# 3dlg-hcvc/minsu3d

Measured on AMD Instinct MI355X. Metric: scenes/sec (fwd+bwd) PointGroup on ~150k-pt 2cm voxels, higher is better.
Workload: dtype f32; 1 GPU; PointGroup m=16, synthetic ScanNet-shaped scenes (~144k points, ~106k voxels @2cm each), 4 scenes/GPU/step, grouping+ScoreNet branch on, fwd+loss+bwd+Adam; scenes_per_gpu=4, parallelism=dp1, grouping_inputs=GT labels, GT offsets + N(0,4cm) (random-init net groups nothing)

## Files before the change

include/minsu3d_hip.h:

```cpp
#ifndef MINSU3D_HIP_H
#define MINSU3D_HIP_H
#include <stddef.h>
#include <stdint.h>

#ifdef __cplusplus
extern "C" {
#endif

#define MS3D_E_WORKSPACE 10001
#define MS3D_E_UNSUPPORTED 10002
#define MS3D_E_INTERNAL 10003

typedef void *ms3d_stream_t;

const char *ms3d_version(void);

size_t ms3d_ballquery_workspace_bytes(int n);
int ms3d_ballquery_batch_p(int n, int meanActive, float radius, const float *xyz, const uint8_t *batch_idxs,
                           const int *batch_offsets, int n_scenes, int max_scene_points, int *idx,
                           int *start_len, int *n_active , int *capped ,
                           void *workspace, size_t workspace_bytes, ms3d_stream_t stream);

size_t ms3d_bfs_workspace_bytes(int N);
int ms3d_pg_bfs_cluster(const int16_t *semantic_label, const int *ball_query_idxs, long n_edges ,
// ... 172 lines not shown
int ms3d_spconv_layer_backward(const float *x, const float *dy, const float *wf_buf, const int *nbr_fwd,
                               const int *nbr_bwd, int Vin, int Vout, int K, int Cin, int Cout, const float *scale,
                               const float *shift, const float *mean, const float *invstd, int pre_relu, int training,
                               int need_dx, float *dx,
                               const float *dx_add ,
                               float *dgb, float *dW, float *ws,
                               const int *ol_fwd_kt_start , const int *ol_fwd_entries,
                               const int *pl_bwd_tile_start , const int *pl_bwd_entries,
                               void *ev_start , void *ev_stop,
                               void *ev_wg_start , void *ev_wg_stop,
                               float *ws_wgrad ,
                               ms3d_stream_t wgrad_stream ,
                               int join ,
                               float *wgrad_slabs ,
                               int *wgrad_deferred_nblk ,
                               void *wgrad_deferred_launch ,
                               ms3d_stream_t stream);
int ms3d_spconv_aux_kind_p(int K, int Cin, int Cout, int precision);
int ms3d_spconv_prep_weights_multi_p(const void *descs, int n, int total_blocks, int precision, ms3d_stream_t stream);
int ms3d_spconv_wgrad_pieces(int Vout, int K, int Cin, int Cout, int offset_list, int precision);
size_t ms3d_spconv_wgrad_ws_floats_p(int Vout, int K, int Cin, int Cout, int precision);
int ms3d_spconv_backward_weight_p(const float *in, const float *dout, const int *nbr, int Vout, int K, int Cin,
                                  int Cout, float *dW, const float *pre_scale, const float *pre_shift, int pre_relu,
                                  float *partial_ws, const int *ol_kt_start, const int *ol_entries, int precision,
                                  ms3d_stream_t stream);
int ms3d_spconv_layer_forward_p(const float *x, const float *W, const int *nbr_fwd, int Vout, int K, int Cin, int Cout,
                                int mirror_bwd, const float *pre_scale, const float *pre_shift, int pre_relu,
                                const float *residual, const float *bias, float *wf_buf, float *y, float *stat_partial,
                                const int *pl_tile_start, const int *pl_entries, void *ev_start, void *ev_stop,
                                int precision, ms3d_stream_t stream);
int ms3d_spconv_layer_backward_p(const float *x, const float *dy, const float *wf_buf, const int *nbr_fwd,
                                 const int *nbr_bwd, int Vin, int Vout, int K, int Cin, int Cout, const float *scale,
                                 const float *shift, const float *mean, const float *invstd, int pre_relu, int training,
                                 int need_dx, float *dx, const float *dx_add, float *dgb, float *dW, float *ws,
                                 const int *ol_fwd_kt_start, const int *ol_fwd_entries, const int *pl_bwd_tile_start,
                                 const int *pl_bwd_entries, void *ev_start, void *ev_stop, void *ev_wg_start,
                                 void *ev_wg_stop, float *ws_wgrad, ms3d_stream_t wgrad_stream, int join,
                                 float *wgrad_slabs, int *wgrad_deferred_nblk, void *wgrad_deferred_launch, int precision,
                                 ms3d_stream_t stream);
int ms3d_spconv_wgrad_is_bf16x3_g(int Vout, int K, int Cin, int Cout, int offset_list, int submanifold);
int ms3d_spconv_backward_weight_g(const float *in, const float *dout, const int *nbr, int Vin, int Vout, int K, int Cin,
                                  int Cout, float *dW, const float *pre_scale, const float *pre_shift, int pre_relu,
                                  float *partial_ws, const int *ol_kt_start, const int *ol_entries, int submanifold,
                                  int precision, ms3d_stream_t stream);
int ms3d_spconv_layer_backward_g(const float *x, const float *dy, const float *wf_buf, const int *nbr_fwd,
                                 const int *nbr_bwd, int Vin, int Vout, int K, int Cin, int Cout, const float *scale,
                                 const float *shift, const float *mean, const float *invstd, int pre_relu, int training,
                                 int need_dx, float *dx, const float *dx_add, float *dgb, float *dW, float *ws,
                                 const int *ol_fwd_kt_start, const int *ol_fwd_entries, const int *pl_bwd_tile_start,
                                 const int *pl_bwd_entries, void *ev_start, void *ev_stop, void *ev_wg_start,
                                 void *ev_wg_stop, float *ws_wgrad, ms3d_stream_t wgrad_stream, int join,
                                 float *wgrad_slabs, int *wgrad_deferred_nblk, void *wgrad_deferred_launch, int precision,
                                 int submanifold, ms3d_stream_t stream);
size_t ms3d_spconv_wgrad_launch_bytes(void);
int ms3d_spconv_wgrad_is_table_walk(int Vout, int K, int Cin, int Cout, int offset_list);
int ms3d_spconv_wgrad_multi(const void *descs, int n_desc, int total_blocks, int variant, ms3d_stream_t stream);
int ms3d_wgrad_reduce_blocks(long n, const float *slabs, const float *dW, int *wide );
int ms3d_wgrad_reduce_multi(const void *descs, int n_desc, int total_blocks, ms3d_stream_t stream);

int ms3d_bn_stats(const float *x, long V, int C, float eps, float momentum, const float *gamma, const float *beta,
                  float *running_mean, float *running_var, float *mean, float *invstd, float *scale, float *shift,
                  float *partial_ws, int partial_rows, ms3d_stream_t stream);
int ms3d_bn_apply(const float *x, long V, int C, const float *scale, const float *shift, int relu, float *y,
                  ms3d_stream_t stream);
int ms3d_reduce_partials(const float *partial, int nparts, int n, float *out, ms3d_stream_t stream);
int ms3d_column_sum(const float *x, long V, int C, float *partial_ws, int partial_rows, float *out2c, ms3d_stream_t stream);
int ms3d_bn_bwd_apply(const float *dz, const float *x, long V, int C, const float *scale, const float *mean,
                      const float *invstd, const float *s1s2, float *dx, ms3d_stream_t stream);
int ms3d_bn_bwd_reduce_apply(const float *partial, int nparts, const float *dz, const float *x, long V, int C,
                             const float *scale, const float *mean, const float *invstd, const float *add, float *dx,
                             float *s1s2, ms3d_stream_t stream);
int ms3d_bn_bwd_apply_add(const float *dz, const float *x, long V, int C, const float *scale, const float *mean,
                          const float *invstd, const float *s1s2, const float *add, float *dx, ms3d_stream_t stream);
int ms3d_bn_bwd_partial(const float *dy, const float *x, long V, int C, const float *scale, const float *shift,
                        const float *mean, const float *invstd, int relu, float *dz, float *partial_ws,
                        int partial_rows, int *nparts_out , ms3d_stream_t stream);

int ms3d_proposal_cross_intersection(const int *pair_point, const int *pair_cluster, int S, int P, int *inter ,
                                     ms3d_stream_t stream);
int ms3d_nms_greedy(const int *inter, const int *order, int P, float threshold, unsigned char *suppressed_ws, int *pick,
                    int *n_pick, ms3d_stream_t stream);

int ms3d_elastic_distort(const double *xyz , int N, float *noise, float *noise_tmp, int bx, int by, int bz,
                         double gran, double mag, double *out , ms3d_stream_t stream);

int ms3d_adam_chunk_elems(void);
int ms3d_adam_step(const int *chunks, int n_chunks, void *const *p_ptrs, const void *const *g_ptrs, void *const *m_ptrs,
                   void *const *v_ptrs, const long *sizes, float lr, float beta1, float beta2, float eps,
                   float weight_decay, double bias_correction1, double bias_correction2, ms3d_stream_t stream);
int ms3d_adam_step_multi(const int *chunks, int n_chunks, void *const *p_ptrs, const void *const *g_ptrs,
                         void *const *m_ptrs, void *const *v_ptrs, const long *sizes, const float *coef, float beta1,
                         float beta2, float eps, float weight_decay, ms3d_stream_t stream);

size_t ms3d_scan_i32_workspace_bytes(void);
int ms3d_scan_i32(const int *in, int *out, int n, int *total_out_dev, void *workspace, ms3d_stream_t stream);

int ms3d_point_losses_blocks(long N);
int ms3d_point_losses_forward(const float *scores , const short *labels , const float *pred_offsets ,
                              const float *centre , const float *xyz , const short *instance_ids ,
                              long N, int C, float *d_scores, float *d_norm, float *d_dir, double *partial_ws, float *out5,
                              ms3d_stream_t stream);
int ms3d_point_losses_scale_grads(float *d_scores, long n_scores, float *d_norm, const float *d_dir, long n_off,
                                  const float *out5, const float *g_sem, const float *g_norm, const float *g_dir,
                                  ms3d_stream_t stream);

#ifdef __cplusplus
// ... 4 lines not shown
```

minsu3d_amd/MinkowskiEngine/functional.py:

```python
import contextlib
import threading

import torch

from ..backend import get_backend

PRECISION_CODES = {"highest": 0, "high": 1, "medium": 2}
_pass = threading.local()


def precision_code(name):
    try:
        return PRECISION_CODES[name]
    except KeyError:
        raise ValueError(f"unknown float32 matmul precision {name!r}") from None


@contextlib.contextmanager
def pass_precision(code):
    prev = getattr(_pass, "code", None)
    _pass.code = code
    try:
        yield
    finally:
# ... 92 lines not shown
                skip[1].armed = True
            elif not (skip[1].armed and residual is not None):
                skip = None
        ctx.skip = skip
        ctx.save_for_backward(x, W)
        ctx.mark_non_differentiable(stats)
        ctx.set_materialize_grads(False)
        return y, stats

    @staticmethod
    def backward(ctx, dy, _dstats):
        be = get_backend()
        spec, bn = ctx.spec, ctx.bn
        x, W = ctx.saved_tensors
        dy = dy.contiguous()
        role, link = ctx.skip if ctx.skip is not None else (None, None)
        add = None
        if role == "head":
            add, link.grad = link.grad, None
        if bn is not None and not bn["relu"]:
            wft = be.prep_weights(W.view(spec.K, spec.cin, spec.cout), spec.K, spec.cout, spec.cin, transpose=True,
                                  mirror=spec.mirror)
            da = be.conv_forward(dy, wft, spec.nbr_bwd, spec.vin, spec.K, spec.cout, spec.cin)
            dz, dgb = be.bn_bwd_reduce(da, x, bn["scale"], bn["shift"], bn["mean"], bn["invstd"], False)
            dx = (be.bn_bwd_apply(dz, x, bn["scale"], bn["mean"], bn["invstd"], dgb) if bn["training"] else dz * bn["scale"])
            dW = be.conv_backward_weight(x, dy, spec.nbr_fwd, spec.vout, spec.K, spec.cin, spec.cout,
                                         pre=(bn["scale"], bn["shift"]), pre_relu=False, **_pk(ctx.prec), **_sk(spec))
        else:
            fused = add is not None and ctx.needs_input_grad[0] and be.fuses_dx_add(bn)
            extra = {"dx_add": add} if fused else {}
            if _queue(ctx.defer) is not None:
                extra["defer"] = _queue(ctx.defer)
            elif (not ctx.w_direct or (W.is_leaf and W.grad is not None)) and hasattr(be, "wgrad_stream_mode") \
                    and be.wgrad_stream_mode() == 2:
                extra["join_now"] = True
            dx, dgb, dW = be.conv_layer_backward(x, dy, ctx.wf_buf, spec.nbr_fwd, spec.nbr_bwd, spec.vin, spec.vout,
                                                 spec.K, spec.cin, spec.cout, bn, ctx.needs_input_grad[0], **extra,
                                                 **_pk(ctx.prec), **_sk(spec))
            if fused:
                add = None
        if add is not None and dx is not None:
            dx = dx + add
        dgamma = dgb[1] if dgb is not None else None
        dbeta = dgb[0] if dgb is not None else None
        d_res = dy if ctx.has_res else None
        if role == "tail" and ctx.has_res:
            link.grad, d_res = dy, None
        db = None
        if ctx.bias_shape is not None and ctx.needs_input_grad[9]:
            db = (be.column_sum(dy) if (hasattr(be, "column_sum") and dy.is_cuda) else dy.sum(0)).view(ctx.bias_shape)
        return dx, dW.view_as(W), dgamma, dbeta, d_res, None, None, None, None, db


class ResBlockFn(torch.autograd.Function):

    @staticmethod
    def forward(ctx, x, W1, g0, b0, W2, g1, b1, spec, stats_in, bn0, bn1, want_stats):
        be = get_backend()
        V = spec.vout
        tok = getattr(be, "weight_token", None)
        prec = ctx.prec = conv_precision(be)
        r1, r2 = _ready(W1, tok, prec), _ready(W2, tok, prec)
        fast = None
        if (r1 is not None and r2 is not None and spec.cin == spec.cout and torch.is_tensor(stats_in) and x.is_contiguous()
                and hasattr(be, "res_block_forward")):
            fast = be.res_block_forward(x, stats_in, r1, r2, spec.nbr_fwd, V, spec.cout, bn0, g0.detach(), b0.detach(), bn1,
                                        g1.detach(), b1.detach(), want_stats, **_pk(prec))
        if fast is not None:
            y1, y2, st2, (m0, i0, s0, h0), (m1, i1, s1, h1) = fast
            wf1, wf2 = r1, r2
        else:
            m0, i0, s0, h0 = be.bn_finalize(stats_in, V, bn0.eps, bn0.momentum, g0.detach(), b0.detach(), bn0.running_mean,
                                            bn0.running_var)
            y1, st1, wf1 = be.conv_layer_forward(x, W1, spec.nbr_fwd, V, 27, spec.cin, spec.cout, True, (s0, h0), True, None,
                                                 None, True, **({"wf_ready": r1} if r1 is not None else {}), **_pk(prec))
            m1, i1, s1, h1 = be.bn_finalize(st1, V, bn1.eps, bn1.momentum, g1.detach(), b1.detach(), bn1.running_mean,
                                            bn1.running_var)
            y2, st2, wf2 = be.conv_layer_forward(y1, W2, spec.nbr_fwd, V, 27, spec.cout, spec.cout, True, (s1, h1), True, x,
                                                 None, want_stats, **({"wf_ready": r2} if r2 is not None else {}), **_pk(prec))
        ctx.spec, ctx.wf = spec, (wf1, wf2)
        ctx.bn = (dict(scale=s0, shift=h0, mean=m0, invstd=i0, relu=True, training=True),
                  dict(scale=s1, shift=h1, mean=m1, invstd=i1, relu=True, training=True))
        ctx.defer = (_defer_of(W1, tok), _defer_of(W2, tok))
        ctx.save_for_backward(x, y1, W1, W2)
        if st2 is None:
            st2 = x.new_zeros(0)
        ctx.mark_non_differentiable(st2)
        ctx.set_materialize_grads(False)
        return y2, st2

    @staticmethod
    def backward(ctx, dy, _dstats):
        be = get_backend()
        spec = ctx.spec
        x, y1, W1, W2 = ctx.saved_tensors
        dy = dy.contiguous()
        V, c0, c1 = spec.vout, spec.cin, spec.cout
        e2 = {"defer": _queue(ctx.defer[1])} if _queue(ctx.defer[1]) is not None else {}
        dx1, dgb1, dW2 = be.conv_layer_backward(y1, dy, ctx.wf[1], spec.nbr_fwd, spec.nbr_bwd, V, V, 27, c1, c1, ctx.bn[1], True, **e2,
                                                **_pk(ctx.prec))
        e1 = {"defer": _queue(ctx.defer[0])} if _queue(ctx.defer[0]) is not None else {}
        dx, dgb0, dW1 = be.conv_layer_backward(x, dx1, ctx.wf[0], spec.nbr_fwd, spec.nbr_bwd, V, V, 27, c0, c1, ctx.bn[0],
                                               ctx.needs_input_grad[0], dx_add=dy, **e1, **_pk(ctx.prec))
        return dx, dW1.view_as(W1), dgb0[1], dgb0[0], dW2.view_as(W2), dgb1[1], dgb1[0], None, None, None, None, None


class ResBlockDownFn(torch.autograd.Function):

    @staticmethod
    def forward(ctx, x, Wd, W1, g0, b0, W2, g1, b1, spec, ident, stats_in, bn0, bn1):
        be = get_backend()
        V, cin, cout = spec.vout, spec.cin, spec.cout
        tok = getattr(be, "weight_token", None)
        prec = ctx.prec = conv_precision(be)

        def ready(W):
            r = _ready(W, tok, prec)
            return dict({"wf_ready": r} if r is not None else {}, **_pk(prec))

        skip, _, wfd = be.conv_layer_forward(x, Wd.view(1, cin, cout), ident, V, 1, cin, cout, False, None, False, None, None,
                                             False, **ready(Wd))
        if isinstance(stats_in, tuple):
            m0, i0, s0, h0 = be.bn_finalize_parts(stats_in, V, bn0.eps, bn0.momentum, g0.detach(), b0.detach(),
                                                  bn0.running_mean, bn0.running_var)
        else:
            m0, i0, s0, h0 = be.bn_finalize(stats_in, V, bn0.eps, bn0.momentum, g0.detach(), b0.detach(), bn0.running_mean,
                                            bn0.running_var)
        y1, st1, wf1 = be.conv_layer_forward(x, W1, spec.nbr_fwd, V, 27, cin, cout, True, (s0, h0), True, None, None, True,
                                             **ready(W1))
        m1, i1, s1, h1 = be.bn_finalize(st1, V, bn1.eps, bn1.momentum, g1.detach(), b1.detach(), bn1.running_mean,
                                        bn1.running_var)
        y2, st2, wf2 = be.conv_layer_forward(y1, W2, spec.nbr_fwd, V, 27, cout, cout, True, (s1, h1), True, skip, None, True,
                                             **ready(W2))
        ctx.spec, ctx.wf, ctx.ident = spec, (wfd, wf1, wf2), ident
        ctx.bn = (dict(scale=s0.contiguous(), shift=h0.contiguous(), mean=m0.contiguous(), invstd=i0.contiguous(), relu=True,
                       training=True),
                  dict(scale=s1, shift=h1, mean=m1, invstd=i1, relu=True, training=True))

        ctx.defer = (_defer_of(Wd, tok), _defer_of(W1, tok), _defer_of(W2, tok))
        ctx.save_for_backward(x, y1, Wd, W1, W2)
        ctx.mark_non_differentiable(st2)
        ctx.set_materialize_grads(False)
        return y2, st2

    @staticmethod
    def backward(ctx, dy, _dstats):
        be = get_backend()
        spec = ctx.spec
        x, y1, Wd, W1, W2 = ctx.saved_tensors
        dy = dy.contiguous()
        V, cin, cout = spec.vout, spec.cin, spec.cout
        ex = lambda d: dict({"defer": _queue(d)} if _queue(d) is not None else {}, **_pk(ctx.prec))
        dx1, dgb1, dW2 = be.conv_layer_backward(y1, dy, ctx.wf[2], spec.nbr_fwd, spec.nbr_bwd, V, V, 27, cout, cout, ctx.bn[1],
                                                True, **ex(ctx.defer[2]))
        need = ctx.needs_input_grad[0]
        dxb, dgb0, dW1 = be.conv_layer_backward(x, dx1, ctx.wf[1], spec.nbr_fwd, spec.nbr_bwd, V, V, 27, cin, cout, ctx.bn[0],
                                                need, **ex(ctx.defer[1]))
        dx, _, dWd = be.conv_layer_backward(x, dy, ctx.wf[0], ctx.ident, ctx.ident, V, V, 1, cin, cout, None, need,
                                            **({"dx_add": dxb} if need else {}), **ex(ctx.defer[0]))
        return dx, dWd.view_as(Wd), dW1.view_as(W1), dgb0[1], dgb0[0], dW2.view_as(W2), dgb1[1], dgb1[0], None, None, None, None, None


class BnReluConvFn(torch.autograd.Function):

    @staticmethod
    def forward(ctx, x, W, g, b, spec, stats_in, bn, want_stats):
        be = get_backend()
        tok = getattr(be, "weight_token", None)
        if isinstance(stats_in, tuple):
            m0, i0, s0, h0 = be.bn_finalize_parts(stats_in, spec.vin, bn.eps, bn.momentum, g.detach(), b.detach(),
                                                  bn.running_mean, bn.running_var)
        else:
            m0, i0, s0, h0 = be.bn_finalize(stats_in, spec.vin, bn.eps, bn.momentum, g.detach(), b.detach(), bn.running_mean,
                                            bn.running_var)
        prec = ctx.prec = conv_precision(be)
        r = _ready(W, tok, prec)
        y, st, wf = be.conv_layer_forward(x, W.view(spec.K, spec.cin, spec.cout), spec.nbr_fwd, spec.vout, spec.K, spec.cin,
                                          spec.cout, spec.mirror, (s0, h0), True, None, None, want_stats,
                                          **({"wf_ready": r} if r is not None else {}), **_pk(prec))
        ctx.spec, ctx.wf = spec, wf
        ctx.bn = dict(scale=s0.contiguous(), shift=h0.contiguous(), mean=m0.contiguous(), invstd=i0.contiguous(), relu=True,
                      training=True)
        ctx.defer = _defer_of(W, tok)
        ctx.save_for_backward(x, W)
        if st is None:
            st = x.new_zeros(0)
        ctx.mark_non_differentiable(st)
        ctx.set_materialize_grads(False)
        return y, st

    @staticmethod
    def backward(ctx, dy, _dstats):
        be = get_backend()
        spec = ctx.spec
        x, W = ctx.saved_tensors
        e = {"defer": _queue(ctx.defer)} if _queue(ctx.defer) is not None else {}
        dx, dgb, dW = be.conv_layer_backward(x, dy.contiguous(), ctx.wf, spec.nbr_fwd, spec.nbr_bwd, spec.vin, spec.vout, spec.K,
                                             spec.cin, spec.cout, ctx.bn, ctx.needs_input_grad[0], **e, **_pk(ctx.prec), **_sk(spec))
        return dx, dW.view_as(W), dgb[1], dgb[0], None, None, None, None


class BNActFn(torch.autograd.Function):
    @staticmethod
    def forward(ctx, x, gamma, beta, bn):
        ctx.bn = bn
        ctx.save_for_backward(x)
        return get_backend().bn_apply(x, bn["scale"], bn["shift"], bn["relu"])

    @staticmethod
    def backward(ctx, dy):
# ... 235 lines not shown
```

minsu3d_amd/backend.py:

```python
import ctypes as C
import os

import numpy as np
import torch

from . import _lib

_BACKEND = None


def get_backend():
    global _BACKEND
    if _BACKEND is None:
        _BACKEND = HipBackend()
    return _BACKEND


def set_backend(b):
    global _BACKEND
    prev = _BACKEND
    _BACKEND = b
    return prev


# ... 83 lines not shown
def wgrad_stream(device):
    s = _WGRAD.get(device)
    if s is None:
        s = _WGRAD[device] = torch.cuda.Stream(device=device)
    return s


_HEADS = {}


def heads_stream(device):
    s = _HEADS.get(device)
    if s is None:
        s = _HEADS[device] = torch.cuda.Stream(device=device)
    return s


def side_stream(device):
    s = _SIDE.get(device)
    if s is None:
        s = _SIDE[device] = torch.cuda.Stream(device=device)
    return s


def _load_host_ext():
    if os.environ.get("MS3D_HOST_EXT", "1") == "0":
        return None
    path = os.path.join(os.path.dirname(os.path.abspath(__file__)), "lib", "_ms3d_host.so")
    if not os.path.exists(path) or (os.environ.get("MS3D_LIB") and os.environ["MS3D_LIB"] != _lib.LIB_PATH):
        return None
    import importlib.util
    try:
        spec = importlib.util.spec_from_file_location("_ms3d_host", path)
        mod = importlib.util.module_from_spec(spec)
        spec.loader.exec_module(mod)
        return mod
    except (ImportError, OSError) as e:
        import warnings
        warnings.warn(f"minsu3d_amd: host extension {path} did not load ({e}); using the ctypes path")
        return None


class HipBackend:
    name = "hip"

    def __init__(self):
        self.lib = _lib.lib()
        self.ext = _load_host_ext() if not os.environ.get("MS3D_LIB") else None
        self.ws = _Workspace()
        self.kernel_timer = None
        self.weight_token = 0
        self.matmul_precision_aware = True
        self._prep_table = None

    @staticmethod
    def _dev(t):
        if not t.is_cuda:
            if not torch.cuda.is_available():
                raise _lib.HipLibraryError("HipBackend needs a GPU (got a CPU tensor and no device is present); "
                                           "the product path has no CPU fallback")
            t = t.cuda(non_blocking=True)
        return t.contiguous()

    def ballquery_batch_p(self, coords, batch_idxs, batch_offsets, radius, meanActive, max_scene_points=0):
        coords = self._dev(coords); batch_idxs = self._dev(batch_idxs); batch_offsets = self._dev(batch_offsets)
        n = coords.size(0)
        dev = coords.device
        start_len = torch.zeros((n, 2), dtype=torch.int32, device=dev)
        if n == 0:
            return torch.zeros(0, dtype=torch.int32, device=dev), start_len
        if max_scene_points <= 0:
            max_scene_points = SCENE_BOUNDS.get(batch_offsets)
            if max_scene_points is None:
                max_scene_points = int((batch_offsets[1:] - batch_offsets[:-1]).max().item())
                SCENE_BOUNDS.put(batch_offsets, max_scene_points)
        ws_bytes = self.lib.ms3d_ballquery_workspace_bytes(n)
        ws = self.ws.get("bq", ws_bytes, dev)
        n_active, capped = C.c_int(0), C.c_int(0)
        timer = self.kernel_timer
        ev0 = timer.op_begin() if timer is not None else None
        hint_key = (round(float(radius), 6), int(meanActive))
        hints = self.__dict__.setdefault("_bq_mean_active", {})
        meanActive = max(int(meanActive), hints.get(hint_key, 0))
        while True:
            idx = torch.empty(n * meanActive, dtype=torch.int32, device=dev)
            rc = self.lib.ms3d_ballquery_batch_p(
                n, int(meanActive), C.c_float(radius), _lib.ptr(coords), _lib.ptr(batch_idxs),
                _lib.ptr(batch_offsets), int(batch_offsets.numel() - 1), int(max_scene_points), _lib.ptr(idx),
                _lib.ptr(start_len), C.byref(n_active), C.byref(capped), _lib.ptr(ws), C.c_size_t(ws.numel()),
                _lib.stream_handle())
            _lib.check(rc, "ms3d_ballquery_batch_p")
            if n_active.value <= n * meanActive:
                break
            meanActive = int(n_active.value // n + 1)
            hints[hint_key] = meanActive + meanActive // 8 + 1
        if ev0 is not None:
            timer.op_end("ballquery_batch_p", ev0, n * 20 + n_active.value * (6.64 * 12 + 4))
        GRAPHS.put(start_len, int(capped.value))
        return idx[:n_active.value], start_len

    def _bfs(self, fn_name, args_head, ball_idx, start_len, args_tail):
        hint = int(GRAPHS.get(start_len, -1))
        ball_idx = self._dev(ball_idx); start_len = self._dev(start_len)
        N = start_len.size(0)
        dev = start_len.device
        cluster_idxs = torch.empty((max(N, 1), 2), dtype=torch.int32, device=dev)
# ... 236 lines not shown
            _lib.ptr(d_scores), C.c_long(d_scores.numel()), _lib.ptr(d_off[0]), _lib.ptr(d_off[1]),
            C.c_long(d_off[0].numel()), _lib.ptr(out5), _lib.ptr(g_sem), _lib.ptr(g_norm), _lib.ptr(g_dir),
            _lib.stream_handle()), "ms3d_point_losses_scale_grads")

    def _iou(self, fn_name, prop_idx, prop_off, inst_labels, inst_pointnum, sigmoid=None):
        prop_idx = self._dev(prop_idx); prop_off = self._dev(prop_off)
        inst_labels = self._dev(inst_labels); inst_pointnum = self._dev(inst_pointnum)
        assert prop_idx.dtype == torch.int32 and inst_labels.dtype == torch.int16
        I, P = inst_pointnum.numel(), prop_off.numel() - 1
        iou = torch.zeros((P, I), dtype=torch.float32, device=prop_idx.device)
        args = [I, P, _lib.ptr(prop_idx), _lib.ptr(prop_off), _lib.ptr(inst_labels), _lib.ptr(inst_pointnum),
                _lib.ptr(iou)]
        if sigmoid is not None:
            args.append(_lib.ptr(self._dev(sigmoid)))
        rc = getattr(self.lib, fn_name)(*args, _lib.stream_handle())
        _lib.check(rc, fn_name)
        return iou

    def get_iou(self, pi, po, il, pn): return self._iou("ms3d_get_iou", pi, po, il, pn)
    def get_mask_iou_on_cluster(self, pi, po, il, pn): return self._iou("ms3d_get_mask_iou_on_cluster", pi, po, il, pn)
    def get_mask_iou_on_pred(self, pi, po, il, pn, sg): return self._iou("ms3d_get_mask_iou_on_pred", pi, po, il, pn, sg)

    def get_mask_label(self, prop_idx, prop_off, inst_labels, inst_cls, iou, ignored_label, iou_thr):
        prop_idx = self._dev(prop_idx); prop_off = self._dev(prop_off); iou = self._dev(iou)
        P, I = iou.shape
        ml = torch.zeros(prop_idx.shape, dtype=torch.bool, device=prop_idx.device)
        mlm = torch.zeros(prop_idx.shape, dtype=torch.bool, device=prop_idx.device)
        rc = self.lib.ms3d_get_mask_label(I, P, int(ignored_label), C.c_float(iou_thr), _lib.ptr(prop_idx),
                                          _lib.ptr(prop_off), _lib.ptr(self._dev(inst_labels)),
                                          _lib.ptr(self._dev(inst_cls)), _lib.ptr(iou), _lib.ptr(ml), _lib.ptr(mlm),
                                          _lib.stream_handle())
        _lib.check(rc, "ms3d_get_mask_label")
        return ml, mlm


def _f32(t):
    return None if t is None else t.contiguous()


def _p(t):
    return None if t is None else t.data_ptr()


_VP, _I = C.c_void_p, C.c_int
_FAST_ARGTYPES = {
    "ms3d_spconv_layer_forward": [_VP] * 3 + [_I] * 5 + [_VP] * 2 + [_I] + [_VP] * 5 + [_VP] * 2 + [_VP] * 2 + [_VP],
    "ms3d_spconv_layer_backward": [_VP] * 5 + [_I] * 5 + [_VP] * 4 + [_I] * 3 + [_VP] * 5 + [_VP] * 4 + [_VP] * 4 +
                                  [_VP, _VP, _I, _VP, _VP, _VP, _VP],
    "ms3d_spconv_layer_forward_p": [_VP] * 3 + [_I] * 5 + [_VP] * 2 + [_I] + [_VP] * 5 + [_VP] * 2 + [_VP] * 2 + [_I, _VP],
    "ms3d_spconv_layer_backward_p": [_VP] * 5 + [_I] * 5 + [_VP] * 4 + [_I] * 3 + [_VP] * 5 + [_VP] * 4 + [_VP] * 4 +
                                    [_VP, _VP, _I, _VP, _VP, _VP, _I, _VP],
    "ms3d_spconv_layer_backward_g": [_VP] * 5 + [_I] * 5 + [_VP] * 4 + [_I] * 3 + [_VP] * 5 + [_VP] * 4 + [_VP] * 4 +
                                    [_VP, _VP, _I, _VP, _VP, _VP, _I, _I, _VP],
    "ms3d_bn_finalize": [_VP, _I, C.c_long, _I, C.c_float, C.c_float] + [_VP] * 4 + [_VP] * 4 + [_VP],
}


class KernelTimer:

    def __init__(self, lib):
        self.lib = lib
        lib.ms3d_event_create.restype = C.c_void_p
        lib.ms3d_event_elapsed_ms.restype = C.c_float
        self.records = []
        self.sampling = False
        self.steps_sampled = 0
        self._pool = []

    def reserve(self, n_events):
        while len(self._pool) < n_events:
            self._pool.append(C.c_void_p(self.lib.ms3d_event_create()))

    def _event(self):
        return self._pool.pop() if self._pool else C.c_void_p(self.lib.ms3d_event_create())

    def conv(self, kind, K, cin, cout, nbr, rows):
        if not self.sampling:
            return None
        pairs = getattr(nbr, "_ms3d_pairs_dev", None)
        if pairs is None:
            pairs = (nbr >= 0).sum()
            nbr._ms3d_pairs_dev = pairs
        ev = (self._event(), self._event())
        self.records.append((("spconv_" + kind, K, cin, cout, rows), ev[0], ev[1],
                             (pairs, (cin + cout) * 4 + 8, K * cin * cout * 4), 2 * cin * cout))
        return ev

    def conv_group(self, kind, layers):
        if not self.sampling or not layers:
            return None
        ev = (self._event(), self._event())
        parts = []
        for K, cin, cout, rows, nbr in layers:
            pairs = getattr(nbr, "_ms3d_pairs_dev", None)
            if pairs is None:
                pairs = (nbr >= 0).sum()
                nbr._ms3d_pairs_dev = pairs
            parts.append((pairs, (cin + cout) * 4 + 8, K * cin * cout * 4, 2 * cin * cout))
        K, cin, cout, rows, _ = layers[0]
        self.records.append((("spconv_" + kind, K, cin, cout, rows, len(layers)), ev[0], ev[1], parts, None))
        return ev

    def op_begin(self):
        if not self.sampling:
            return None
        ev = self._event()
# ... 575 lines not shown
        if not on:
            return None
        q = WgradQueue(self.lib, self.kernel_timer)
        q.side_mode = self.wgrad_stream_mode() == 3
        return q

    def wgrad_batch_enabled(self):
        on = self.__dict__.get("_wgrad_batch")
        if on is None:
            on = self._wgrad_batch = os.environ.get("MS3D_WGRAD_BATCH", "1") != "0"
        return on

    def conv_layer_forward(self, x, W3, nbr_fwd, vout, K, cin, cout, mirror_bwd, pre, pre_relu, residual, bias,
                           want_stats, wf_ready=None, precision=0):
        x = self._dev(x)
        dev = x.device
        wf_buf = wf_ready if wf_ready is not None else torch.empty(self.wf_floats(K, cin, cout), dtype=torch.float32, device=dev)
        pl = self.pairlist(nbr_fwd, K, vout, cin, cout)
        nparts = self._geom("ms3d_spconv_partial_blocks", vout, K, cin, cout, self._pl_rows(pl)) if want_stats else 0
        ps, pb = (pre if pre is not None else (None, None))
        timer = self.kernel_timer
        tok = timer.conv("fwd", K, cin, cout, nbr_fwd, vout) if timer is not None else None
        ev0, ev1 = tok if tok is not None else (None, None)
        ext = self.ext
        if ext is not None:
            y, stats = ext.conv_layer_forward(
                x, None if wf_ready is not None else self._dev(W3), nbr_fwd, vout, K, cin, cout, bool(mirror_bwd),
                _f32(ps), _f32(pb), bool(pre_relu), _f32(residual), _f32(bias), wf_buf, nparts, pl[0], pl[1],
                (ev0.value or 0) if ev0 is not None else 0, (ev1.value or 0) if ev1 is not None else 0, int(precision))
            return y, stats, wf_buf
        y = torch.empty((vout, cout), dtype=torch.float32, device=dev)
        stats = torch.empty((nparts, 2, cout), dtype=torch.float32, device=dev) if want_stats else None
        _lib.check(self._fast("ms3d_spconv_layer_forward_p")(
            _p(x), _p(None if wf_ready is not None else self._dev(W3)), _p(nbr_fwd), int(vout), int(K), int(cin), int(cout),
            int(bool(mirror_bwd)), _p(_f32(ps)), _p(_f32(pb)), int(bool(pre_relu)), _p(_f32(residual)),
            _p(_f32(bias)), _p(wf_buf), _p(y), _p(stats), _p(pl[0]), _p(pl[1]),
            ev0, ev1, int(precision), _lib.stream_handle()), "ms3d_spconv_layer_forward_p")
        return y, stats, wf_buf

    def res_block_forward(self, x, stats_in, wf1, wf2, nbr, V, c, bn0, g0, b0, bn1, g1, b1, want_stats, precision=0):
        ext = self.ext
        timer = self.kernel_timer
        if (ext is None or (timer is not None and getattr(timer, "sampling", True)) or not hasattr(ext, "res_block_forward")
                or os.environ.get("MS3D_RESBLOCK_EXT", "1") == "0"):
            return None
        pl = self.pairlist(nbr, 27, V, c, c)
        nparts = self._geom("ms3d_spconv_partial_blocks", V, 27, c, c, self._pl_rows(pl))
        y1, y2, st2, o0, o1 = ext.res_block_forward(
            x, stats_in, wf1, wf2, nbr, V, c, pl[0], pl[1], nparts, bool(want_stats), _f32(g0), _f32(b0), bn0.running_mean,
            bn0.running_var, bn0.eps, bn0.momentum, _f32(g1), _f32(b1), bn1.running_mean, bn1.running_var, bn1.eps, bn1.momentum,
            int(precision))
        return y1, y2, st2, o0.unbind(0), o1.unbind(0)

    def conv_layer_backward(self, x, dy, wf_buf, nbr_fwd, nbr_bwd, vin, vout, K, cin, cout, bn, need_dx, dx_add=None,
                            defer=None, join_now=False, precision=0, submanifold=None):
        sub = -1 if submanifold is None else int(bool(submanifold))
        x = self._dev(x); dy = self._dev(dy)
        dev = x.device
        ws = self.ws.get("layer", 4 * self._geom("ms3d_spconv_layer_ws_floats", vin, vout, K, cin, cout), dev)
        has_bn = bn is not None
        want_dx = need_dx or has_bn
        plf = self.offsetlist(nbr_fwd, K, vout)
        plb = self.pairlist(nbr_bwd, K, vin, cout, cin) if want_dx else (None, None)
        timer = self.kernel_timer
        tok = timer.conv("fwd", K, cout, cin, nbr_bwd, vin) if (timer is not None and want_dx) else None
        ev0, ev1 = tok if tok is not None else (None, None)
        tok = timer.conv("wgrad", K, cin, cout, nbr_fwd, vout) if timer is not None else None
        ev2, ev3 = tok if tok is not None else (None, None)
        mode = self.wgrad_stream_mode()
        batch = defer is not None and mode == 0 and self.wgrad_batch_enabled() and \
            self._geom("ms3d_spconv_wgrad_is_table_walk", vout, K, cin, cout, int(plf[0] is not None)) == 1
        timing = None
        if batch and ev2 is not None:
            timing = timer.records.pop()[0][1:] + (nbr_fwd,)
            timer._pool.extend((ev2, ev3))
            ev2 = ev3 = None
        if self.ext is not None and mode == 0:
            evs = [(e.value or 0) if e is not None else 0 for e in (ev0, ev1, ev2, ev3)]
            dx, dgb, dW, slabs, nblk, desc = (self.ext.conv_layer_backward_g if sub >= 0 else self.ext.conv_layer_backward)(
                x, dy, wf_buf, nbr_fwd, nbr_bwd, vin, vout, K, cin, cout,
                bn["scale"] if has_bn else None, bn["shift"] if has_bn else None, bn["mean"] if has_bn else None,
                bn["invstd"] if has_bn else None, bool(has_bn and bn["relu"]), bool(has_bn and bn["training"]), bool(need_dx),
                _f32(dx_add) if (dx_add is not None and need_dx) else None, ws, plf[0], plf[1], plb[0], plb[1], *evs,
                self._geom("ms3d_spconv_wgrad_ws_floats", vout, K, cin, cout) if defer is not None else 0, batch,
                int(precision), *((sub,) if sub >= 0 else ()))
            if desc:
                defer.add_launch(desc, (x, dy, nbr_fwd, bn, slabs, dW), timing)
            if nblk > 0:
                defer.add(slabs, dW, K * cin * cout, nblk)
            return dx, dgb, dW
        dx = torch.empty((vin, cin), dtype=torch.float32, device=dev) if want_dx else None
        dgb = torch.empty((2, cin), dtype=torch.float32, device=dev) if has_bn else None
        dW = torch.empty((K, cin, cout), dtype=torch.float32, device=dev)
        side = wgrad_stream(dev) if mode else None
        ws2 = None
        if side is not None:
            with torch.cuda.stream(side):
                ws2 = self.ws.get("layer_wgrad", 4 * self._geom("ms3d_spconv_layer_ws_floats", vin, vout, K, cin, cout), dev)
            if mode != 3:
                defer = None
        slabs, n_defer = None, None
        if defer is not None:
            if "_defer_n" not in self.__dict__:
                self._defer_n = C.c_int(0)
                self._defer_n_addr = C.addressof(self._defer_n)
            slabs = torch.empty(self._geom("ms3d_spconv_wgrad_ws_floats", vout, K, cin, cout), dtype=torch.float32, device=dev)
            n_defer = self._defer_n_addr
        launch = (C.c_char * 128)() if (batch and slabs is not None) else None
        _lib.check(self._fast("ms3d_spconv_layer_backward_g")(
            _p(x), _p(dy), _p(wf_buf), _p(nbr_fwd), _p(nbr_bwd), int(vin), int(vout), int(K),
            int(cin), int(cout), _p(bn["scale"] if has_bn else None), _p(bn["shift"] if has_bn else None),
            _p(bn["mean"] if has_bn else None), _p(bn["invstd"] if has_bn else None),
            int(bool(has_bn and bn["relu"])), int(bool(has_bn and bn["training"])), int(bool(need_dx)), _p(dx),
            _p(_f32(dx_add) if (dx_add is not None and need_dx) else None), _p(dgb), _p(dW), _p(ws), _p(plf[0]), _p(plf[1]), _p(plb[0]),
            _p(plb[1]), ev0, ev1, ev2, ev3, _p(ws2), side.cuda_stream if side is not None else None,
            int(mode == 1 or (mode == 2 and join_now) or (mode == 3 and defer is None)), _p(slabs), n_defer,
            C.addressof(launch) if launch is not None else None, int(precision),
            sub if sub >= 0 else int(K == 27 and vin == vout), _lib.stream_handle()),
            "ms3d_spconv_layer_backward_g")
        if launch is not None and np.frombuffer(launch, dtype=np.int32, count=6)[4] != 0:
            defer.add_launch(bytes(launch), (x, dy, nbr_fwd, bn, slabs, dW), timing)
        if slabs is not None and self._defer_n.value > 0:
            defer.add(slabs, dW, K * cin * cout, self._defer_n.value)
        if mode == 2:
            x.record_stream(side); dy.record_stream(side); dW.record_stream(side)
            if not join_now:
                self._queue_wgrad_join(side)
        elif mode == 3 and defer is not None:
            x.record_stream(side); dy.record_stream(side); dW.record_stream(side)
            if slabs is not None:
                slabs.record_stream(side)
        return (dx if need_dx else None), dgb, dW

    @staticmethod
    def fuses_dx_add(bn):
        return bn is None or (bool(bn["relu"]) and bool(bn["training"]))

    def wgrad_stream_mode(self):
        m = self.__dict__.get("_wgrad_mode")
        if m is None:
            m = self._wgrad_mode = int(os.environ.get("MS3D_WGRAD_STREAM", "0"))
        return m

    def _queue_wgrad_join(self, side):
        if self.__dict__.get("_wgrad_join_queued"):
            return

        def join():
            self._wgrad_join_queued = False
            torch.cuda.current_stream().wait_stream(side)
        try:
            torch.autograd.Variable._execution_engine.queue_callback(join)
            self._wgrad_join_queued = True
        except RuntimeError:
            join()

    def conv_backward_weight(self, x, dout, nbr, vout, K, cin, cout, pre=None, pre_relu=False, precision=0, submanifold=None):
        x = self._dev(x); dout = self._dev(dout)
        dW = torch.empty((K, cin, cout), dtype=torch.float32, device=x.device)
        ps, pb = (pre if pre is not None else (None, None))
        self.lib.ms3d_spconv_wgrad_ws_floats.restype = C.c_size_t
        ws = self.ws.get("wgrad", 4 * self.lib.ms3d_spconv_wgrad_ws_floats(int(vout), int(K), int(cin), int(cout)), x.device)
        ol = self.offsetlist(nbr, K, vout)
        if submanifold is not None:
            _lib.check(self.lib.ms3d_spconv_backward_weight_g(
                _lib.ptr(x), _lib.ptr(dout), _lib.ptr(nbr), int(x.size(0)), int(vout), int(K), int(cin), int(cout), _lib.ptr(dW),
                _lib.ptr(_f32(ps)), _lib.ptr(_f32(pb)), int(bool(pre_relu)), _lib.ptr(ws), _lib.ptr(ol[0]), _lib.ptr(ol[1]),
                int(bool(submanifold)), int(precision), _lib.stream_handle()), "ms3d_spconv_backward_weight_g")
            return dW
        _lib.check(self.lib.ms3d_spconv_backward_weight_p(
            _lib.ptr(x), _lib.ptr(dout), _lib.ptr(nbr), int(vout), int(K), int(cin), int(cout), _lib.ptr(dW),
            _lib.ptr(_f32(ps)), _lib.ptr(_f32(pb)), int(bool(pre_relu)), _lib.ptr(ws), _lib.ptr(ol[0]), _lib.ptr(ol[1]),
            int(precision), _lib.stream_handle()), "ms3d_spconv_backward_weight_p")
        return dW
# ... 90 lines not shown
```

minsu3d_amd/csrc/spconv.hip:

```cpp
#include <stdlib.h>
#include <atomic>
#include <map>
#include <mutex>
#include <unordered_map>
#include "common.h"
#include "../../include/minsu3d_hip.h"

typedef float f32x4 __attribute__((ext_vector_type(4)));

namespace {

constexpr int MAX_NBT = 8;
constexpr size_t LDS_BUDGET = 150 * 1024;
static hipError_t raise_lds_ceiling(const void *fn)
{
    hipFuncAttributes fa;
    hipError_t e = hipFuncGetAttributes(&fa, fn);
    if (e != hipSuccess) return e;
    return hipFuncSetAttribute(fn, hipFuncAttributeMaxDynamicSharedMemorySize, 160 * 1024 - (int)fa.sharedSizeBytes);
}

int env_int(const char *name, int dflt)
{
    const char *e = getenv(name);
    return e ? atoi(e) : dflt;
}

struct ConvArgs {
    const float *in;
    const float *wf;
    const float *wfs;
    const void *wfb;
    const int *nbr;
    float *out;
    const float *pre_scale;
    const float *pre_shift;
    const float *residual;
    const float *bias;
    const float *bn_x;
    const float *bn_scale;
    const float *bn_shift;
    const float *bn_mean;
    const float *bn_invstd;
    float *bn_partial;
    int out_stats;
    int Vout, K, Cin, Cout;
    int NCH;
    int NBtot;
    int G;
    int GC;
    int RT;
    int ntiles;
    int pre_relu;
    const int *pl_tile_start;
    const int *pl_entries;
    int dyn_picks;
    int k1_path;
    float *ws_slabs;
    unsigned *ws_cnt;
    int ws_ng, ws_kg, ws_R, ws_tpp;
};

__device__ __forceinline__ long stream_slot(long o, int NBtot)
{
    const int lane = (int)(o & 63);
    long r = o >> 6;
    const int nb = (int)(r % NBtot); r /= NBtot;
    const int t = (int)(r & 3); r >>= 2;
    return ((r * NBtot + nb) * 64 + lane) * 4 + t;
}

typedef __bf16 bf16x8 __attribute__((ext_vector_type(8)));

__host__ __device__ constexpr int aux_pieces(int aux_kind) { return aux_kind == 2 ? 3 : aux_kind == 3 ? 2 : aux_kind == 4 ? 1 : 0; }

__host__ __device__ inline bool bf3_dims_ok(int K, int Cin, int Cout)
{
    return K > 1 && Cin % 16 == 0 && Cout % 16 == 0 && Cin >= 48 && Cout >= 48 && Cin <= 256 && Cout <= 256;
}

__device__ __forceinline__ void split3(float v, __bf16 &h0, __bf16 &h1, __bf16 &h2)
{
    h0 = (__bf16)v;
    const float r1 = v - (float)h0;
    h1 = (__bf16)r1;
    const float r2 = r1 - (float)h1;
    h2 = (__bf16)r2;
}

typedef float f32x2_t __attribute__((ext_vector_type(2)));
typedef __bf16 bf16x2_t __attribute__((ext_vector_type(2)));
__device__ __forceinline__ uint32_t cvt_pk_bf16(float a, float b)
{
    const bf16x2_t h = __builtin_convertvector((f32x2_t){a, b}, bf16x2_t);
    return *reinterpret_cast<const uint32_t *>(&h);
}
template <int P = 3>
__device__ __forceinline__ void act_split8(const f32x4 &lo, const f32x4 &hi, bool affine, const f32x4 &s0, const f32x4 &s1,
                                           const f32x4 &b0, const f32x4 &b1, float floor_, int keep, bf16x8 &a0, bf16x8 &a1,
                                           bf16x8 &a2)
{
    float v[8];
#pragma unroll
    for (int t = 0; t < 4; t++) { v[t] = lo[t]; v[4 + t] = hi[t]; }
    if (affine) {
#pragma unroll
        for (int t = 0; t < 4; t++) {
            v[t] = fmaxf(fmaf(v[t], s0[t], b0[t]), floor_);
            v[4 + t] = fmaxf(fmaf(v[4 + t], s1[t], b1[t]), floor_);
        }
    }
    uint32_t q0[4], q1[4], q2[4];
    if constexpr (P == 3) {
#pragma unroll
// ... 139 lines not shown
        const int ch = (int)(r % NB), k = (int)(r / NB);
        const int c = 16 * ch + 4 * q + t, j = 16 * nb + jl;
        const int ks = d.mirror_bwd ? (d.K - 1 - k) : k;
        const float v = (c < d.Cout && j < d.Cin) ? d.W[((size_t)ks * d.Cin + j) * d.Cout + c] : 0.f;
        d.wft[o] = v;
        if (d.stream == 1) d.wft[total + stream_slot(o, NCH)] = v;
    }
    if (d.stream == 5 - PB) {
        constexpr int P = PB;
        auto image = [&](float *aux, int Ci, int Co, int nb_tot, bool transposed) {
            const int NC32 = (Ci + 31) >> 5;
            if (o >= (long)d.K * NC32 * nb_tot * 64) return;
            const int g = lane >> 4;
            long r = o >> 6;
            const int nb = (int)(r % nb_tot); r /= nb_tot;
            const int c32 = (int)(r % NC32), k = (int)(r / NC32);
            const int ks = (transposed && d.mirror_bwd) ? (d.K - 1 - k) : k;
            const int j = 16 * nb + jl;
            bf16x8 p0, p1, p2;
#pragma unroll
            for (int e = 0; e < 8; e++) {
                const int c = 32 * c32 + 8 * g + e;
                float v = 0.f;
                if (c < Ci && j < Co) v = transposed ? d.W[((size_t)ks * d.Cin + j) * d.Cout + c] : d.W[((size_t)ks * d.Cin + c) * d.Cout + j];
                __bf16 h0, h1, h2;
                split3(v, h0, h1, h2);
                p0[e] = h0; p1[e] = h1; p2[e] = h2;
            }
            bf16x8 *dst = reinterpret_cast<bf16x8 *>(aux) + ((((size_t)k * NC32 + c32) * nb_tot + nb) * P) * 64 + lane;
            dst[0] = p0;
            if (P >= 2) dst[64] = p1;
            if (P >= 3) dst[128] = p2;
        };
        image(d.wf + total, d.Cin, d.Cout, NB, false);
        image(d.wft + total, d.Cout, d.Cin, NCH, true);
    }
}

constexpr int OG = 9;

template <int GSZ>
__device__ __forceinline__ void load_indices(const ConvArgs &p, int row, int g0, int k_hi, int (&idx)[GSZ])
{
    const bool row_ok = row >= 0 && row < p.Vout;
    const int safe_row = row_ok ? row : 0;
#pragma unroll
    for (int u = 0; u < GSZ; u++) {
        const int k = min(g0 + u, k_hi - 1);
        const int v = p.nbr[(size_t)k * p.Vout + safe_row];
        idx[u] = v | ((row_ok && g0 + u < k_hi) ? 0 : -1);
    }
}

template <int NBT, bool ALIGNED, bool DIRECT = false, int GSZ = ((DIRECT || NBT < 5) ? OG : (NBT < 7 ? 7 : 6))>
__device__ __forceinline__ void accumulate_offsets(const ConvArgs &p, const float *__restrict__ sW, int k_lo, int k_hi,
                                                   int kw0, int my_row, int q, int nb0, f32x4 (&acc)[NBT])
{
    const int l = lane_id();
    int opaque0 = 0;
    asm volatile("" : "+s"(opaque0));
    for (int g0 = k_lo; g0 < k_hi; g0 += GSZ) {
        int idx[GSZ];
        load_indices(p, my_row, g0, k_hi, idx);
        bool any[GSZ];
#pragma unroll
        for (int u = 0; u < GSZ; u++) any[u] = __ballot(idx[u] >= 0) != 0ull;
        auto fetch = [&](int ch, f32x4 (&a)[GSZ], f32x4 &sc, f32x4 &sh) {
            const int c0 = 16 * ch + 4 * q;
#pragma unroll
            for (int u = 0; u < GSZ; u++) {
                const float *row = p.in + (size_t)max(idx[u], 0) * p.Cin + c0;
                if (ALIGNED) {
                    a[u] = *reinterpret_cast<const f32x4 *>(row);
                } else {
#pragma unroll
                    for (int t = 0; t < 4; t++) a[u][t] = (c0 + t < p.Cin) ? row[t] : 0.f;
                }
            }
            if (p.pre_scale) {
                if (ALIGNED) {
                    sc = *reinterpret_cast<const f32x4 *>(p.pre_scale + c0);
                    sh = *reinterpret_cast<const f32x4 *>(p.pre_shift + c0);
                } else {
#pragma unroll
                    for (int t = 0; t < 4; t++) {
                        sc[t] = (c0 + t < p.Cin) ? p.pre_scale[c0 + t] : 0.f;
                        sh[t] = (c0 + t < p.Cin) ? p.pre_shift[c0 + t] : 0.f;
                    }
                }
            }
        };
        f32x4 a_next[GSZ], sc_next = {0.f, 0.f, 0.f, 0.f}, sh_next = sc_next;
        if (DIRECT) fetch(0, a_next, sc_next, sh_next);
        for (int ch = 0; ch < p.NCH; ch++) {
            f32x4 a[GSZ], s = {0.f, 0.f, 0.f, 0.f}, b = s;
            if (DIRECT) {
#pragma unroll
                for (int u = 0; u < GSZ; u++) a[u] = a_next[u];
                s = sc_next;
                b = sh_next;
                if (ch + 1 < p.NCH) fetch(ch + 1 + opaque0, a_next, sc_next, sh_next);
            } else {
                fetch(ch, a, s, b);
            }
            if (p.pre_scale) {
#pragma unroll
                for (int u = 0; u < GSZ; u++)
#pragma unroll
                    for (int t = 0; t < 4; t++) {
                        const float v = fmaf(a[u][t], s[t], b[t]);
                        a[u][t] = p.pre_relu ? fmaxf(v, 0.f) : v;
                    }
            }
#pragma unroll
            for (int u = 0; u < GSZ; u++) {
                const int keep = ~(idx[u] >> 31);
#pragma unroll
                for (int t = 0; t < 4; t++) a[u][t] = __int_as_float(__float_as_int(a[u][t]) & keep);
            }
            if (DIRECT) {
                constexpr int UB0 = NBT <= 2 ? GSZ : (NBT <= 4 ? 3 : 1);
                constexpr int UB = UB0 < GSZ ? UB0 : GSZ;
#pragma unroll
                for (int u0 = 0; u0 < GSZ; u0 += UB) {
                    float wreg[UB][4][NBT];
#pragma unroll
                    for (int uu = 0; uu < UB; uu++) {
                        const float *w = p.wf + ((size_t)((min(g0 + u0 + uu, p.K - 1) * p.NCH + ch) * 4) * p.NBtot + nb0) * 64 + l;
#pragma unroll
                        for (int t = 0; t < 4; t++)
#pragma unroll
                            for (int nb = 0; nb < NBT; nb++) wreg[uu][t][nb] = w[(size_t)(t * p.NBtot + nb) * 64];
                    }
                    __builtin_amdgcn_sched_barrier(0);
#pragma unroll
                    for (int uu = 0; uu < UB; uu++)
#pragma unroll
                        for (int t = 0; t < 4; t++)
#pragma unroll
                            for (int nb = 0; nb < NBT; nb++)
                                acc[nb] = __builtin_amdgcn_mfma_f32_16x16x4f32(a[u0 + uu][t], wreg[uu][t][nb], acc[nb], 0, 0, 0);
                }
            } else {
#pragma unroll
                for (int u = 0; u < GSZ; u++) {
                    if (!any[u]) continue;
                    const float *w = sW + (size_t)(((kw0 + (g0 - k_lo) + u) * p.NCH + ch) * 4) * NBT * 64 + l;
#pragma unroll
                    for (int t = 0; t < 4; t++) {
#pragma unroll
                        for (int nb = 0; nb < NBT; nb++)
                            acc[nb] = __builtin_amdgcn_mfma_f32_16x16x4f32(a[u][t], w[(t * NBT + nb) * 64], acc[nb], 0, 0, 0);
                    }
                }
            }
        }
// ... 294 lines not shown
        }
    };

    {
        const int tile = vb * waves + wave_id();
        const int row0 = tile * 16, my_row = row0 + (l & 15);
        f32x4 acc[NBT];
#pragma unroll
        for (int nb = 0; nb < NBT; nb++) acc[nb] = (f32x4){0.f, 0.f, 0.f, 0.f};
        int idx[OG];
        load_idx(0, min(p.G, p.K), my_row, idx);
        for (int k0 = 0; k0 < p.K; k0 += p.G) {
            const int gn = min(p.G, p.K - k0);
            int idx_n[OG];
            load_idx(k0 + p.G, min(k0 + 2 * p.G, p.K), my_row, idx_n);
            bool any[OG];
#pragma unroll
            for (int u = 0; u < OG; u++) any[u] = __ballot(idx[u] >= 0) != 0ull;
            for (int c_lo = 0; c_lo < NC32; c_lo += GC) {
                const int ccnt = min(GC, NC32 - c_lo);
                Round r;
                gather(c_lo, idx, r);
                __syncthreads();
                stage(k0, gn, c_lo, ccnt);
                asm volatile("s_waitcnt vmcnt(0)" ::: "memory");
                __syncthreads();
                if (tile < p.ntiles) compute(c_lo, 0, ccnt, idx, any, r, acc);
                for (int cc = 1; cc < ccnt; cc++) {
                    gather(c_lo + cc, idx, r);
                    if (tile < p.ntiles) compute(c_lo + cc, cc, ccnt, idx, any, r, acc);
                }
            }
#pragma unroll
            for (int u = 0; u < OG; u++) idx[u] = idx_n[u];
        }
        if (tile < p.ntiles) store_tile<NBT>(p, row0, nb0, acc, s_part + (size_t)wave_id() * stat_slot_floats(NBT));
    }
    if (with_partial) stats_flush<NBT>(p, s_part, waves, nb0);
}

constexpr int bf3_round_offsets(int nbt) { return nbt == 2 || nbt == 4 || nbt == 6 ? 5 : 4; }

template <int NBT, int P = 3>
int launch_fwd_bf3(const ConvArgs &p, dim3 grid, int threads, size_t lds, hipStream_t stream)
{
    constexpr int OG = bf3_round_offsets(NBT);
    static const hipError_t attr = raise_lds_ceiling((const void *)spconv_fwd_bf3_kernel<NBT, OG, P>);
    MS3D_CHECK(attr);
    spconv_fwd_bf3_kernel<NBT, OG, P><<<grid, threads, lds, stream>>>(p);
    MS3D_LAUNCH_CHECK();
    return 0;
}

template <int NBT, bool ALIGNED>
__global__ __launch_bounds__(256) void spconv_fwd_small_kernel(ConvArgs p)
{
    extern __shared__ float lds[];
    const int l = lane_id(), q = l >> 4;
    const int waves = blockDim.x >> 6;
    const int nb0 = blockIdx.y * NBT;
    float *s_acc = lds;
    float *s_part = lds + (size_t)(waves - 1) * NBT * 256;
    const bool with_partial = p.bn_x != nullptr || p.out_stats != 0;
    if (with_partial) stats_clear<NBT>(s_part, 1);
    const int rt = p.RT > 1 ? p.RT : 1;
    for (int tt = 0; tt < rt; tt++) {
        const int tile = blockIdx.x * rt + tt;
        if (tile >= p.ntiles) break;
        const int row0 = tile * 16, my_row = row0 + (l & 15);
        f32x4 acc[NBT];
#pragma unroll
        for (int nb = 0; nb < NBT; nb++) acc[nb] = (f32x4){0.f, 0.f, 0.f, 0.f};
        const int k_lo = wave_id() * OG, k_hi = min(p.K, k_lo + OG);
        if (p.K == 1 && (p.k1_path & 2)) { if (k_lo < k_hi) accumulate_k1<NBT, ALIGNED, true>(p, nullptr, my_row, q, nb0, acc); }
        else if (k_lo < k_hi) accumulate_offsets<NBT, ALIGNED, true>(p, nullptr, k_lo, k_hi, 0, my_row, q, nb0, acc);
        if (tt > 0) __syncthreads();
        if (wave_id() > 0) {
#pragma unroll
            for (int nb = 0; nb < NBT; nb++)
#pragma unroll
                for (int r = 0; r < 4; r++) s_acc[((size_t)(wave_id() - 1) * NBT + nb) * 256 + r * 64 + l] = acc[nb][r];
        }
        __syncthreads();
        if (wave_id() == 0) {
            for (int w = 1; w < waves; w++)
#pragma unroll
                for (int nb = 0; nb < NBT; nb++)
#pragma unroll
                    for (int r = 0; r < 4; r++) acc[nb][r] += s_acc[((size_t)(w - 1) * NBT + nb) * 256 + r * 64 + l];
            store_tile<NBT>(p, row0, nb0, acc, s_part);
        }
    }
    if (with_partial) stats_flush<NBT>(p, s_part, 1, nb0);
}

template <int NBT, int P = 3>
__global__ __launch_bounds__(256) void spconv_fwd_small_bf3_kernel(ConvArgs p)
{
    extern __shared__ float lds[];
    constexpr int NG = (NBT + 3) / 4;
    constexpr int GB = NBT / NG, GR = NBT % NG;
    const int l = lane_id(), g8 = l >> 4;
    const int waves = blockDim.x >> 6;
    const int nb0 = blockIdx.y * NBT;
    const int NC32 = (p.Cin + 31) >> 5;
    float *s_acc = lds;
    float *s_part = lds + (size_t)(waves - 1) * NBT * 256;
    const bool with_partial = p.bn_x != nullptr || p.out_stats != 0;
    if (with_partial) stats_clear<NBT>(s_part, 1);
    const int tile = blockIdx.x;
    const int row0 = tile * 16, my_row = row0 + (l & 15);
    const bool row_ok = my_row < p.Vout;
    const int safe_row = row_ok ? my_row : 0;
    f32x4 acc[NBT];
#pragma unroll
    for (int nb = 0; nb < NBT; nb++) acc[nb] = (f32x4){0.f, 0.f, 0.f, 0.f};
    const uint4 *img = reinterpret_cast<const uint4 *>(p.wfb);
    const int k_lo = wave_id() * OG, k_hi = min(p.K, k_lo + OG);
    for (int k0 = k_lo; k0 < k_hi; k0 += OGB) {
        int idx[OGB];
#pragma unroll
        for (int u = 0; u < OGB; u++) {
            const int k = min(k0 + u, k_hi - 1);
            const int v = p.nbr[(size_t)k * p.Vout + safe_row];
            idx[u] = v | ((row_ok && k0 + u < k_hi) ? 0 : -1);
        }
        bool any[OGB];
#pragma unroll
// ... 203 lines not shown
        for (int t = 0; t < RT; t++) { g_c.lo[t] = g_n.lo[t]; g_c.hi[t] = g_n.hi[t]; }
        if (wrap) {
#pragma unroll
            for (int t = 0; t < RT; t++) idx_c[t] = idx_n[t];
            load_idx(kn + 1, idx_n);
        }
        k = kn; c32 = c32n;
    }
#pragma unroll
    for (int t = 0; t < RT; t++)
#pragma unroll
        for (int nb = 0; nb < NBT; nb++)
#pragma unroll
            for (int r = 0; r < 4; r++) s_acc[(((size_t)w * RT + t) * NBT + nb) * 256 + r * 64 + l] = acc[t][nb][r];
    __syncthreads();
    for (int t = w; t < RT; t += waves) {
        if (tile0 + t >= p.ntiles) break;
        f32x4 sum[NBT];
#pragma unroll
        for (int nb = 0; nb < NBT; nb++) sum[nb] = (f32x4){0.f, 0.f, 0.f, 0.f};
        for (int ww = 0; ww < waves; ww++)
#pragma unroll
            for (int nb = 0; nb < NBT; nb++)
#pragma unroll
                for (int r = 0; r < 4; r++) sum[nb][r] += s_acc[(((size_t)ww * RT + t) * NBT + nb) * 256 + r * 64 + l];
        store_tile<NBT>(p, (tile0 + t) * 16, nb0, sum, s_part + (size_t)w * stat_slot_floats(NBT));
    }
    if (with_partial) stats_flush<NBT>(p, s_part, waves, nb0);
}

template <int NBT, int RT, int P = 3>
int launch_fwd_small_bf3_rt(const ConvArgs &p, dim3 grid, int threads, size_t lds, hipStream_t stream)
{
    static const hipError_t attr = raise_lds_ceiling((const void *)spconv_fwd_small_bf3_rt_kernel<NBT, RT, P>);
    MS3D_CHECK(attr);
    spconv_fwd_small_bf3_rt_kernel<NBT, RT, P><<<grid, threads, lds, stream>>>(p);
    MS3D_LAUNCH_CHECK();
    return 0;
}

template <int NBT, int P = 3>
int launch_fwd_small_bf3(const ConvArgs &p, dim3 grid, int threads, size_t lds, hipStream_t stream)
{
    spconv_fwd_small_bf3_kernel<NBT, P><<<grid, threads, lds, stream>>>(p);
    MS3D_LAUNCH_CHECK();
    return 0;
}

template <int NBT>
int launch_fwd_small(const ConvArgs &p, dim3 grid, int threads, size_t lds, bool aligned, hipStream_t stream)
{
    const size_t need = ((size_t)(threads / 64 - 1) * NBT * 256 + ((p.bn_x || p.out_stats) ? stat_slot_floats(NBT) : 0)) * sizeof(float) + 16;
    if (lds > need) lds = need;
    if (aligned)
        spconv_fwd_small_kernel<NBT, true><<<grid, threads, lds, stream>>>(p);
    else
        spconv_fwd_small_kernel<NBT, false><<<grid, threads, lds, stream>>>(p);
    MS3D_LAUNCH_CHECK();
    return 0;
}

template <int NBT>
int launch_fwd(const ConvArgs &p, dim3 grid, int threads, size_t lds, bool aligned, hipStream_t stream)
{
    const bool res = p.G >= p.K;
#define MS3D_FWD_LAUNCH(A, R)                                                                                        \
    do {                                                                                                             \
        static const hipError_t attr = raise_lds_ceiling((const void *)spconv_fwd_kernel<NBT, A, R>);                \
        MS3D_CHECK(attr);                                                                                            \
        spconv_fwd_kernel<NBT, A, R><<<grid, threads, lds, stream>>>(p);                                             \
    } while (0)
    if (aligned && res) MS3D_FWD_LAUNCH(true, true);
    else if (aligned) MS3D_FWD_LAUNCH(true, false);
    else if (res) MS3D_FWD_LAUNCH(false, true);
    else MS3D_FWD_LAUNCH(false, false);
#undef MS3D_FWD_LAUNCH
    MS3D_LAUNCH_CHECK();
    return 0;
}


struct WsBlock { int u, g, nb0, k_lo, kcnt, t_begin, t_end; };

template <int NBT>
__device__ __forceinline__ bool ws_block(const ConvArgs &p, WsBlock &b)
{
    const int ny = p.NBtot / NBT, units = p.ws_R * ny;
    const int id = (int)blockIdx.x;
    b.u = (id / (8 * p.ws_ng)) * 8 + (id & 7);
    b.g = (id >> 3) % p.ws_ng;
    if (b.u >= units) return false;
    const int c = b.u % ny, r = b.u / ny;
    b.nb0 = c * NBT;
    b.k_lo = b.g * p.ws_kg;
    b.kcnt = min(p.K, b.k_lo + p.ws_kg) - b.k_lo;
    b.t_begin = r * p.ws_tpp;
    b.t_end = min(p.ntiles, b.t_begin + p.ws_tpp);
    return true;
}

__device__ __forceinline__ f32x4 *ws_slab_ptr(const ConvArgs &p, int g, int tile, int nb)
{
    return reinterpret_cast<f32x4 *>(p.ws_slabs) + (((size_t)g * p.ntiles + tile) * p.NBtot + nb) * 64 + lane_id();
}

template <int NBT>
__device__ __forceinline__ void ws_finish(const ConvArgs &p, const WsBlock &b, float *s_part, int *s_flag)
// ... 712 lines not shown
            }
        }
        if (l < F4) reinterpret_cast<f32x4 *>(acc_t + PSR * RS)[l] = (f32x4){0.f, 0.f, 0.f, 0.f};
        __builtin_amdgcn_wave_barrier();
    }
    if (with_partial) {
        float *scr = acc_t;
        *reinterpret_cast<f32x4 *>(scr + 8 * l) = ep_lane ? st1 : (f32x4){0.f, 0.f, 0.f, 0.f};
        *reinterpret_cast<f32x4 *>(scr + 8 * l + 4) = ep_lane ? st2 : (f32x4){0.f, 0.f, 0.f, 0.f};
        __builtin_amdgcn_wave_barrier();
        if (l < F4) {
            f32x4 a1 = {0.f, 0.f, 0.f, 0.f}, a2 = a1;
            for (int j = 0; j < RPS; j++) {
                const f32x4 v1 = *reinterpret_cast<const f32x4 *>(scr + 8 * (l + j * F4));
                const f32x4 v2 = *reinterpret_cast<const f32x4 *>(scr + 8 * (l + j * F4) + 4);
#pragma unroll
                for (int t = 0; t < 4; t++) { a1[t] += v1[t]; a2[t] += v2[t]; }
            }
            *reinterpret_cast<f32x4 *>(scr + 512 + 4 * l) = a1;
            *reinterpret_cast<f32x4 *>(scr + 512 + CW + 4 * l) = a2;
        }
        __syncthreads();
        float *dst = p.bn_partial + ((size_t)blockIdx.y * gridDim.x + blockIdx.x) * 2 * p.Cout;
        const float *wave0 = s_pre + ((2 * p.Cin + 3) & ~3) + PSCH + 512;
        for (int t = threadIdx.x; t < 2 * p.Cout; t += blockDim.x) {
            const int which = t >= p.Cout, c = t - which * p.Cout - 16 * nb0;
            float sum = 0.f;
            if (c >= 0 && c < CW)
                for (int wv = 0; wv < waves; wv++) sum += wave0[(size_t)wv * pairstream_wave_floats(NBT) + which * CW + c];
            dst[t] = sum;
        }
    }
}

template <int NBT, int CG>
int launch_fwd_pairstream(ConvArgs p, dim3 grid, int threads, size_t lds, hipStream_t stream)
{
    p.ntiles = ms3d_divup(p.Vout, PSR);
    static const hipError_t attr = raise_lds_ceiling((const void *)spconv_fwd_pairstream_kernel<NBT, CG>);
    MS3D_CHECK(attr);
    spconv_fwd_pairstream_kernel<NBT, CG><<<grid, threads, lds, stream>>>(p);
    MS3D_LAUNCH_CHECK();
    return 0;
}

struct WgradArgs {
    const float *in;
    const float *dout;
    const int *nbr;
    float *partial;
    const float *pre_scale;
    const float *pre_shift;
    int Vout, K, Cin, Cout, NBtot, rows_per_block, pre_relu;
    const int *ol_kt_start;
    const int *ol_entries;
};

template <int KG, int NBT>
__device__ __forceinline__ void wgrad_body(const WgradArgs &p, const int bx, const int by, const int bz, float *s_red)
{
    const int l = lane_id(), q = l >> 4, cl = l & 15;
    const int k0 = by * KG;
    const int c = bz * 16 + cl;
    const bool c_ok = c < p.Cin;
    const int c_safe = c_ok ? c : 0;
    const int c_mask = c_ok ? -1 : 0;
    const float sc = (p.pre_scale && c_ok) ? p.pre_scale[c] : 1.f;
    const float sh = (p.pre_scale && c_ok) ? p.pre_shift[c] : 0.f;
    f32x4 acc[KG][NBT];
#pragma unroll
    for (int a = 0; a < KG; a++)
#pragma unroll
        for (int b = 0; b < NBT; b++) acc[a][b] = (f32x4){0.f, 0.f, 0.f, 0.f};

    const int r_begin = bx * p.rows_per_block;
    const int r_end = min(p.Vout, r_begin + p.rows_per_block);
    const int nw = blockDim.x >> 6;
    for (int r0 = r_begin + wave_id() * 4; r0 < r_end; r0 += 8 * nw) {
        int idx[2][KG];
        float a[2][KG], b[2][NBT];
        bool ok[2];
#pragma unroll
        for (int h = 0; h < 2; h++) {
            const int row = r0 + h * 4 * nw + q;
            ok[h] = row < r_end;
            const int safe_row = ok[h] ? row : r_begin;
#pragma unroll
            for (int nb = 0; nb < NBT; nb++) {
                const int j = 16 * nb + cl;
                const float v = p.dout[(size_t)safe_row * p.Cout + (j < p.Cout ? j : 0)];
                b[h][nb] = __int_as_float(__float_as_int(v) & ((ok[h] && j < p.Cout) ? -1 : 0));
            }
#pragma unroll
            for (int kk = 0; kk < KG; kk++) {
                const int v = p.nbr[(size_t)min(k0 + kk, p.K - 1) * p.Vout + safe_row];
                idx[h][kk] = v | ((k0 + kk < p.K && ok[h]) ? 0 : -1);
            }
        }
#pragma unroll
        for (int h = 0; h < 2; h++)
#pragma unroll
            for (int kk = 0; kk < KG; kk++) a[h][kk] = p.in[(size_t)max(idx[h][kk], 0) * p.Cin + c_safe];
#pragma unroll
        for (int h = 0; h < 2; h++) {
#pragma unroll
            for (int kk = 0; kk < KG; kk++) {
                float v = a[h][kk];
                if (p.pre_scale) {
                    v = fmaf(v, sc, sh);
                    if (p.pre_relu) v = fmaxf(v, 0.f);
                }
                a[h][kk] = __int_as_float(__float_as_int(v) & ~(idx[h][kk] >> 31) & c_mask);
            }
#pragma unroll
            for (int kk = 0; kk < KG; kk++) {
                if (__ballot(idx[h][kk] >= 0) == 0ull) continue;
#pragma unroll
                for (int nb = 0; nb < NBT; nb++)
                    acc[kk][nb] = __builtin_amdgcn_mfma_f32_16x16x4f32(a[h][kk], b[h][nb], acc[kk][nb], 0, 0, 0);
            }
        }
    }
    float *dst = p.partial + (size_t)bx * p.K * p.Cin * p.Cout;
#pragma unroll
    for (int kk = 0; kk < KG; kk++) {
        const int k = k0 + kk;
        __syncthreads();
#pragma unroll
        for (int nb = 0; nb < NBT; nb++)
#pragma unroll
            for (int r = 0; r < 4; r++) s_red[(wave_id() * NBT + nb) * 256 + r * 64 + l] = acc[kk][nb][r];
        __syncthreads();
        for (int e = threadIdx.x; e < NBT * 256; e += blockDim.x) {
            float v = 0.f;
            for (int w = 0; w < nw; w++) v += s_red[w * NBT * 256 + e];
            const int nb = e >> 8, r = (e >> 6) & 3, ln = e & 63;
            const int ci = bz * 16 + 4 * (ln >> 4) + r, j = 16 * nb + (ln & 15);
            if (k < p.K && ci < p.Cin && j < p.Cout) dst[((size_t)k * p.Cin + ci) * p.Cout + j] = v;
        }
    }
}

template <int KG, int NBT>
__global__ __launch_bounds__(256) void spconv_wgrad_kernel(WgradArgs p)
{
    __shared__ float s_red[4 * NBT * 256];
    wgrad_body<KG, NBT>(p, blockIdx.x, blockIdx.y, blockIdx.z, s_red);
}

struct WgradLaunch {
    int block_begin;
    int gx, gy, gz;
    int variant;
    int nblk;
    int pad[2];
    WgradArgs p;
};
static_assert(sizeof(WgradLaunch) <= 128, "ms3d_spconv_wgrad_launch_bytes() promises 128");

template <int KG, int NBT>
__global__ __launch_bounds__(256) void spconv_wgrad_multi_kernel(const unsigned char *__restrict__ descs, int n_desc)
{
    __shared__ float s_red[4 * NBT * 256];
    int lo = 0, hi = n_desc - 1;
    const int blk = blockIdx.x;
    while (lo < hi) {
        const int mid = (lo + hi + 1) >> 1;
        if (reinterpret_cast<const WgradLaunch *>(descs + 128 * (size_t)mid)->block_begin <= blk) lo = mid; else hi = mid - 1;
    }
    const WgradLaunch d = *reinterpret_cast<const WgradLaunch *>(descs + 128 * (size_t)lo);
    const int local = blk - d.block_begin;
    wgrad_body<KG, NBT>(d.p, local % d.gx, (local / d.gx) % d.gy, local / (d.gx * d.gy), s_red);
}

template <int P>
__device__ __forceinline__ void split_rows_bf3(long blk, const float *__restrict__ x, long V, int C, int NB, long ntile,
                                               bf16x8 *__restrict__ img)
{
    const long o = blk * 256 + threadIdx.x;
    if (o >= ntile * NB * 64) return;
    const int lane = (int)(o & 63);
    const long tn = o >> 6;
    const int nb = (int)(tn % NB);
    const long t = tn / NB;
    const int j = 16 * nb + (lane & 15);
    bf16x8 p0, p1, p2;
#pragma unroll
    for (int e = 0; e < 8; e++) {
        const long row = 32 * t + 8 * (lane >> 4) + e;
        const float v = (row < V && j < C) ? x[row * C + j] : 0.f;
        __bf16 h0, h1, h2;
        split3(v, h0, h1, h2);
        p0[e] = h0; p1[e] = h1; p2[e] = h2;
    }
    bf16x8 *dst = img + (tn * P) * 64 + lane;
    dst[0] = p0;
    if (P >= 2) dst[64] = p1;
    if (P >= 3) dst[128] = p2;
}

template <int P>
__device__ __forceinline__ void act_split_bf3(long blk, const float *__restrict__ x, long V, int C,
                                              const float *__restrict__ scale, const float *__restrict__ shift, int relu,
                                              bf16x8 *__restrict__ xs)
{
    const int C8 = C >> 3;
    const long o = blk * 256 + threadIdx.x;
    if (o >= V * C8) return;
    const long row = o / C8;
    const int c0 = (int)(o % C8) * 8;
    const f32x4 a = *reinterpret_cast<const f32x4 *>(x + row * C + c0), b = *reinterpret_cast<const f32x4 *>(x + row * C + c0 + 4);
    float v[8] = {a[0], a[1], a[2], a[3], b[0], b[1], b[2], b[3]};
    bf16x8 p0, p1, p2;
#pragma unroll
    for (int e = 0; e < 8; e++) {
        float y = v[e];
        if (scale) {
            y = fmaf(y, scale[c0 + e], shift[c0 + e]);
            if (relu) y = fmaxf(y, 0.f);
        }
        __bf16 h0, h1, h2;
        split3(y, h0, h1, h2);
        p0[e] = h0; p1[e] = h1; p2[e] = h2;
    }
    bf16x8 *dst = xs + (row * P) * C8 + (c0 >> 3);
// ... 243 lines not shown
        const long e4 = (long)b0 * 64 + sub * 16 + g;
        const float4 *p4 = reinterpret_cast<const float4 *>(partial);
        float4 s = make_float4(0.f, 0.f, 0.f, 0.f);
        if (e4 < n4) {
            int b = sl;
            for (; b + 12 < nblk; b += 16) {
                float4 v[4];
#pragma unroll
                for (int u = 0; u < 4; u++) v[u] = p4[(size_t)(b + 4 * u) * n4 + e4];
#pragma unroll
                for (int u = 0; u < 4; u++) { s.x += v[u].x; s.y += v[u].y; s.z += v[u].z; s.w += v[u].w; }
            }
            for (; b < nblk; b += 4) {
                const float4 v = p4[(size_t)b * n4 + e4];
                s.x += v.x; s.y += v.y; s.z += v.z; s.w += v.w;
            }
        }
#pragma unroll
        for (int dd = 16; dd <= 32; dd <<= 1) {
            s.x += __shfl_xor(s.x, dd, 64); s.y += __shfl_xor(s.y, dd, 64);
            s.z += __shfl_xor(s.z, dd, 64); s.w += __shfl_xor(s.w, dd, 64);
        }
        if (sl == 0 && e4 < n4) reinterpret_cast<float4 *>(d.dW)[e4] = s;
        return;
    }
    const int el = threadIdx.x & 15, sl = threadIdx.x >> 4;
    const long n = d.n, e = (long)b0 * 16 + el;
    float s0 = 0.f, s1 = 0.f;
    if (e < n) {
        int b = sl;
        for (; b + 16 < nblk; b += 32) {
            s0 += partial[(size_t)b * n + e];
            s1 += partial[(size_t)(b + 16) * n + e];
        }
        if (b < nblk) s0 += partial[(size_t)b * n + e];
    }
    s_sum[sl][el] = s0 + s1;
    __syncthreads();
    if (threadIdx.x < 16 && e < n) {
        float t = 0.f;
#pragma unroll
        for (int j = 0; j < 16; j++) t += s_sum[j][threadIdx.x];
        d.dW[e] = t;
    }
}

template <int KG, int NBT>
int launch_wgrad(const WgradArgs &p, int nblk_rows, hipStream_t stream, WgradLaunch *defer = nullptr)
{
    dim3 grid(nblk_rows, ms3d_divup(p.K, KG), ms3d_divup(p.Cin, 16));
    if (defer) {
        defer->block_begin = 0;
        defer->gx = grid.x; defer->gy = grid.y; defer->gz = grid.z;
        defer->variant = KG * 100 + NBT;
        defer->nblk = nblk_rows;
        defer->p = p;
        return 0;
    }
    spconv_wgrad_kernel<KG, NBT><<<grid, 256, 0, stream>>>(p);
    MS3D_LAUNCH_CHECK();
    return 0;
}

template <int KG, int NBT>
int launch_wgrad_multi(const void *descs, int n_desc, int total_blocks, hipStream_t stream)
{
    spconv_wgrad_multi_kernel<KG, NBT><<<total_blocks, 256, 0, stream>>>(static_cast<const unsigned char *>(descs), n_desc);
    MS3D_LAUNCH_CHECK();
    return 0;
}

constexpr int WGRAD_TB = 2;

constexpr int wgrad_list_wave_kb(int nbt, int nch, int tb) { return tb * (nch + nbt) > 2 * nch * nbt ? tb * (nch + nbt) : 2 * nch * nbt; }
constexpr int wgrad_list_max_waves(int nbt, int nch, int tb) { return 150 / wgrad_list_wave_kb(nbt, nch, tb) > 16 ? 16 : 150 / wgrad_list_wave_kb(nbt, nch, tb); }

template <int NBT, int NCH, int TB = WGRAD_TB>
__global__ __launch_bounds__(64 * wgrad_list_max_waves(NBT, NCH, TB)) void spconv_wgrad_offsetlist_kernel(WgradArgs p)
{
    constexpr int NT = NCH + NBT;
    constexpr int NA = NCH * NBT;
    constexpr int WAVE_KB = TB * NT > 2 * NA ? TB * NT : 2 * NA;
    extern __shared__ float lds[];
    __shared__ int s_lo[32], s_cum[33], s_pk[16][2];
    const int l = lane_id(), q = l >> 4, cl = l & 15;
    const int nw = blockDim.x >> 6, w = wave_id();
    float *s_tile = lds + (size_t)w * WAVE_KB * 256;
    const int tiles = (p.Vout + MS3D_PL_ROWS - 1) / MS3D_PL_ROWS;
    const int *__restrict__ part_start = p.ol_kt_start + (size_t)p.K * tiles + 1;
    const int t_lo = part_start[blockIdx.x << p.rows_per_block], t_hi = part_start[(blockIdx.x + 1) << p.rows_per_block];
    if (w == 0) {
        const int kk = min(l, p.K - 1);
        const int lo = p.ol_kt_start[(size_t)kk * tiles + t_lo], hi = p.ol_kt_start[(size_t)kk * tiles + t_hi];
        const int n = l < p.K ? hi - lo : 0;
        const int incl = wave_incl_scan(n);
        if (l < p.K) {
            s_lo[l] = lo;
            s_cum[l] = incl - n;
        }
        if (l == p.K - 1) s_cum[p.K] = incl;
    }
    if (threadIdx.x < 32) s_pk[threadIdx.x >> 1][threadIdx.x & 1] = -1;
    __syncthreads();

    const int qs = q ^ ((cl >> 1) & 3);
    const int cbase = blockIdx.z * NCH * 16;
    const int col0 = blockIdx.y * NBT * 16;
    f32x4 sc[NCH], sh[NCH];
#pragma unroll
    for (int ch = 0; ch < NCH; ch++) {
        const int c0 = cbase + 16 * ch + 4 * q;
        const bool ok = p.pre_scale && c0 < p.Cin;
        sc[ch] = ok ? *reinterpret_cast<const f32x4 *>(p.pre_scale + c0) : (f32x4){1.f, 1.f, 1.f, 1.f};
        sh[ch] = ok ? *reinterpret_cast<const f32x4 *>(p.pre_shift + c0) : (f32x4){0.f, 0.f, 0.f, 0.f};
    }
    const int2 *__restrict__ entries = reinterpret_cast<const int2 *>(p.ol_entries);
    float *slab = p.partial + (size_t)blockIdx.x * p.K * p.Cin * p.Cout;
    int opaque0 = 0;
    asm volatile("" : "+s"(opaque0));
    auto store_slab = [&](int k, const f32x4 (&acc)[NA]) {
// ... 358 lines not shown
                    if (!(fmaf(xv.z, sc.z, sh.z) > 0.f)) g.z = 0.f;
                    if (!(fmaf(xv.w, sc.w, sh.w) > 0.f)) g.w = 0.f;
                }
                reinterpret_cast<float4 *>(dz)[e] = g;
                s1[0] += g.x; s1[1 % VEC] += g.y; s1[2 % VEC] += g.z; s1[3 % VEC] += g.w;
                s2[0] += g.x * ((xv.x - mu.x) * is.x); s2[1 % VEC] += g.y * ((xv.y - mu.y) * is.y);
                s2[2 % VEC] += g.z * ((xv.z - mu.z) * is.z); s2[3 % VEC] += g.w * ((xv.w - mu.w) * is.w);
            }
        } else {
            const float sc = scale[c], sh = shift[c], mu = mean[c], is = invstd[c];
#pragma unroll 2
            for (long e = r_begin * CQ + tid; e < e_end; e += stride) {
                const float xv = x[e];
                float g = dy[e];
                if (relu && !(fmaf(xv, sc, sh) > 0.f)) g = 0.f;
                dz[e] = g;
                s1[0] += g;
                s2[0] += g * ((xv - mu) * is);
            }
        }
    }
#pragma unroll
    for (int u = 0; u < VEC; u++) {
        s_red[tid * 2 * VEC + u] = s1[u];
        s_red[tid * 2 * VEC + VEC + u] = s2[u];
    }
    __syncthreads();
    for (int t = tid; t < 2 * C; t += 256) {
        const int which = t >= C, c = t - which * C, cq = c / VEC, u = c - cq * VEC;
        float sum = 0.f;
        for (int j = 0; j < rpp; j++) sum += s_red[(j * CQ + cq) * 2 * VEC + which * VEC + u];
        partial[(size_t)blockIdx.x * 2 * C + t] = sum;
    }
}

__global__ __launch_bounds__(1024) void reduce_partial_kernel(const float *__restrict__ partial, int nparts, int n,
                                                              float *__restrict__ out)
{
    __shared__ double s_sum[16][17];
    const int col = blockIdx.x * 16 + (threadIdx.x & 15), lane_p = threadIdx.x >> 4;
    double s = 0.0;
    if (col < n)
        for (int p = lane_p; p < nparts; p += 64) s += (double)partial[(size_t)p * n + col];
    s += __shfl_xor(s, 16, 64);
    s += __shfl_xor(s, 32, 64);
    if ((threadIdx.x & 63) < 16) s_sum[threadIdx.x >> 6][threadIdx.x & 15] = s;
    __syncthreads();
    if (threadIdx.x < 16 && col < n) {
        double t = 0.0;
#pragma unroll
        for (int i = 0; i < 16; i++) t += s_sum[i][threadIdx.x];
        out[col] = (float)t;
    }
}

struct BnBwdState {
    unsigned long long word[1024];
    int ticket, done;
};

__global__ __launch_bounds__(1024) void bn_bwd_reduce_apply_kernel(const float *__restrict__ partial, int nparts, const float *dz,
                                                                  const float *__restrict__ x, long n, int C, long V,
                                                                  const float *__restrict__ scale,
                                                                  const float *__restrict__ mean,
                                                                  const float *__restrict__ invstd,
                                                                  const float *__restrict__ add, float *dx,
                                                                  float *__restrict__ s1s2_out, BnBwdState *__restrict__ st)
{
    __shared__ double s_sum[16][17];
    __shared__ float s_s[1024];
    __shared__ int s_bid;
    const int n2 = 2 * C, nred = (n2 + 15) / 16;
    if (threadIdx.x == 0) s_bid = atomicAdd(&st->ticket, 1);
    __syncthreads();
    const int bid = s_bid;
    if (bid < nred) {
        const int col = bid * 16 + (threadIdx.x & 15), lane_p = threadIdx.x >> 4;
        double s = 0.0;
        if (col < n2)
            for (int p = lane_p; p < nparts; p += 64) s += (double)partial[(size_t)p * n2 + col];
        s += __shfl_xor(s, 16, 64);
        s += __shfl_xor(s, 32, 64);
        if ((threadIdx.x & 63) < 16) s_sum[threadIdx.x >> 6][threadIdx.x & 15] = s;
        __syncthreads();
        if (threadIdx.x < 16 && col < n2) {
            double t = 0.0;
#pragma unroll
            for (int i = 0; i < 16; i++) t += s_sum[i][threadIdx.x];
            const float f = (float)t;
            s1s2_out[col] = f;
            __hip_atomic_store(&st->word[col], (1ull << 32) | (unsigned long long)__float_as_uint(f), __ATOMIC_RELAXED,
                               __HIP_MEMORY_SCOPE_AGENT);
        }
    }
    for (int t = threadIdx.x; t < n2; t += 1024) {
        unsigned long long w;
        do {
            w = __hip_atomic_load(&st->word[t], __ATOMIC_RELAXED, __HIP_MEMORY_SCOPE_AGENT);
        } while ((w >> 32) == 0);
        s_s[t] = __uint_as_float((unsigned)w);
    }
    __syncthreads();
    if (dx) {
        const float invV = 1.f / (float)V;
        const long stride = (long)gridDim.x * 1024;
        if ((C & 3) == 0) {
// ... 193 lines not shown
        if (sp.slabs) { if (hipStreamSynchronize(stream) != hipSuccess || hipFree(sp.slabs) != hipSuccess) return nullptr; }
        sp.slabs = nullptr; sp.slab_floats = 0;
        const size_t n = need_floats < ((size_t)8 << 20) ? ((size_t)8 << 20) : need_floats + need_floats / 2;
        if (hipMalloc((void **)&sp.slabs, n * sizeof(float)) != hipSuccess) return nullptr;
        sp.slab_floats = n;
    }
    if (need_cnt > sp.ncnt) {
        if (sp.cnt) { if (hipStreamSynchronize(stream) != hipSuccess || hipFree(sp.cnt) != hipSuccess) return nullptr; }
        sp.cnt = nullptr; sp.ncnt = 0;
        const int n = need_cnt < 4096 ? 4096 : 2 * need_cnt;
        if (hipMalloc((void **)&sp.cnt, (size_t)n * sizeof(unsigned)) != hipSuccess) return nullptr;
        if (hipMemset(sp.cnt, 0, (size_t)n * sizeof(unsigned)) != hipSuccess || hipDeviceSynchronize() != hipSuccess) return nullptr;
        sp.ncnt = n;
    }
    return &sp;
}
constexpr int PAIRLIST_MIN_ROWS = 30000;
int pairlist_min_rows()
{
    static const int v = [] {
        const char *e = getenv("MS3D_PAIRLIST_MIN_ROWS");
        return e ? atoi(e) : PAIRLIST_MIN_ROWS;
    }();
    return v;
}
int pairstream_mode()
{
    static const int v = [] { const char *e = getenv("MS3D_PAIRSTREAM"); return e ? atoi(e) : 1; }();
    return v;
}
bool pairlist_shape_ok(int Vout, int K, int Cin, int Cout)
{
    const bool wide_ok = pairstream_mode() == 2 && Cin <= 64 && Cout <= 256 && (size_t)Vout * 8 * Cin < (1ull << 32);
    return pairlist_min_rows() >= 0 && Vout >= pairlist_min_rows() && Vout <= (1 << 22) && K > 1 && K <= 27 &&
           Cin % 16 == 0 && Cout % 16 == 0 && ((Cin <= 32 && Cout <= 32) || wide_ok);
}
bool bf3_enabled()
{
    static const bool on = [] { const char *e = getenv("MS3D_BF16X3"); return !e || atoi(e) != 0; }();
    return on;
}
bool pairstream_layer_ok(int K, int Cin, int Cout)
{
    if (bf3_enabled() && bf3_dims_ok(K, Cin, Cout)) return false;
    const int mode = pairstream_mode();
    const bool on = (mode == 1 && Cin != Cout) || mode == 3 || (mode == 2 && Cin > 64);
    return on && pairlist_min_rows() >= 0 && K > 1 && K <= 27 && Cin % 16 == 0 && Cout % 16 == 0 && (Cin > 32 || Cout > 32) &&
           Cin <= 256 && Cout <= 256;
}
bool pairstream_shape_ok(int Vout, int K, int Cin, int Cout)
{
    return pairstream_layer_ok(K, Cin, Cout) && Vout >= pairlist_min_rows() && Vout <= (1 << 22);
}
constexpr int SMALL_TILES = 1100;
FwdGeom fwd_geometry(int Vout, int K, int Cin, int Cout, bool with_bn_partial, int pl_rows)
{
    const bool with_pairlist = pl_rows != 0;
    FwdGeom g{};
    const int NCH = ms3d_divup(Cin, 16), NBtot = ms3d_divup(Cout, 16);
    const int ntiles = ms3d_divup(Vout, 16);
    static const int small_tiles = [] {
        const char *e = getenv("MS3D_SMALL_TILES");
        return e ? atoi(e) : SMALL_TILES;
    }();
    if (ws_geometry(Vout, K, Cin, Cout, g)) return g;
    if (ntiles <= small_tiles && (size_t)NCH * NBtot >= 4 && ms3d_divup(K, OG) <= 4) {
        const int ks = ms3d_divup(K, OG);
        int ny = ms3d_divup(NBtot, MAX_NBT);
        while (NBtot % ny != 0) ny++;
        while ((long)ntiles * ny * ks < 1024 && ny < NBtot) {
            ny++;
            while (NBtot % ny != 0) ny++;
        }
        g.small = true;
        g.ny = ny;
        g.nbt = NBtot / ny;
        g.threads = ks * 64;
        g.nblk = ntiles;
        g.G = K;
        g.rt = 1;
        g.lds = ((size_t)(ks - 1) * g.nbt * 256 + (with_bn_partial ? stat_slot_floats(g.nbt) : 0)) * sizeof(float) + 16;
        g.ok = ks <= 4 && g.nbt >= 1 && g.nbt <= MAX_NBT;
        static const int env_rt = [] { const char *e = getenv("MS3D_SMALL_RT"); return e ? atoi(e) : 3; }();
        if (bf3_enabled() && bf3_dims_ok(K, Cin, Cout) && g.nbt >= 2 && K >= 4) {
            const int rt = (ntiles >= 3 * 230 && env_rt >= 3) ? 3 : 1;
            if (rt > 1) {
                const int waves = 4;
                g.rt = rt;
                g.threads = waves * 64;
                g.nblk = ms3d_divup(ntiles, rt);
                g.lds = ((size_t)waves * rt * g.nbt * 256 + (with_bn_partial ? waves * stat_slot_floats(g.nbt) : 0)) * sizeof(float) + 16;
            }
        }
        return g;
    }
    if (with_pairlist && pairstream_shape_ok(Vout, K, Cin, Cout)) {
        static const int env_nbt = [] { const char *e = getenv("MS3D_PS_NBT"); return e ? atoi(e) : 0; }();
        static const int env_w = [] { const char *e = getenv("MS3D_PS_W"); return e ? atoi(e) : 8; }();
        int nbt = 1, cg = 1;
        const int max_nbt = env_nbt > 0 ? env_nbt : ((K == 27 && NBtot % 4 == 0) ? 4 : 2);
        for (int c = max_nbt; c >= 1; c--)
            if (NBtot % c == 0) { nbt = c; break; }
        for (int c = 4; c >= 1; c--)
            if (NCH % c == 0) { cg = c; break; }
        const int ny = NBtot / nbt;
        const size_t spart = (size_t)(((2 * Cout + 3) & ~3) + 4 + ((2 * Cin + 3) & ~3)) * sizeof(float);
// ... 42 lines not shown
        const int tiles = ms3d_divup(Vout, cr);
        g.pl_rows = cr;
        if (W > 16) W = 16;
        if (env_w > 0 && W > env_w) W = env_w;
        if (W >= 2) {
            const int wfill = ms3d_divup(tiles, MS3D_PL_PARTS);
            if (W > wfill) W = wfill < 2 ? 2 : wfill;
            g.pairlist = true;
            g.ny = NBtot / nbt;
            g.nbt = nbt;
            g.threads = W * 64;
            g.nblk = MS3D_PL_PARTS;
            g.G = K;
            g.lds = (size_t)K * NCH * 4 * nbt * 64 * sizeof(float) + spart + (size_t)W * pairlist_wave_floats(nbt, cr) * sizeof(float);
            g.ok = true;
            return g;
        }
    }
    int ny = ms3d_divup(NBtot, MAX_NBT);
    while (NBtot % ny != 0) ny++;
    while ((long)ntiles * ny < 1024 && ny < NBtot) {
        ny++;
        while (NBtot % ny != 0) ny++;
    }
    g.ny = ny;
    g.nbt = NBtot / ny;
    const size_t per_offset = (size_t)NCH * 4 * g.nbt * 64 * sizeof(float);
    const size_t extra = with_bn_partial ? STAT_MAX_WAVES * stat_slot_floats(g.nbt) * sizeof(float) : 0;
    const bool resident = per_offset * K + extra <= LDS_BUDGET;
    if (resident) {
        g.G = K;
        const size_t need = per_offset * K + extra;
        int threads = need <= 32 * 1024 ? 256 : (need <= 76 * 1024 ? 512 : 1024);
        while (threads > 128 && (long)ms3d_divup(ntiles, threads / 64) * ny < 128) threads >>= 1;
        g.threads = threads;
        g.nblk = ms3d_divup(ntiles, threads / 64);
        if (g.nblk > 1024) g.nblk = 1024;
        g.lds = need;
    } else {
        g.G = (int)((LDS_BUDGET - extra) / per_offset);
        if (g.G > K) g.G = K;
        static const int env_waves = [] { const char *e = getenv("MS3D_STREAM_WAVES"); return e ? atoi(e) : 0; }();
        const int rounds = ms3d_divup(ms3d_divup(ntiles, 16), 256);
        int waves = env_waves > 0 ? env_waves : ms3d_divup(ntiles, rounds * 256);
        waves = waves < 2 ? 2 : (waves > 16 ? 16 : waves);
        g.threads = waves * 64;
        g.nblk = ms3d_divup(ntiles, waves);
        g.lds = per_offset * g.G + extra;
    }
    if (g.nblk < 1) g.nblk = 1;
    g.ok = g.G >= 1 && g.nbt >= 1 && g.nbt <= MAX_NBT;
    return g;
}
}

extern "C" {

int ms3d_spconv_wants_stream_image(int K, int Cin, int Cout)
{
    return (pairstream_layer_ok(K, Cin, Cout) || pairstream_layer_ok(K, Cout, Cin)) ? 1 : 0;
}

int ms3d_spconv_aux_kind(int K, int Cin, int Cout)
{
    if (bf3_enabled() && bf3_dims_ok(K, Cin, Cout)) return 2;
    return ms3d_spconv_wants_stream_image(K, Cin, Cout) ? 1 : 0;
}

int ms3d_spconv_aux_kind_p(int K, int Cin, int Cout, int precision)
{
    if (precision < 0 || precision > 2) return MS3D_E_UNSUPPORTED;
    const int kind = ms3d_spconv_aux_kind(K, Cin, Cout);
    return kind == 2 ? 2 + precision : kind;
}

int ms3d_kmap_pairlist_wanted(int K, int Vout) { return pairlist_min_rows() >= 0 && Vout >= pairlist_min_rows() && K > 1 && K <= 27; }

int ms3d_spconv_pairlist_rows(int Vout, int K, int Cin, int Cout)
{
    const FwdGeom g = fwd_geometry(Vout, K, Cin, Cout, false, MS3D_PL_ROWS);
    return g.stream ? PSR : (g.pairlist ? g.pl_rows : 0);
}

int ms3d_spconv_pairlist_rows_dense(int Vout, int K, int Cin, int Cout)
{
    const int plain = ms3d_spconv_pairlist_rows(Vout, K, Cin, Cout);
    static const int narrow = env_int("MS3D_PL_NARROW", 1);
    if (plain != MS3D_PL_ROWS || !narrow || K != 27 || Cin != 32 || Cout != 32) return plain;
    const FwdGeom g = fwd_geometry(Vout, K, Cin, Cout, false, PL_ROWS_NARROW);
    return (g.ok && g.pairlist && g.pl_rows == PL_ROWS_NARROW) ? PL_ROWS_NARROW : plain;
}

int ms3d_spconv_partial_blocks(int Vout, int K, int Cin, int Cout, int with_pairlist)
{
    const FwdGeom g = fwd_geometry(Vout, K, Cin, Cout, true, with_pairlist == 1 ? MS3D_PL_ROWS : with_pairlist);
    return g.nblk * g.ny;
}

static int spconv_forward_impl(const float *in, const float *wf, const int *nbr, int Vout, int K, int Cin, int Cout,
                               float *out, const float *pre_scale, const float *pre_shift, int pre_relu,
                               const float *residual, const float *bn_x, const float *bn_scale, const float *bn_shift,
                               const float *bn_mean, const float *bn_invstd, float *bn_partial, int out_stats,
                               const float *bias, const int *pl_tile_start, const int *pl_entries, const float *wf_aux,
                               int aux_kind, ms3d_stream_t stream_);

int ms3d_spconv_forward(const float *in, const float *wf, const int *nbr, int Vout, int K, int Cin, int Cout,
                        float *out, const float *pre_scale, const float *pre_shift, int pre_relu,
                        const float *residual, const float *bn_x, const float *bn_scale, const float *bn_shift,
                        const float *bn_mean, const float *bn_invstd, float *bn_partial, int out_stats,
                        const float *bias, const int *pl_tile_start, const int *pl_entries, const float *wf_stream,
                        ms3d_stream_t stream_)
{
    return spconv_forward_impl(in, wf, nbr, Vout, K, Cin, Cout, out, pre_scale, pre_shift, pre_relu, residual, bn_x, bn_scale,
                               bn_shift, bn_mean, bn_invstd, bn_partial, out_stats, bias, pl_tile_start, pl_entries,
                               wf_stream, wf_stream ? 1 : 0, stream_);
}

static int spconv_forward_impl(const float *in, const float *wf, const int *nbr, int Vout, int K, int Cin, int Cout,
                               float *out, const float *pre_scale, const float *pre_shift, int pre_relu,
                               const float *residual, const float *bn_x, const float *bn_scale, const float *bn_shift,
                               const float *bn_mean, const float *bn_invstd, float *bn_partial, int out_stats,
                               const float *bias, const int *pl_tile_start, const int *pl_entries, const float *wf_stream,
                               int aux_kind, ms3d_stream_t stream_)
{
    hipStream_t stream = (hipStream_t)stream_;
    if (Vout <= 0) return 0;
    ConvArgs p;
    p.bias = bias;
    p.wfs = nullptr;
    p.wfb = nullptr;
    const int pieces = aux_pieces(aux_kind);
    if (aux_kind != 1 && !pieces) wf_stream = nullptr;
    p.pl_tile_start = pl_tile_start; p.pl_entries = pl_entries;
    p.out_stats = (out_stats && bn_partial && !bn_x) ? 1 : 0;
    static const int dyn_picks = [] { const char *e = getenv("MS3D_PL_DYNAMIC"); return e ? atoi(e) : 0; }();
    p.dyn_picks = dyn_picks;
    static const int k1_path = [] { const char *e = getenv("MS3D_K1_PATH"); return e ? atoi(e) : 3; }();
    p.k1_path = k1_path;
    p.in = in; p.wf = wf; p.nbr = nbr; p.out = out; p.pre_scale = pre_scale; p.pre_shift = pre_shift;
    p.residual = residual; p.bn_x = bn_x; p.bn_scale = bn_scale; p.bn_shift = bn_shift; p.bn_mean = bn_mean;
    p.bn_invstd = bn_invstd; p.bn_partial = bn_partial; p.Vout = Vout; p.K = K; p.Cin = Cin; p.Cout = Cout;
    p.NCH = ms3d_divup(Cin, 16); p.NBtot = ms3d_divup(Cout, 16); p.ntiles = ms3d_divup(Vout, 16); p.pre_relu = pre_relu;
    const FwdGeom g = fwd_geometry(Vout, K, Cin, Cout, bn_x != nullptr || p.out_stats,
                                   (pl_tile_start && pl_entries) ? ms3d_kmap_pairlist_rows_of(pl_tile_start) : 0);
    if (!g.ok) return MS3D_E_UNSUPPORTED;
    p.G = g.G;
    dim3 grid(g.nblk, g.ny);
    const bool aligned = (Cin % 16 == 0);
    p.ws_slabs = nullptr; p.ws_cnt = nullptr; p.ws_ng = p.ws_kg = p.ws_R = p.ws_tpp = 0;
    if (g.ws) {
        const int units = g.ws_R * g.ny;
        WsSpace *sp = ws_space(stream, g.ws_ng > 1 ? (size_t)g.ws_ng * p.ntiles * p.NBtot * 256 : 0, units);
        if (!sp) return (int)hipErrorOutOfMemory;
        p.ws_slabs = sp->slabs; p.ws_cnt = sp->cnt;
        p.ws_ng = g.ws_ng; p.ws_kg = g.ws_kg; p.ws_R = g.ws_R; p.ws_tpp = g.ws_tpp;
        const int nblk = ms3d_divup(units, 8) * 8 * g.ws_ng;
        switch (g.nbt) {
            case 1: return launch_fwd_ws<1>(p, nblk, g.threads, g.lds, stream);
            case 2: return launch_fwd_ws<2>(p, nblk, g.threads, g.lds, stream);
            case 3: return launch_fwd_ws<3>(p, nblk, g.threads, g.lds, stream);
            case 4: return launch_fwd_ws<4>(p, nblk, g.threads, g.lds, stream);
        }
        return MS3D_E_UNSUPPORTED;
    }
    if (g.stream) {
        if (!wf_stream || aux_kind != 1) return MS3D_E_UNSUPPORTED;
        p.wfs = wf_stream;
#define MS3D_PS(NBT_, CG_) \
    if (g.nbt == NBT_ && g.cg == CG_) return launch_fwd_pairstream<NBT_, CG_>(p, grid, g.threads, g.lds, stream);
        MS3D_PS(1, 1) MS3D_PS(1, 2) MS3D_PS(1, 3) MS3D_PS(1, 4)
        MS3D_PS(2, 1) MS3D_PS(2, 2) MS3D_PS(2, 3) MS3D_PS(2, 4)
        MS3D_PS(3, 1) MS3D_PS(3, 2) MS3D_PS(3, 3) MS3D_PS(3, 4)
        MS3D_PS(4, 1) MS3D_PS(4, 2) MS3D_PS(4, 3) MS3D_PS(4, 4)
#undef MS3D_PS
        return MS3D_E_UNSUPPORTED;
    }
    if (g.pairlist) {
        if (g.nbt == 1 && p.NCH == 1) return launch_fwd_pairlist<1, 1>(p, grid, g.threads, g.lds, stream);
        if (g.nbt == 1 && p.NCH == 2) return launch_fwd_pairlist<1, 2>(p, grid, g.threads, g.lds, stream);
        if (g.nbt == 2 && p.NCH == 1) return launch_fwd_pairlist<2, 1>(p, grid, g.threads, g.lds, stream);
        if (g.nbt == 2 && p.NCH == 2 && g.pl_rows == PL_ROWS_NARROW) return launch_fwd_pairlist<2, 2, PL_ROWS_NARROW>(p, grid, g.threads, g.lds, stream);
        if (g.nbt == 2 && p.NCH == 2) return launch_fwd_pairlist<2, 2>(p, grid, g.threads, g.lds, stream);
        if (g.nbt == 1 && p.NCH == 3) return launch_fwd_pairlist<1, 3>(p, grid, g.threads, g.lds, stream);
        if (g.nbt == 1 && p.NCH == 4) return launch_fwd_pairlist<1, 4>(p, grid, g.threads, g.lds, stream);
        return MS3D_E_UNSUPPORTED;
    }
    p.RT = g.small ? g.rt : 1;
#define MS3D_BF_NBT(LAUNCH, P_, ...)                                                                                   \
    switch (g.nbt) {                                                                                                   \
        case 2: return LAUNCH<2, ##__VA_ARGS__, P_>(p, grid, g.threads, LDS_, stream);                                \
        case 3: return LAUNCH<3, ##__VA_ARGS__, P_>(p, grid, g.threads, LDS_, stream);                                \
        case 4: return LAUNCH<4, ##__VA_ARGS__, P_>(p, grid, g.threads, LDS_, stream);                                \
        case 5: return LAUNCH<5, ##__VA_ARGS__, P_>(p, grid, g.threads, LDS_, stream);                                \
        case 6: return LAUNCH<6, ##__VA_ARGS__, P_>(p, grid, g.threads, LDS_, stream);                                \
        case 7: return LAUNCH<7, ##__VA_ARGS__, P_>(p, grid, g.threads, LDS_, stream);                                \
        case 8: return LAUNCH<8, ##__VA_ARGS__, P_>(p, grid, g.threads, LDS_, stream);                                \
    }
#define MS3D_BF_P(LAUNCH, ...)                                                                                         \
    if (pieces == 3) { MS3D_BF_NBT(LAUNCH, 3, ##__VA_ARGS__) }                                                         \
    else if (pieces == 2) { MS3D_BF_NBT(LAUNCH, 2, ##__VA_ARGS__) }                                                    \
    else { MS3D_BF_NBT(LAUNCH, 1, ##__VA_ARGS__) }
// ... 72 lines not shown
int ms3d_spconv_wgrad_is_bf16x3(int Vout, int K, int Cin, int Cout, int offset_list) { return wgrad_bf3_ok(Vout, K, Cin, Cout, offset_list != 0) ? 1 : 0; }
int ms3d_spconv_wgrad_is_bf16x3_g(int Vout, int K, int Cin, int Cout, int offset_list, int submanifold)
{
    return wgrad_bf3_ok(Vout, K, Cin, Cout, offset_list != 0, submanifold != 0) ? 1 : 0;
}
int ms3d_spconv_wgrad_is_table_walk(int Vout, int K, int Cin, int Cout, int offset_list)
{
    const bool use_list = offset_list && wgrad_list_cols_ok(K, ms3d_divup(Cout, 16)) && K <= 27 && Cin % 16 == 0 && Cout % 16 == 0;
    return (Vout > 0 && !use_list && !wgrad_bf3_ok(Vout, K, Cin, Cout, use_list) && ms3d_divup(Cout, 16) <= 14) ? 1 : 0;
}
static int wgrad_k1_chunks(int Vout, int K, int Cin, int Cout)
{
    static const int k1_max = [] { const char *e = getenv("MS3D_WGRAD_K1_CHUNKS"); return e ? atoi(e) : 1024; }();
    if (K != 1 || (long)Cin * Cout > 4096 || k1_max <= 0) return 0;
    int c = ms3d_divup(Vout, 128);
    return c > k1_max ? k1_max : c;
}
int ms3d_spconv_wgrad_pieces(int Vout, int K, int Cin, int Cout, int offset_list, int precision)
{
    if (precision < 0 || precision > 2) return MS3D_E_UNSUPPORTED;
    return ms3d_spconv_wgrad_is_bf16x3(Vout, K, Cin, Cout, offset_list) ? 3 - precision : 0;
}

size_t ms3d_spconv_wgrad_ws_floats_p(int Vout, int K, int Cin, int Cout, int precision)
{
    if (precision < 0 || precision > 2) return 0;
    const int k1 = wgrad_k1_chunks(Vout, K, Cin, Cout), rc = ms3d_spconv_wgrad_row_chunks(Vout);
    size_t n = (size_t)(k1 > rc ? k1 : rc) * K * Cin * Cout + 64;
    if (wgrad_bf3_ok(Vout, K, Cin, Cout, false)) {
        const int P = 3 - precision;
        n += (size_t)ms3d_divup(Vout, 32) * ms3d_divup(Cout, 16) * P * 64 * 4 + 8;
        n += (size_t)Vout * Cin * P / 2 + 8;
    }
    return n;
}

size_t ms3d_spconv_wgrad_ws_floats(int Vout, int K, int Cin, int Cout) { return ms3d_spconv_wgrad_ws_floats_p(Vout, K, Cin, Cout, 0); }

int ms3d_spconv_wgrad_row_chunks(int Vout)
{
    static const int max_chunks = [] {
        const char *e = getenv("MS3D_WGRAD_MAX_CHUNKS");
        return e ? atoi(e) : 256;
    }();
    int chunks = ms3d_divup(Vout, 256);
    if (chunks > max_chunks) chunks = max_chunks;
    return chunks < 1 ? 1 : chunks;
}

static int spconv_backward_weight_impl(const float *in, const float *dout, const int *nbr, int Vout, int K, int Cin, int Cout,
                                       float *dW, const float *pre_scale, const float *pre_shift, int pre_relu,
                                       float *partial_ws, const int *ol_kt_start, const int *ol_entries, int *defer_nblk,
                                       ms3d_stream_t stream_, void *defer_launch = nullptr, int precision = 0,
                                       bool submanifold = true);

int ms3d_spconv_backward_weight_p(const float *in, const float *dout, const int *nbr, int Vout, int K, int Cin, int Cout,
                                  float *dW, const float *pre_scale, const float *pre_shift, int pre_relu,
                                  float *partial_ws, const int *ol_kt_start, const int *ol_entries, int precision,
                                  ms3d_stream_t stream_)
{
    if (precision < 0 || precision > 2) return MS3D_E_UNSUPPORTED;
    return spconv_backward_weight_impl(in, dout, nbr, Vout, K, Cin, Cout, dW, pre_scale, pre_shift, pre_relu, partial_ws,
                                       ol_kt_start, ol_entries, nullptr, stream_, nullptr, precision);
}

int ms3d_spconv_backward_weight_g(const float *in, const float *dout, const int *nbr, int Vin, int Vout, int K, int Cin,
                                  int Cout, float *dW, const float *pre_scale, const float *pre_shift, int pre_relu,
                                  float *partial_ws, const int *ol_kt_start, const int *ol_entries, int submanifold,
                                  int precision, ms3d_stream_t stream_)
{
    if (precision < 0 || precision > 2 || Vin < 0) return MS3D_E_UNSUPPORTED;
    if (submanifold && Vin != Vout) return MS3D_E_UNSUPPORTED;
    return spconv_backward_weight_impl(in, dout, nbr, Vout, K, Cin, Cout, dW, pre_scale, pre_shift, pre_relu, partial_ws,
                                       ol_kt_start, ol_entries, nullptr, stream_, nullptr, precision, submanifold != 0);
}

int ms3d_spconv_backward_weight(const float *in, const float *dout, const int *nbr, int Vout, int K, int Cin, int Cout,
                                float *dW, const float *pre_scale, const float *pre_shift, int pre_relu,
                                float *partial_ws, const int *ol_kt_start, const int *ol_entries, ms3d_stream_t stream_)
{
    return spconv_backward_weight_impl(in, dout, nbr, Vout, K, Cin, Cout, dW, pre_scale, pre_shift, pre_relu, partial_ws,
                                       ol_kt_start, ol_entries, nullptr, stream_);
}

static int spconv_backward_weight_impl(const float *in, const float *dout, const int *nbr, int Vout, int K, int Cin, int Cout,
                                       float *dW, const float *pre_scale, const float *pre_shift, int pre_relu,
                                       float *partial_ws, const int *ol_kt_start, const int *ol_entries, int *defer_nblk,
                                       ms3d_stream_t stream_, void *defer_launch, int precision, bool submanifold)
{
    hipStream_t stream = (hipStream_t)stream_;
    const long n = (long)K * Cin * Cout;
    if (defer_nblk) *defer_nblk = 0;
    WgradLaunch *dl = defer_nblk ? static_cast<WgradLaunch *>(defer_launch) : nullptr;
    if (dl) dl->variant = 0;
    if (Vout <= 0) {
        MS3D_CHECK(hipMemsetAsync(dW, 0, sizeof(float) * n, stream));
        return 0;
    }
    WgradArgs p;
    p.in = in; p.dout = dout; p.nbr = nbr; p.partial = partial_ws; p.pre_scale = pre_scale; p.pre_shift = pre_shift;
    p.Vout = Vout; p.K = K; p.Cin = Cin; p.Cout = Cout; p.NBtot = ms3d_divup(Cout, 16); p.pre_relu = pre_relu;
    int chunks = ms3d_spconv_wgrad_row_chunks(Vout);
    static const int wide_chunks = [] { const char *e = getenv("MS3D_WGRAD_WIDE_CHUNKS"); return e ? atoi(e) : 128; }();
    static const int xwide_chunks = [] { const char *e = getenv("MS3D_WGRAD_XWIDE_CHUNKS"); return e ? atoi(e) : 128; }();
    if (n >= 100000 && chunks > wide_chunks) chunks = wide_chunks;
    if (n >= 400000 && chunks > xwide_chunks) chunks = xwide_chunks;
    const bool use_list = ol_kt_start && ol_entries && wgrad_list_cols_ok(K, p.NBtot) && K <= 27 && Cin % 16 == 0 && Cout % 16 == 0;
    p.ol_kt_start = ol_kt_start; p.ol_entries = ol_entries;
    int nblk;
    static const int list_wide_chunks = [] { const char *e = getenv("MS3D_WGRAD_LIST_WIDE_CHUNKS"); return e ? atoi(e) : 64; }();
    static const int nch2 = env_int("MS3D_WGRAD_LIST_NCH2", 1);
    const bool wide2 = nch2 && use_list && K == 27 && p.NBtot == 4 && Cin % 32 == 0 && Cin >= 64;
    if (use_list && ms3d_divup(Cin, 16) >= 3 && chunks > list_wide_chunks) chunks = wide2 ? 2 * list_wide_chunks : list_wide_chunks;
    if (use_list) {
        int shift = 0;
        while ((MS3D_PL_PARTS >> shift) > chunks) shift++;
        p.rows_per_block = shift;
        nblk = MS3D_PL_PARTS >> shift;
    } else {
        if (!wgrad_bf3_ok(Vout, K, Cin, Cout, false, submanifold)) {
            static const int rounds = [] { const char *e = getenv("MS3D_WGRAD_F32_ROUNDS"); return e ? atoi(e) : 1; }();
            const int nbq = p.NBtot;
            const int kg = nbq <= 3 ? (K >= 27 ? 9 : 8) : nbq <= 7 ? 4 : nbq == 8 ? 3 : 2;
            const int yz = ms3d_divup(K, kg) * ms3d_divup(Cin, 16);
            if (rounds > 0) {
                int c = (1024 * rounds) / yz;
                if (c < 4) c = 4;
                if (c < chunks) chunks = c;
            }
            const int k1 = wgrad_k1_chunks(Vout, K, Cin, Cout);
            if (k1 > chunks) chunks = k1;
        }
        p.rows_per_block = ms3d_divup(ms3d_divup(Vout, chunks), 16) * 16;
        nblk = ms3d_divup(Vout, p.rows_per_block);
    }
    const int nb = p.NBtot;
    if (nb > 14) return MS3D_E_UNSUPPORTED;
    int rc;
    if (use_list) {
        const int nbs = nb <= 4 ? nb : ms3d_divup(nb, ms3d_divup(nb, 4));
        const bool two = ms3d_divup(Cin, 16) % 2 == 0 && nbs <= 2;
        rc = nbs == 1 ? (two ? launch_wgrad_offsetlist<1, 2>(p, nblk, stream) : launch_wgrad_offsetlist<1, 1>(p, nblk, stream))
           : nbs == 2 ? (two ? launch_wgrad_offsetlist<2, 2>(p, nblk, stream) : launch_wgrad_offsetlist<2, 1>(p, nblk, stream))
           : nbs == 3 ? launch_wgrad_offsetlist<3, 1>(p, nblk, stream)
                      : (wide2 ? launch_wgrad_offsetlist<4, 2, 1>(p, nblk, stream) : launch_wgrad_offsetlist<4, 1>(p, nblk, stream));
        if (rc) return rc;
        if (defer_nblk) { *defer_nblk = nblk; return 0; }
        launch_wgrad_reduce(partial_ws, nblk, n, dW, stream);
        MS3D_LAUNCH_CHECK();
        return 0;
    }
    if (wgrad_bf3_ok(Vout, K, Cin, Cout, use_list, submanifold)) {
        const int P = 3 - precision;
        float *base = partial_ws + (size_t)ms3d_spconv_wgrad_row_chunks(Vout) * K * Cin * Cout;
        bf16x8 *img = reinterpret_cast<bf16x8 *>((reinterpret_cast<uintptr_t>(base) + 15) & ~(uintptr_t)15);
        const long ntile = ms3d_divup(Vout, 32);
        bf16x8 *xs = img + (size_t)ntile * nb * P * 64;
        const long t1 = ntile * nb * 64, t2 = (long)Vout * (Cin / 8);
        const int nb1 = (int)((t1 + 255) / 256), nb2 = (int)((t2 + 255) / 256);
        if (P == 3)
            wgrad_bf3_operands_kernel<3><<<nb1 + nb2, 256, 0, stream>>>(dout, in, Vout, Cin, Cout, nb, ntile, nb1, pre_scale,
// ... 8 lines not shown
        WgradBf3Args q;
        q.xs = xs; q.dout_img = img; q.nbr = nbr; q.partial = partial_ws; q.Vout = Vout; q.K = K; q.Cin = Cin; q.Cout = Cout;
        q.NBtot = nb;
        {
            const int kg = nb <= 4 ? (nb == 3 ? 14 : 9) : 9;
            const int yz = ms3d_divup(K, kg) * ms3d_divup(Cin, 16);
            static const int rounds = [] { const char *e = getenv("MS3D_WGRAD_BF3_ROUNDS"); return e ? atoi(e) : 2; }();
            int c = (512 * rounds) / yz;
            if (c < 8) c = 8;
            if (c < chunks) chunks = c;
        }
        q.rows_per_block = ms3d_divup(ms3d_divup(Vout, chunks), 32) * 32;
        nblk = ms3d_divup(Vout, q.rows_per_block);
#define MS3D_WG_BF(P_)                                                                                                 \
    (nb == 3 ? launch_wgrad_bf3<14, 3, 1, P_>(q, nblk, stream) : nb == 4 ? launch_wgrad_bf3<9, 4, 1, P_>(q, nblk, stream)   \
     : nb <= 6 ? launch_wgrad_bf3<9, 3, 2, P_>(q, nblk, stream) : launch_wgrad_bf3<9, 4, 2, P_>(q, nblk, stream))
        rc = P == 3 ? MS3D_WG_BF(3) : P == 2 ? MS3D_WG_BF(2) : MS3D_WG_BF(1);
#undef MS3D_WG_BF
        if (rc) return rc;
        if (defer_nblk) { *defer_nblk = nblk; return 0; }
        launch_wgrad_reduce(partial_ws, nblk, n, dW, stream);
        MS3D_LAUNCH_CHECK();
        return 0;
    }
    if (nb == 1) rc = (K >= 27) ? launch_wgrad<9, 1>(p, nblk, stream, dl) : launch_wgrad<8, 1>(p, nblk, stream, dl);
    else if (nb == 2) rc = (K >= 27) ? launch_wgrad<9, 2>(p, nblk, stream, dl) : launch_wgrad<8, 2>(p, nblk, stream, dl);
    else if (nb == 3) rc = (K >= 27) ? launch_wgrad<9, 3>(p, nblk, stream, dl) : launch_wgrad<8, 3>(p, nblk, stream, dl);
    else if (nb == 4) rc = launch_wgrad<4, 4>(p, nblk, stream, dl);
    else if (nb == 5) rc = launch_wgrad<4, 5>(p, nblk, stream, dl);
    else if (nb == 6) rc = launch_wgrad<4, 6>(p, nblk, stream, dl);
    else if (nb == 7) rc = launch_wgrad<4, 7>(p, nblk, stream, dl);
    else if (nb == 8) rc = launch_wgrad<3, 8>(p, nblk, stream, dl);
    else if (nb <= 10) rc = launch_wgrad<2, 10>(p, nblk, stream, dl);
    else if (nb <= 12) rc = launch_wgrad<2, 12>(p, nblk, stream, dl);
    else rc = launch_wgrad<2, 14>(p, nblk, stream, dl);
    if (rc) return rc;
    if (defer_nblk) { *defer_nblk = nblk; return 0; }
    launch_wgrad_reduce(partial_ws, nblk, n, dW, stream);
    MS3D_LAUNCH_CHECK();
    return 0;
}

size_t ms3d_spconv_wgrad_launch_bytes(void) { return 128; }

int ms3d_spconv_wgrad_multi(const void *descs, int n_desc, int total_blocks, int variant, ms3d_stream_t stream_)
{
    hipStream_t stream = (hipStream_t)stream_;
    if (n_desc <= 0 || total_blocks <= 0) return 0;
    switch (variant) {
#define MS3D_WM(KG, NBT) case KG * 100 + NBT: return launch_wgrad_multi<KG, NBT>(descs, n_desc, total_blocks, stream);
        MS3D_WM(9, 1) MS3D_WM(8, 1) MS3D_WM(9, 2) MS3D_WM(8, 2) MS3D_WM(9, 3) MS3D_WM(8, 3) MS3D_WM(4, 4) MS3D_WM(4, 5)
        MS3D_WM(4, 6) MS3D_WM(4, 7) MS3D_WM(3, 8) MS3D_WM(2, 10) MS3D_WM(2, 12) MS3D_WM(2, 14)
#undef MS3D_WM
    }
    return MS3D_E_UNSUPPORTED;
}

int ms3d_wgrad_reduce_blocks(long n, const float *slabs, const float *dW, int *wide)
{
    const bool w = n >= 32768 && (n & 3) == 0 && ((uintptr_t)slabs & 15) == 0 && ((uintptr_t)dW & 15) == 0;
    if (wide) *wide = w ? 1 : 0;
    return w ? ms3d_divup(n / 4, 64) : ms3d_divup(n, 16);
}

int ms3d_wgrad_reduce_multi(const void *descs, int n_desc, int total_blocks, ms3d_stream_t stream)
{
    if (n_desc <= 0 || total_blocks <= 0) return 0;
    wgrad_reduce_multi_kernel<<<total_blocks, 256, 0, (hipStream_t)stream>>>(static_cast<const WgradReduceDesc *>(descs),
                                                                           n_desc);
    MS3D_LAUNCH_CHECK();
    return 0;
}

int ms3d_bn_stats(const float *x, long V, int C, float eps, float momentum, const float *gamma, const float *beta,
                  float *running_mean, float *running_var, float *mean, float *invstd, float *scale, float *shift,
                  float *partial_ws, int partial_rows, ms3d_stream_t stream_)
{
    hipStream_t stream = (hipStream_t)stream_;
    if (V <= 0) return MS3D_E_UNSUPPORTED;
    int nblk = (int)((V + 255) / 256);
    if (nblk > partial_rows) nblk = partial_rows;
    if (nblk < 1) nblk = 1;
    const int rows_per_block = (int)((V + nblk - 1) / nblk);
    const int rc = launch_bn_partial_stats(x, V, C, partial_ws, nblk, rows_per_block, stream);
    if (rc) return rc;
    bn_finalize_stats_kernel<<<ms3d_divup(C, 16), 1024, 0, stream>>>(partial_ws, nblk, C, V, eps, momentum, gamma, beta,
                                                                  running_mean, running_var, mean, invstd, scale, shift);
    MS3D_LAUNCH_CHECK();
    return 0;
}

int ms3d_column_sum(const float *x, long V, int C, float *partial_ws, int partial_rows, float *out2c, ms3d_stream_t stream_)
{
    hipStream_t stream = (hipStream_t)stream_;
    if (V <= 0) {
        MS3D_CHECK(hipMemsetAsync(out2c, 0, sizeof(float) * 2 * C, stream));
        return 0;
    }
    int nblk = (int)((V + 1023) / 1024);
    if (nblk > partial_rows) nblk = partial_rows;
    if (nblk < 1) nblk = 1;
    const int rows_per_block = (int)((V + nblk - 1) / nblk);
    const int rc = launch_bn_partial_stats(x, V, C, partial_ws, nblk, rows_per_block, stream);
    if (rc) return rc;
    return ms3d_reduce_partials(partial_ws, nblk, 2 * C, out2c, stream_);
}
// ... 119 lines not shown
    int rc = W ? prep_weights_pair_impl(W, K, Cin, Cout, mirror_bwd, wf, wft, wf + nwf, wft + nwf, aux_kind, (hipStream_t)stream) : 0;
    if (rc) return rc;
    if (ev_start) MS3D_CHECK(hipEventRecord((hipEvent_t)ev_start, (hipStream_t)stream));
    rc = spconv_forward_impl(x, wf, nbr_fwd, Vout, K, Cin, Cout, y, pre_scale, pre_shift, pre_relu, residual, nullptr,
                             nullptr, nullptr, nullptr, nullptr, stat_partial, stat_partial != nullptr, bias, pl_tile_start,
                             pl_entries, wf + nwf, aux_kind, stream);
    if (ev_stop) MS3D_CHECK(hipEventRecord((hipEvent_t)ev_stop, (hipStream_t)stream));
    return rc;
}

int ms3d_spconv_layer_forward(const float *x, const float *W, const int *nbr_fwd, int Vout, int K, int Cin, int Cout,
                              int mirror_bwd, const float *pre_scale, const float *pre_shift, int pre_relu,
                              const float *residual, const float *bias, float *wf_buf, float *y, float *stat_partial,
                              const int *pl_tile_start, const int *pl_entries, void *ev_start, void *ev_stop,
                              ms3d_stream_t stream)
{
    return ms3d_spconv_layer_forward_p(x, W, nbr_fwd, Vout, K, Cin, Cout, mirror_bwd, pre_scale, pre_shift, pre_relu, residual,
                                       bias, wf_buf, y, stat_partial, pl_tile_start, pl_entries, ev_start, ev_stop, 0, stream);
}

void *ms3d_event_create(void)
{
    hipEvent_t e = nullptr;
    return hipEventCreate(&e) == hipSuccess ? (void *)e : nullptr;
}
void ms3d_event_destroy(void *e) { if (e) (void)hipEventDestroy((hipEvent_t)e); }
int ms3d_event_record(void *e, ms3d_stream_t stream) { return (int)hipEventRecord((hipEvent_t)e, (hipStream_t)stream); }
float ms3d_event_elapsed_ms(void *start, void *stop)
{
    float ms = -1.f;
    if (hipEventSynchronize((hipEvent_t)stop) != hipSuccess) return -1.f;
    if (hipEventElapsedTime(&ms, (hipEvent_t)start, (hipEvent_t)stop) != hipSuccess) return -1.f;
    return ms;
}

static hipEvent_t order_event()
{
    constexpr int MAX_DEV = 16, POOL = 256;
    static hipEvent_t pool[MAX_DEV][POOL];
    static bool ready[MAX_DEV][POOL];
    static unsigned next[MAX_DEV];
    static std::mutex lock;
    int dev = 0;
    if (hipGetDevice(&dev) != hipSuccess || dev < 0 || dev >= MAX_DEV) return nullptr;
    std::lock_guard<std::mutex> guard(lock);
    const unsigned i = next[dev]++ & (POOL - 1);
    if (!ready[dev][i]) {
        if (hipEventCreateWithFlags(&pool[dev][i], hipEventDisableTiming) != hipSuccess) return nullptr;
        ready[dev][i] = true;
    }
    return pool[dev][i];
}

int ms3d_spconv_layer_backward_g(const float *x, const float *dy, const float *wf_buf, const int *nbr_fwd,
                                 const int *nbr_bwd, int Vin, int Vout, int K, int Cin, int Cout, const float *scale,
                                 const float *shift, const float *mean, const float *invstd, int pre_relu, int training,
                                 int need_dx, float *dx, const float *dx_add, float *dgb, float *dW, float *ws,
                                 const int *ol_fwd_kt_start, const int *ol_fwd_entries, const int *pl_bwd_tile_start,
                                 const int *pl_bwd_entries, void *ev_start, void *ev_stop, void *ev_wg_start, void *ev_wg_stop,
                                 float *ws_wgrad, ms3d_stream_t wgrad_stream, int join, float *wgrad_slabs,
                                 int *wgrad_deferred_nblk, void *wgrad_deferred_launch, int precision, int submanifold,
                                 ms3d_stream_t stream)
{
    if (submanifold && Vin != Vout) return MS3D_E_UNSUPPORTED;
    const size_t nwf = ms3d_spconv_wf_floats(K, Cin, Cout);
    const float *wft = wf_buf + 3 * nwf, *wfts = wf_buf + 4 * nwf;
    const int aux_kind = ms3d_spconv_aux_kind_p(K, Cin, Cout, precision);
    if (aux_kind == MS3D_E_UNSUPPORTED) return MS3D_E_UNSUPPORTED;
    const bool bn = scale != nullptr;
    int rc;
    hipStream_t main = (hipStream_t)stream, side = wgrad_stream ? (hipStream_t)wgrad_stream : main;
    float *slabs;
    hipEvent_t done = nullptr;
    auto run_wgrad = [&]() -> int {
        if (ev_wg_start) MS3D_CHECK(hipEventRecord((hipEvent_t)ev_wg_start, side));
        int r = spconv_backward_weight_impl(x, dy, nbr_fwd, Vout, K, Cin, Cout, dW, scale, shift, pre_relu,
                                            wgrad_slabs ? wgrad_slabs : slabs, ol_fwd_kt_start, ol_fwd_entries,
                                            wgrad_slabs ? wgrad_deferred_nblk : nullptr, (ms3d_stream_t)side,
                                            (wgrad_slabs && !ev_wg_start) ? wgrad_deferred_launch : nullptr, precision,
                                            submanifold != 0);
        if (ev_wg_stop) MS3D_CHECK(hipEventRecord((hipEvent_t)ev_wg_stop, side));
        return r;
    };
    if (side != main) {
        if (!ws_wgrad) return MS3D_E_WORKSPACE;
        slabs = ws_wgrad;
        hipEvent_t ready = order_event();
        done = order_event();
        if (!ready || !done) return MS3D_E_INTERNAL;
        MS3D_CHECK(hipEventRecord(ready, main));
        MS3D_CHECK(hipStreamWaitEvent(side, ready, 0));
        rc = run_wgrad();
        if (rc) return rc;
        MS3D_CHECK(hipEventRecord(done, side));
    }
    if (ev_start && (need_dx || bn)) MS3D_CHECK(hipEventRecord((hipEvent_t)ev_start, main));
    if (need_dx || bn) {
        if (!bn) {
            rc = spconv_forward_impl(dy, wft, nbr_bwd, Vin, K, Cout, Cin, dx, nullptr, nullptr, 0, dx_add, nullptr, nullptr,
                                     nullptr, nullptr, nullptr, nullptr, 0, nullptr, pl_bwd_tile_start, pl_bwd_entries, wfts,
                                     aux_kind, stream);
            if (rc) return rc;
            if (ev_stop) MS3D_CHECK(hipEventRecord((hipEvent_t)ev_stop, main));
            ev_stop = nullptr;
        } else {
            if (!pre_relu) return MS3D_E_UNSUPPORTED;
            const int nparts = ms3d_spconv_partial_blocks(Vin, K, Cout, Cin, (pl_bwd_tile_start && pl_bwd_entries)
                                                                                 ? ms3d_kmap_pairlist_rows_of(pl_bwd_tile_start) : 0);
            float *partial = ws;
            rc = spconv_forward_impl(dy, wft, nbr_bwd, Vin, K, Cout, Cin, dx, nullptr, nullptr, 0, nullptr, x, scale, shift,
                                     mean, invstd, partial, 0, nullptr, pl_bwd_tile_start, pl_bwd_entries, wfts, aux_kind,
                                     stream);
            if (rc) return rc;
            if (ev_stop) MS3D_CHECK(hipEventRecord((hipEvent_t)ev_stop, main));
            ev_stop = nullptr;
            if (need_dx && training) {
                rc = ms3d_bn_bwd_reduce_apply(partial, nparts, dx, x, Vin, Cin, scale, mean, invstd, dx_add, dx, dgb, stream);
                if (rc) return rc;
            } else {
                rc = ms3d_reduce_partials(partial, nparts, 2 * Cin, dgb, stream);
                if (rc) return rc;
            }
            if (need_dx && !training) {
                {
                    if (dx_add) return MS3D_E_UNSUPPORTED;
                    rc = ms3d_bn_apply(dx, Vin, Cin, scale, nullptr, 0, dx, stream);
                }
                if (rc) return rc;
            }
        }
    }
    if (side != main) {
        if (join) MS3D_CHECK(hipStreamWaitEvent(main, done, 0));
        return 0;
    }
    const int pb0 = ms3d_spconv_partial_blocks(Vin, K, Cout, Cin, 0), pb1 = ms3d_spconv_partial_blocks(Vin, K, Cout, Cin, 1);
    const int pb2 = ms3d_spconv_partial_blocks(Vin, K, Cout, Cin, ms3d_spconv_pairlist_rows_dense(Vin, K, Cout, Cin));
    slabs = ws + (size_t)(pb0 > pb1 ? (pb0 > pb2 ? pb0 : pb2) : (pb1 > pb2 ? pb1 : pb2)) * 2 * Cin;
    return run_wgrad();
}

int ms3d_spconv_layer_backward_p(const float *x, const float *dy, const float *wf_buf, const int *nbr_fwd,
                                 const int *nbr_bwd, int Vin, int Vout, int K, int Cin, int Cout, const float *scale,
                                 const float *shift, const float *mean, const float *invstd, int pre_relu, int training,
                                 int need_dx, float *dx, const float *dx_add, float *dgb, float *dW, float *ws,
                                 const int *ol_fwd_kt_start, const int *ol_fwd_entries, const int *pl_bwd_tile_start,
                                 const int *pl_bwd_entries, void *ev_start, void *ev_stop, void *ev_wg_start, void *ev_wg_stop,
                                 float *ws_wgrad, ms3d_stream_t wgrad_stream, int join, float *wgrad_slabs,
                                 int *wgrad_deferred_nblk, void *wgrad_deferred_launch, int precision, ms3d_stream_t stream)
{
    return ms3d_spconv_layer_backward_g(x, dy, wf_buf, nbr_fwd, nbr_bwd, Vin, Vout, K, Cin, Cout, scale, shift, mean, invstd,
                                        pre_relu, training, need_dx, dx, dx_add, dgb, dW, ws, ol_fwd_kt_start, ol_fwd_entries,
                                        pl_bwd_tile_start, pl_bwd_entries, ev_start, ev_stop, ev_wg_start, ev_wg_stop, ws_wgrad,
                                        wgrad_stream, join, wgrad_slabs, wgrad_deferred_nblk, wgrad_deferred_launch, precision,
                                        K == 27 && Vin == Vout, stream);
}

int ms3d_spconv_layer_backward(const float *x, const float *dy, const float *wf_buf, const int *nbr_fwd,
                               const int *nbr_bwd, int Vin, int Vout, int K, int Cin, int Cout, const float *scale,
                               const float *shift, const float *mean, const float *invstd, int pre_relu, int training,
                               int need_dx, float *dx, const float *dx_add, float *dgb, float *dW, float *ws,
                               const int *ol_fwd_kt_start, const int *ol_fwd_entries, const int *pl_bwd_tile_start,
                               const int *pl_bwd_entries, void *ev_start, void *ev_stop, void *ev_wg_start, void *ev_wg_stop,
                               float *ws_wgrad, ms3d_stream_t wgrad_stream, int join, float *wgrad_slabs,
                               int *wgrad_deferred_nblk, void *wgrad_deferred_launch, ms3d_stream_t stream)
{
    return ms3d_spconv_layer_backward_p(x, dy, wf_buf, nbr_fwd, nbr_bwd, Vin, Vout, K, Cin, Cout, scale, shift, mean, invstd,
                                        pre_relu, training, need_dx, dx, dx_add, dgb, dW, ws, ol_fwd_kt_start, ol_fwd_entries,
                                        pl_bwd_tile_start, pl_bwd_entries, ev_start, ev_stop, ev_wg_start, ev_wg_stop, ws_wgrad,
                                        wgrad_stream, join, wgrad_slabs, wgrad_deferred_nblk, wgrad_deferred_launch, 0, stream);
}

}
```

minsu3d_amd/csrc_host/ms3d_host.cpp:

```cpp
#include <torch/extension.h>
#include <c10/hip/HIPStream.h>

#include <tuple>

#include "../../include/minsu3d_hip.h"

namespace {

inline ms3d_stream_t cur() { return (ms3d_stream_t)c10::hip::getCurrentHIPStream().stream(); }

inline void check(int rc, const char *what)
{
    TORCH_CHECK(rc == 0, what, " failed with code ", rc, " (libminsu3d_hip.so; there is no CPU fallback)");
}

using OptT = c10::optional<at::Tensor>;

inline const float *fptr(const OptT &t)
{
    if (!t.has_value() || !t->defined()) return nullptr;
    TORCH_CHECK(t->is_contiguous() && t->scalar_type() == at::kFloat, "expected a contiguous float32 tensor");
    return t->data_ptr<float>();
}
inline const int *iptr(const OptT &t)
{
    if (!t.has_value() || !t->defined()) return nullptr;
    TORCH_CHECK(t->is_contiguous() && t->scalar_type() == at::kInt, "expected a contiguous int32 tensor");
    return t->data_ptr<int>();
}

}

std::tuple<at::Tensor, OptT> conv_layer_forward(const at::Tensor &x, const OptT &W, const at::Tensor &nbr_fwd, int64_t vout,
                                                int64_t K, int64_t cin, int64_t cout, bool mirror_bwd, const OptT &pre_scale,
                                                const OptT &pre_shift, bool pre_relu, const OptT &residual, const OptT &bias,
                                                at::Tensor wf_buf, int64_t nparts , const OptT &pl_tile_start,
                                                const OptT &pl_entries, int64_t ev_start, int64_t ev_stop, int64_t precision)
{
    TORCH_CHECK(x.is_cuda() && x.is_contiguous() && x.scalar_type() == at::kFloat, "x: contiguous float32 device tensor");
    at::Tensor y = at::empty({vout, cout}, x.options());
    OptT stats;
    if (nparts > 0) stats = at::empty({nparts, 2, cout}, x.options());
    check(ms3d_spconv_layer_forward_p(x.data_ptr<float>(), fptr(W), nbr_fwd.data_ptr<int>(), (int)vout, (int)K, (int)cin,
                                      (int)cout, mirror_bwd ? 1 : 0, fptr(pre_scale), fptr(pre_shift), pre_relu ? 1 : 0,
                                      fptr(residual), fptr(bias), wf_buf.data_ptr<float>(), y.data_ptr<float>(),
                                      stats.has_value() ? stats->data_ptr<float>() : nullptr, iptr(pl_tile_start),
                                      iptr(pl_entries), (void *)ev_start, (void *)ev_stop, (int)precision, cur()),
          "ms3d_spconv_layer_forward_p");
    return {y, stats};
}

std::tuple<OptT, OptT, at::Tensor, OptT, int64_t, py::bytes> conv_layer_backward(
    const at::Tensor &x, const at::Tensor &dy, const at::Tensor &wf_buf, const at::Tensor &nbr_fwd, const at::Tensor &nbr_bwd,
    int64_t vin, int64_t vout, int64_t K, int64_t cin, int64_t cout, const OptT &scale, const OptT &shift, const OptT &mean,
    const OptT &invstd, bool relu, bool training, bool need_dx, const OptT &dx_add, at::Tensor ws, const OptT &ol_kt_start,
    const OptT &ol_entries, const OptT &pl_tile_start, const OptT &pl_entries, int64_t ev0, int64_t ev1, int64_t ev2,
    int64_t ev3, int64_t defer_floats, bool defer_launch, int64_t precision, int64_t submanifold)
{
    if (submanifold < 0) submanifold = (K == 27 && vin == vout) ? 1 : 0;
    TORCH_CHECK(x.is_cuda() && x.is_contiguous() && dy.is_contiguous(), "x / dy: contiguous device tensors");
    const bool has_bn = scale.has_value() && scale->defined();
    OptT dx, dgb, slabs;
    if (need_dx || has_bn) dx = at::empty({vin, cin}, x.options());
    if (has_bn) dgb = at::empty({2, cin}, x.options());
    at::Tensor dW = at::empty({K, cin, cout}, x.options());
    int nblk = 0;
    alignas(16) unsigned char launch[128];
    reinterpret_cast<int *>(launch)[4] = 0;
    if (defer_floats > 0) slabs = at::empty({defer_floats}, x.options());
    check(ms3d_spconv_layer_backward_g(
              x.data_ptr<float>(), dy.data_ptr<float>(), wf_buf.data_ptr<float>(), nbr_fwd.data_ptr<int>(),
              nbr_bwd.data_ptr<int>(), (int)vin, (int)vout, (int)K, (int)cin, (int)cout, fptr(scale), fptr(shift), fptr(mean),
              fptr(invstd), (has_bn && relu) ? 1 : 0, (has_bn && training) ? 1 : 0, need_dx ? 1 : 0,
              dx.has_value() ? dx->data_ptr<float>() : nullptr, need_dx ? fptr(dx_add) : nullptr,
              dgb.has_value() ? dgb->data_ptr<float>() : nullptr, dW.data_ptr<float>(), (float *)ws.data_ptr(), iptr(ol_kt_start),
              iptr(ol_entries), iptr(pl_tile_start), iptr(pl_entries), (void *)ev0, (void *)ev1, (void *)ev2, (void *)ev3,
              nullptr, nullptr, 0, slabs.has_value() ? slabs->data_ptr<float>() : nullptr,
              slabs.has_value() ? &nblk : nullptr, (slabs.has_value() && defer_launch) ? (void *)launch : nullptr,
              (int)precision, (int)submanifold, cur()),
          "ms3d_spconv_layer_backward_g");
    if (!need_dx) dx = c10::nullopt;
    const bool described = reinterpret_cast<int *>(launch)[4] != 0;
    return {dx, dgb, dW, slabs, (int64_t)nblk, py::bytes(reinterpret_cast<const char *>(launch), described ? 128 : 0)};
}

at::Tensor bn_finalize(const at::Tensor &partial, int64_t V, double eps, double momentum, const OptT &gamma, const OptT &beta,
                       OptT running_mean, OptT running_var)
{
    const int64_t C = partial.size(2);
    at::Tensor outs = at::empty({4, C}, partial.options());
    float *o = outs.data_ptr<float>();
    check(ms3d_bn_finalize(partial.data_ptr<float>(), (int)partial.size(0), (long)V, (int)C, (float)eps, (float)momentum,
                           fptr(gamma), fptr(beta),
                           running_mean.has_value() && running_mean->defined() ? running_mean->data_ptr<float>() : nullptr,
                           running_var.has_value() && running_var->defined() ? running_var->data_ptr<float>() : nullptr, o,
                           o + C, o + 2 * C, o + 3 * C, cur()),
          "ms3d_bn_finalize");
    return outs;
}

std::tuple<at::Tensor, at::Tensor, OptT, at::Tensor, at::Tensor> res_block_forward(
    const at::Tensor &x, const at::Tensor &stats_in, at::Tensor wf1, at::Tensor wf2, const at::Tensor &nbr, int64_t V, int64_t C,
    const OptT &pl_tile_start, const OptT &pl_entries, int64_t nparts, bool want_stats, const OptT &g0, const OptT &b0,
    OptT rm0, OptT rv0, double eps0, double mom0, const OptT &g1, const OptT &b1, OptT rm1, OptT rv1, double eps1, double mom1,
    int64_t precision)
{
    TORCH_CHECK(x.is_cuda() && x.is_contiguous() && x.scalar_type() == at::kFloat && x.size(1) == C, "x: contiguous f32 [V, C]");
    TORCH_CHECK(stats_in.dim() == 3 && stats_in.size(2) == C && stats_in.is_contiguous(), "stats_in: [nparts, 2, C]");
    auto rs = [](OptT &t) -> float * { return t.has_value() && t->defined() ? t->data_ptr<float>() : nullptr; };
    const ms3d_stream_t st = cur();
    at::Tensor bn0 = at::empty({4, C}, x.options()), bn1 = at::empty({4, C}, x.options());
    float *o0 = bn0.data_ptr<float>(), *o1 = bn1.data_ptr<float>();
    check(ms3d_bn_finalize(stats_in.data_ptr<float>(), (int)stats_in.size(0), (long)V, (int)C, (float)eps0, (float)mom0, fptr(g0),
                           fptr(b0), rs(rm0), rs(rv0), o0, o0 + C, o0 + 2 * C, o0 + 3 * C, st), "ms3d_bn_finalize");
    at::Tensor y1 = at::empty({V, C}, x.options()), st1 = at::empty({nparts, 2, C}, x.options());
    check(ms3d_spconv_layer_forward_p(x.data_ptr<float>(), nullptr, nbr.data_ptr<int>(), (int)V, 27, (int)C, (int)C, 1, o0 + 2 * C,
                                      o0 + 3 * C, 1, nullptr, nullptr, wf1.data_ptr<float>(), y1.data_ptr<float>(),
                                      st1.data_ptr<float>(), iptr(pl_tile_start), iptr(pl_entries), nullptr, nullptr,
                                      (int)precision, st),
          "ms3d_spconv_layer_forward_p");
    check(ms3d_bn_finalize(st1.data_ptr<float>(), (int)nparts, (long)V, (int)C, (float)eps1, (float)mom1, fptr(g1), fptr(b1),
                           rs(rm1), rs(rv1), o1, o1 + C, o1 + 2 * C, o1 + 3 * C, st), "ms3d_bn_finalize");
    at::Tensor y2 = at::empty({V, C}, x.options());
    OptT st2;
    if (want_stats) st2 = at::empty({nparts, 2, C}, x.options());
    check(ms3d_spconv_layer_forward_p(y1.data_ptr<float>(), nullptr, nbr.data_ptr<int>(), (int)V, 27, (int)C, (int)C, 1, o1 + 2 * C,
                                      o1 + 3 * C, 1, x.data_ptr<float>(), nullptr, wf2.data_ptr<float>(), y2.data_ptr<float>(),
                                      st2.has_value() ? st2->data_ptr<float>() : nullptr, iptr(pl_tile_start), iptr(pl_entries),
                                      nullptr, nullptr, (int)precision, st),
          "ms3d_spconv_layer_forward_p");
    return {y1, y2, st2, bn0, bn1};
}

at::Tensor gather_rows(const at::Tensor &x, const at::Tensor &idx)
{
    TORCH_CHECK(x.is_cuda() && x.is_contiguous() && idx.is_contiguous() && idx.scalar_type() == at::kLong &&
                x.scalar_type() == at::kFloat && x.dim() == 2, "gather_rows: f32 [V, C] rows and an int64 index");
    at::Tensor out = at::empty({idx.numel(), x.size(1)}, x.options());
    check(ms3d_gather_rows(x.data_ptr<float>(), (const long long *)idx.data_ptr<int64_t>(), (long)idx.numel(), (int)x.size(1),
                           out.data_ptr<float>(), cur()), "ms3d_gather_rows");
    return out;
}

PYBIND11_MODULE(TORCH_EXTENSION_NAME, m)
{
    m.doc() = "host-side fast path of the minsu3d_amd sparse-voxel engine (pybind over libminsu3d_hip.so's C ABI)";
    m.def("conv_layer_forward", &conv_layer_forward);
    m.def("conv_layer_forward",
          [](const at::Tensor &x, const OptT &W, const at::Tensor &nbr_fwd, int64_t vout, int64_t K, int64_t cin, int64_t cout,
             bool mirror_bwd, const OptT &pre_scale, const OptT &pre_shift, bool pre_relu, const OptT &residual,
             const OptT &bias, at::Tensor wf_buf, int64_t nparts, const OptT &pl_tile_start, const OptT &pl_entries,
             int64_t ev_start, int64_t ev_stop) {
              return conv_layer_forward(x, W, nbr_fwd, vout, K, cin, cout, mirror_bwd, pre_scale, pre_shift, pre_relu, residual,
                                        bias, wf_buf, nparts, pl_tile_start, pl_entries, ev_start, ev_stop, 0);
          });
    m.def("conv_layer_backward_g", &conv_layer_backward);
    m.def("conv_layer_backward",
          [](const at::Tensor &x, const at::Tensor &dy, const at::Tensor &wf_buf, const at::Tensor &nbr_fwd,
             const at::Tensor &nbr_bwd, int64_t vin, int64_t vout, int64_t K, int64_t cin, int64_t cout, const OptT &scale,
             const OptT &shift, const OptT &mean, const OptT &invstd, bool relu, bool training, bool need_dx,
             const OptT &dx_add, at::Tensor ws, const OptT &ol_kt_start, const OptT &ol_entries, const OptT &pl_tile_start,
             const OptT &pl_entries, int64_t ev0, int64_t ev1, int64_t ev2, int64_t ev3, int64_t defer_floats,
             bool defer_launch, int64_t precision) {
              return conv_layer_backward(x, dy, wf_buf, nbr_fwd, nbr_bwd, vin, vout, K, cin, cout, scale, shift, mean, invstd,
                                         relu, training, need_dx, dx_add, ws, ol_kt_start, ol_entries, pl_tile_start,
                                         pl_entries, ev0, ev1, ev2, ev3, defer_floats, defer_launch, precision, -1);
          });
    m.def("conv_layer_backward",
          [](const at::Tensor &x, const at::Tensor &dy, const at::Tensor &wf_buf, const at::Tensor &nbr_fwd,
             const at::Tensor &nbr_bwd, int64_t vin, int64_t vout, int64_t K, int64_t cin, int64_t cout, const OptT &scale,
             const OptT &shift, const OptT &mean, const OptT &invstd, bool relu, bool training, bool need_dx,
             const OptT &dx_add, at::Tensor ws, const OptT &ol_kt_start, const OptT &ol_entries, const OptT &pl_tile_start,
             const OptT &pl_entries, int64_t ev0, int64_t ev1, int64_t ev2, int64_t ev3, int64_t defer_floats,
             bool defer_launch) {
              return conv_layer_backward(x, dy, wf_buf, nbr_fwd, nbr_bwd, vin, vout, K, cin, cout, scale, shift, mean, invstd,
                                         relu, training, need_dx, dx_add, ws, ol_kt_start, ol_entries, pl_tile_start,
                                         pl_entries, ev0, ev1, ev2, ev3, defer_floats, defer_launch, 0, -1);
          });
    m.def("bn_finalize", &bn_finalize);
    m.def("gather_rows", &gather_rows);
    m.def("res_block_forward", &res_block_forward);
    m.def("res_block_forward",
          [](const at::Tensor &x, const at::Tensor &stats_in, at::Tensor wf1, at::Tensor wf2, const at::Tensor &nbr, int64_t V,
             int64_t C, const OptT &pl_tile_start, const OptT &pl_entries, int64_t nparts, bool want_stats, const OptT &g0,
             const OptT &b0, OptT rm0, OptT rv0, double eps0, double mom0, const OptT &g1, const OptT &b1, OptT rm1, OptT rv1,
             double eps1, double mom1) {
              return res_block_forward(x, stats_in, wf1, wf2, nbr, V, C, pl_tile_start, pl_entries, nparts, want_stats, g0, b0,
                                       rm0, rv0, eps0, mom0, g1, b1, rm1, rv1, eps1, mom1, 0);
          });
}
```

Baseline: 199.0 scenes/sec.

## Fold inner BN-backward apply into next conv's gather prologue in residual blocks

```diff
diff --git a/include/minsu3d_hip.h b/include/minsu3d_hip.h
--- a/include/minsu3d_hip.h
+++ b/include/minsu3d_hip.h
@@ -248,6 +248,17 @@
                                  void *ev_wg_stop, float *ws_wgrad, ms3d_stream_t wgrad_stream, int join,
                                  float *wgrad_slabs, int *wgrad_deferred_nblk, void *wgrad_deferred_launch, int precision,
                                  int submanifold, ms3d_stream_t stream);
+int ms3d_spconv_bn_fold_wanted(int V, int K, int Cin, int Cout, int offset_list, int pl_rows_bwd, int precision);
+int ms3d_spconv_layer_backward_f(const float *x, const float *dy, const float *wf_buf, const int *nbr_fwd,
+                                 const int *nbr_bwd, int Vin, int Vout, int K, int Cin, int Cout, const float *scale,
+                                 const float *shift, const float *mean, const float *invstd, int pre_relu, int training,
+                                 int need_dx, float *dx, const float *dx_add, float *dgb, float *dW, float *ws,
+                                 const int *ol_fwd_kt_start, const int *ol_fwd_entries, const int *pl_bwd_tile_start,
+                                 const int *pl_bwd_entries, void *ev_start, void *ev_stop, void *ev_wg_start,
+                                 void *ev_wg_stop, float *ws_wgrad, ms3d_stream_t wgrad_stream, int join,
+                                 float *wgrad_slabs, int *wgrad_deferred_nblk, void *wgrad_deferred_launch, int precision,
+                                 int submanifold, int defer_apply, const float *fold_x, const float *fold_tab,
+                                 ms3d_stream_t stream);
 size_t ms3d_spconv_wgrad_launch_bytes(void);
 int ms3d_spconv_wgrad_is_table_walk(int Vout, int K, int Cin, int Cout, int offset_list);
 int ms3d_spconv_wgrad_multi(const void *descs, int n_desc, int total_blocks, int variant, ms3d_stream_t stream);
diff --git a/minsu3d_amd/MinkowskiEngine/functional.py b/minsu3d_amd/MinkowskiEngine/functional.py
--- a/minsu3d_amd/MinkowskiEngine/functional.py
+++ b/minsu3d_amd/MinkowskiEngine/functional.py
@@ -168,6 +168,11 @@
         return dx, dW.view_as(W), dgamma, dbeta, d_res, None, None, None, None, db
 
 
+def _fold_inner(be, spec, V, cin, cout, prec):
+    fn = getattr(be, "bn_fold_wanted", None)
+    return bool(fn is not None and fn(spec.nbr_fwd, spec.nbr_bwd, V, 27, cin, cout, **_pk(prec)))
+
+
 class ResBlockFn(torch.autograd.Function):
 
     @staticmethod
@@ -213,9 +218,13 @@
         dy = dy.contiguous()
         V, c0, c1 = spec.vout, spec.cin, spec.cout
         e2 = {"defer": _queue(ctx.defer[1])} if _queue(ctx.defer[1]) is not None else {}
+        e1 = {"defer": _queue(ctx.defer[0])} if _queue(ctx.defer[0]) is not None else {}
+        if _fold_inner(be, spec, V, c0, c1, ctx.prec):
+            e2["defer_apply"] = True
         dx1, dgb1, dW2 = be.conv_layer_backward(y1, dy, ctx.wf[1], spec.nbr_fwd, spec.nbr_bwd, V, V, 27, c1, c1, ctx.bn[1], True, **e2,
                                                 **_pk(ctx.prec))
-        e1 = {"defer": _queue(ctx.defer[0])} if _queue(ctx.defer[0]) is not None else {}
+        if "defer_apply" in e2:
+            e1["fold"] = (y1, dgb1)
         dx, dgb0, dW1 = be.conv_layer_backward(x, dx1, ctx.wf[0], spec.nbr_fwd, spec.nbr_bwd, V, V, 27, c0, c1, ctx.bn[0],
                                                ctx.needs_input_grad[0], dx_add=dy, **e1, **_pk(ctx.prec))
         return dx, dW1.view_as(W1), dgb0[1], dgb0[0], dW2.view_as(W2), dgb1[1], dgb1[0], None, None, None, None, None
@@ -267,11 +276,12 @@
         dy = dy.contiguous()
         V, cin, cout = spec.vout, spec.cin, spec.cout
         ex = lambda d: dict({"defer": _queue(d)} if _queue(d) is not None else {}, **_pk(ctx.prec))
+        fold = _fold_inner(be, spec, V, cin, cout, ctx.prec)
         dx1, dgb1, dW2 = be.conv_layer_backward(y1, dy, ctx.wf[2], spec.nbr_fwd, spec.nbr_bwd, V, V, 27, cout, cout, ctx.bn[1],
-                                                True, **ex(ctx.defer[2]))
+                                                True, **ex(ctx.defer[2]), **({"defer_apply": True} if fold else {}))
         need = ctx.needs_input_grad[0]
         dxb, dgb0, dW1 = be.conv_layer_backward(x, dx1, ctx.wf[1], spec.nbr_fwd, spec.nbr_bwd, V, V, 27, cin, cout, ctx.bn[0],
-                                                need, **ex(ctx.defer[1]))
+                                                need, **ex(ctx.defer[1]), **({"fold": (y1, dgb1)} if fold else {}))
         dx, _, dWd = be.conv_layer_backward(x, dy, ctx.wf[0], ctx.ident, ctx.ident, V, V, 1, cin, cout, None, need,
                                             **({"dx_add": dxb} if need else {}), **ex(ctx.defer[0]))
         return dx, dWd.view_as(Wd), dW1.view_as(W1), dgb0[1], dgb0[0], dW2.view_as(W2), dgb1[1], dgb1[0], None, None, None, None, None
diff --git a/minsu3d_amd/backend.py b/minsu3d_amd/backend.py
--- a/minsu3d_amd/backend.py
+++ b/minsu3d_amd/backend.py
@@ -159,6 +159,7 @@
         self.weight_token = 0
         self.matmul_precision_aware = True
         self._prep_table = None
+        self.counters = {}
 
     @staticmethod
     def _dev(t):
@@ -501,6 +502,8 @@
                                     [_VP, _VP, _I, _VP, _VP, _VP, _I, _VP],
     "ms3d_spconv_layer_backward_g": [_VP] * 5 + [_I] * 5 + [_VP] * 4 + [_I] * 3 + [_VP] * 5 + [_VP] * 4 + [_VP] * 4 +
                                     [_VP, _VP, _I, _VP, _VP, _VP, _I, _I, _VP],
+    "ms3d_spconv_layer_backward_f": [_VP] * 5 + [_I] * 5 + [_VP] * 4 + [_I] * 3 + [_VP] * 5 + [_VP] * 4 + [_VP] * 4 +
+                                    [_VP, _VP, _I, _VP, _VP, _VP, _I, _I, _I, _VP, _VP, _VP],
     "ms3d_bn_finalize": [_VP, _I, C.c_long, _I, C.c_float, C.c_float] + [_VP] * 4 + [_VP] * 4 + [_VP],
 }
 
@@ -1182,8 +1185,24 @@
             int(precision))
         return y1, y2, st2, o0.unbind(0), o1.unbind(0)
 
+    def bn_fold_wanted(self, nbr_fwd, nbr_bwd, V, K, cin, cout, precision=0):
+        if not hasattr(self.lib, "ms3d_spconv_bn_fold_wanted"):
+            return False
+        plf = self.offsetlist(nbr_fwd, K, V)
+        plb = self.pairlist(nbr_bwd, K, V, cout, cin)
+        cache = self.__dict__.setdefault("_fold_cache", {})
+        key = (os.environ.get("MS3D_BN_FOLD"), V, K, cin, cout, plf[0] is not None, self._pl_rows(plb), int(precision))
+        v = cache.get(key)
+        if v is None:
+            v = cache[key] = bool(self.lib.ms3d_spconv_bn_fold_wanted(int(V), int(K), int(cin), int(cout), int(key[5]),
+                                                                      int(key[6]), int(precision)))
+        return v
+
     def conv_layer_backward(self, x, dy, wf_buf, nbr_fwd, nbr_bwd, vin, vout, K, cin, cout, bn, need_dx, dx_add=None,
-                            defer=None, join_now=False, precision=0, submanifold=None):
+                            defer=None, join_now=False, precision=0, submanifold=None, defer_apply=False, fold=None):
+        lazy = bool(defer_apply) or fold is not None
+        if bn is not None and bn["training"] and need_dx and not defer_apply:
+            self.counters["bn_bwd_apply"] = self.counters.get("bn_bwd_apply", 0) + 1
         sub = -1 if submanifold is None else int(bool(submanifold))
         x = self._dev(x); dy = self._dev(dy)
         dev = x.device
@@ -1205,22 +1224,26 @@
             timing = timer.records.pop()[0][1:] + (nbr_fwd,)
             timer._pool.extend((ev2, ev3))
             ev2 = ev3 = None
-        if self.ext is not None and mode == 0:
+        if self.ext is not None and mode == 0 and (not lazy or hasattr(self.ext, "conv_layer_backward_f")):
             evs = [(e.value or 0) if e is not None else 0 for e in (ev0, ev1, ev2, ev3)]
-            dx, dgb, dW, slabs, nblk, desc = (self.ext.conv_layer_backward_g if sub >= 0 else self.ext.conv_layer_backward)(
+            entry = self.ext.conv_layer_backward_f if lazy else \
+                (self.ext.conv_layer_backward_g if sub >= 0 else self.ext.conv_layer_backward)
+            tail = (sub if sub >= 0 else int(K == 27 and vin == vout), bool(defer_apply), fold[0] if fold else None,
+                    fold[1] if fold else None) if lazy else ((sub,) if sub >= 0 else ())
+            dx, dgb, dW, slabs, nblk, desc = entry(
                 x, dy, wf_buf, nbr_fwd, nbr_bwd, vin, vout, K, cin, cout,
                 bn["scale"] if has_bn else None, bn["shift"] if has_bn else None, bn["mean"] if has_bn else None,
                 bn["invstd"] if has_bn else None, bool(has_bn and bn["relu"]), bool(has_bn and bn["training"]), bool(need_dx),
                 _f32(dx_add) if (dx_add is not None and need_dx) else None, ws, plf[0], plf[1], plb[0], plb[1], *evs,
                 self._geom("ms3d_spconv_wgrad_ws_floats", vout, K, cin, cout) if defer is not None else 0, batch,
-                int(precision), *((sub,) if sub >= 0 else ()))
+                int(precision), *tail)
             if desc:
-                defer.add_launch(desc, (x, dy, nbr_fwd, bn, slabs, dW), timing)
+                defer.add_launch(desc, (x, dy, nbr_fwd, bn, slabs, dW, fold), timing)
             if nblk > 0:
                 defer.add(slabs, dW, K * cin * cout, nblk)
             return dx, dgb, dW
         dx = torch.empty((vin, cin), dtype=torch.float32, device=dev) if want_dx else None
-        dgb = torch.empty((2, cin), dtype=torch.float32, device=dev) if has_bn else None
+        dgb = torch.empty((5 if defer_apply else 2, cin), dtype=torch.float32, device=dev) if has_bn else None
         dW = torch.empty((K, cin, cout), dtype=torch.float32, device=dev)
         side = wgrad_stream(dev) if mode else None
         ws2 = None
@@ -1237,7 +1260,9 @@
             slabs = torch.empty(self._geom("ms3d_spconv_wgrad_ws_floats", vout, K, cin, cout), dtype=torch.float32, device=dev)
             n_defer = self._defer_n_addr
         launch = (C.c_char * 128)() if (batch and slabs is not None) else None
-        _lib.check(self._fast("ms3d_spconv_layer_backward_g")(
+        fold_args = (int(bool(defer_apply)), _p(fold[0] if fold else None), _p(fold[1] if fold else None)) if lazy else ()
+        entry = "ms3d_spconv_layer_backward_f" if lazy else "ms3d_spconv_layer_backward_g"
+        _lib.check(self._fast(entry)(
             _p(x), _p(dy), _p(wf_buf), _p(nbr_fwd), _p(nbr_bwd), int(vin), int(vout), int(K),
             int(cin), int(cout), _p(bn["scale"] if has_bn else None), _p(bn["shift"] if has_bn else None),
             _p(bn["mean"] if has_bn else None), _p(bn["invstd"] if has_bn else None),
@@ -1246,10 +1271,12 @@
             _p(plb[1]), ev0, ev1, ev2, ev3, _p(ws2), side.cuda_stream if side is not None else None,
             int(mode == 1 or (mode == 2 and join_now) or (mode == 3 and defer is None)), _p(slabs), n_defer,
             C.addressof(launch) if launch is not None else None, int(precision),
-            sub if sub >= 0 else int(K == 27 and vin == vout), _lib.stream_handle()),
-            "ms3d_spconv_layer_backward_g")
+            sub if sub >= 0 else int(K == 27 and vin == vout), *fold_args, _lib.stream_handle()),
+            entry)
         if launch is not None and np.frombuffer(launch, dtype=np.int32, count=6)[4] != 0:
-            defer.add_launch(bytes(launch), (x, dy, nbr_fwd, bn, slabs, dW), timing)
+            defer.add_launch(bytes(launch), (x, dy, nbr_fwd, bn, slabs, dW, fold), timing)
+        if fold is not None and mode in (2, 3):
+            fold[0].record_stream(side); fold[1].record_stream(side)
         if slabs is not None and self._defer_n.value > 0:
             defer.add(slabs, dW, K * cin * cout, self._defer_n.value)
         if mode == 2:
diff --git a/minsu3d_amd/csrc/spconv.hip b/minsu3d_amd/csrc/spconv.hip
--- a/minsu3d_amd/csrc/spconv.hip
+++ b/minsu3d_amd/csrc/spconv.hip
@@ -59,7 +59,15 @@
     float *ws_slabs;
     unsigned *ws_cnt;
     int ws_ng, ws_kg, ws_R, ws_tpp;
+    const float *fold_x;
+    const float *fold_tab;
+    float fold_invV;
 };
+
+__device__ __forceinline__ float bn_bwd_dx(float g, float x, float sc, float mu, float is, float a1, float a2, float invV)
+{
+    return sc * (g - a1 * invV - ((x - mu) * is) * a2 * invV);
+}
 
 __device__ __forceinline__ long stream_slot(long o, int NBtot)
 {
@@ -305,7 +313,7 @@
     }
 }
 
-template <int NBT, bool ALIGNED, bool DIRECT = false, int GSZ = ((DIRECT || NBT < 5) ? OG : (NBT < 7 ? 7 : 6))>
+template <int NBT, bool ALIGNED, bool DIRECT = false, int GSZ = ((DIRECT || NBT < 5) ? OG : (NBT < 7 ? 7 : 6)), bool FOLD = false>
 __device__ __forceinline__ void accumulate_offsets(const ConvArgs &p, const float *__restrict__ sW, int k_lo, int k_hi,
                                                    int kw0, int my_row, int q, int nb0, f32x4 (&acc)[NBT])
 {
@@ -318,8 +326,17 @@
         bool any[GSZ];
 #pragma unroll
         for (int u = 0; u < GSZ; u++) any[u] = __ballot(idx[u] >= 0) != 0ull;
-        auto fetch = [&](int ch, f32x4 (&a)[GSZ], f32x4 &sc, f32x4 &sh) {
+        static_assert(!FOLD || ALIGNED, "the folded prologue reads whole 16-byte channel groups");
+        constexpr int XG = FOLD ? GSZ : 1;
+        auto fetch = [&](int ch, f32x4 (&a)[GSZ], f32x4 &sc, f32x4 &sh, f32x4 (&xr)[XG], f32x4 (&ft)[5]) {
             const int c0 = 16 * ch + 4 * q;
+            if constexpr (FOLD) {
+#pragma unroll
+                for (int u = 0; u < GSZ; u++)
+                    xr[u] = *reinterpret_cast<const f32x4 *>(p.fold_x + (size_t)max(idx[u], 0) * p.Cin + c0);
+#pragma unroll
+                for (int i = 0; i < 5; i++) ft[i] = *reinterpret_cast<const f32x4 *>(p.fold_tab + (size_t)i * p.Cin + c0);
+            }
 #pragma unroll
             for (int u = 0; u < GSZ; u++) {
                 const float *row = p.in + (size_t)max(idx[u], 0) * p.Cin + c0;
@@ -343,18 +360,31 @@
                 }
             }
         };
-        f32x4 a_next[GSZ], sc_next = {0.f, 0.f, 0.f, 0.f}, sh_next = sc_next;
-        if (DIRECT) fetch(0, a_next, sc_next, sh_next);
+        f32x4 a_next[GSZ], sc_next = {0.f, 0.f, 0.f, 0.f}, sh_next = sc_next, x_next[XG], ft_next[5];
+        if (DIRECT) fetch(0, a_next, sc_next, sh_next, x_next, ft_next);
         for (int ch = 0; ch < p.NCH; ch++) {
-            f32x4 a[GSZ], s = {0.f, 0.f, 0.f, 0.f}, b = s;
+            f32x4 a[GSZ], s = {0.f, 0.f, 0.f, 0.f}, b = s, xr[XG], ft[5];
             if (DIRECT) {
 #pragma unroll
                 for (int u = 0; u < GSZ; u++) a[u] = a_next[u];
                 s = sc_next;
                 b = sh_next;
-                if (ch + 1 < p.NCH) fetch(ch + 1 + opaque0, a_next, sc_next, sh_next);
+                if constexpr (FOLD) {
+#pragma unroll
+                    for (int u = 0; u < GSZ; u++) xr[u] = x_next[u];
+#pragma unroll
+                    for (int i = 0; i < 5; i++) ft[i] = ft_next[i];
+                }
+                if (ch + 1 < p.NCH) fetch(ch + 1 + opaque0, a_next, sc_next, sh_next, x_next, ft_next);
             } else {
-                fetch(ch, a, s, b);
+                fetch(ch, a, s, b, xr, ft);
+            }
+            if constexpr (FOLD) {
+#pragma unroll
+                for (int u = 0; u < GSZ; u++)
+#pragma unroll
+                    for (int t = 0; t < 4; t++)
+                        a[u][t] = bn_bwd_dx(a[u][t], xr[u][t], ft[2][t], ft[3][t], ft[4][t], ft[0][t], ft[1][t], p.fold_invV);
             }
             if (p.pre_scale) {
 #pragma unroll
@@ -755,7 +785,7 @@
     return 0;
 }
 
-template <int NBT, bool ALIGNED>
+template <int NBT, bool ALIGNED, bool FOLD = false>
 __global__ __launch_bounds__(256) void spconv_fwd_small_kernel(ConvArgs p)
 {
     extern __shared__ float lds[];
@@ -775,8 +805,8 @@
 #pragma unroll
         for (int nb = 0; nb < NBT; nb++) acc[nb] = (f32x4){0.f, 0.f, 0.f, 0.f};
         const int k_lo = wave_id() * OG, k_hi = min(p.K, k_lo + OG);
-        if (p.K == 1 && (p.k1_path & 2)) { if (k_lo < k_hi) accumulate_k1<NBT, ALIGNED, true>(p, nullptr, my_row, q, nb0, acc); }
-        else if (k_lo < k_hi) accumulate_offsets<NBT, ALIGNED, true>(p, nullptr, k_lo, k_hi, 0, my_row, q, nb0, acc);
+        if (!FOLD && p.K == 1 && (p.k1_path & 2)) { if (k_lo < k_hi) accumulate_k1<NBT, ALIGNED, true>(p, nullptr, my_row, q, nb0, acc); }
+        else if (k_lo < k_hi) accumulate_offsets<NBT, ALIGNED, true, OG, FOLD>(p, nullptr, k_lo, k_hi, 0, my_row, q, nb0, acc);
         if (tt > 0) __syncthreads();
         if (wave_id() > 0) {
 #pragma unroll
@@ -1086,7 +1116,10 @@
 {
     const size_t need = ((size_t)(threads / 64 - 1) * NBT * 256 + ((p.bn_x || p.out_stats) ? stat_slot_floats(NBT) : 0)) * sizeof(float) + 16;
     if (lds > need) lds = need;
-    if (aligned)
+    if (p.fold_x) {
+        if (!aligned || p.K == 1) return MS3D_E_UNSUPPORTED;
+        spconv_fwd_small_kernel<NBT, true, true><<<grid, threads, lds, stream>>>(p);
+    } else if (aligned)
         spconv_fwd_small_kernel<NBT, true><<<grid, threads, lds, stream>>>(p);
     else
         spconv_fwd_small_kernel<NBT, false><<<grid, threads, lds, stream>>>(p);
@@ -1905,11 +1938,20 @@
     const float *pre_scale;
     const float *pre_shift;
     int Vout, K, Cin, Cout, NBtot, rows_per_block, pre_relu;
-    const int *ol_kt_start;
-    const int *ol_entries;
+    int fold;
+    union {
+        struct {
+            const int *ol_kt_start;
+            const int *ol_entries;
+        };
+        struct {
+            const float *fold_x;
+            const float *fold_tab;
+        };
+    };
 };
 
-template <int KG, int NBT>
+template <int KG, int NBT, bool FOLD = false>
 __device__ __forceinline__ void wgrad_body(const WgradArgs &p, const int bx, const int by, const int bz, float *s_red)
 {
     const int l = lane_id(), q = l >> 4, cl = l & 15;
@@ -1925,6 +1967,16 @@
     for (int a = 0; a < KG; a++)
 #pragma unroll
         for (int b = 0; b < NBT; b++) acc[a][b] = (f32x4){0.f, 0.f, 0.f, 0.f};
+    float ft[FOLD ? NBT : 1][5];
+    const float fold_invV = 1.f / (float)p.Vout;
+    if constexpr (FOLD) {
+#pragma unroll
+        for (int nb = 0; nb < NBT; nb++) {
+            const int j = 16 * nb + cl, js = j < p.Cout ? j : 0;
+#pragma unroll
+            for (int i = 0; i < 5; i++) ft[nb][i] = p.fold_tab[(size_t)i * p.Cout + js];
+        }
+    }
 
     const int r_begin = bx * p.rows_per_block;
     const int r_end = min(p.Vout, r_begin + p.rows_per_block);
@@ -1941,7 +1993,10 @@
 #pragma unroll
             for (int nb = 0; nb < NBT; nb++) {
                 const int j = 16 * nb + cl;
-                const float v = p.dout[(size_t)safe_row * p.Cout + (j < p.Cout ? j : 0)];
+                float v = p.dout[(size_t)safe_row * p.Cout + (j < p.Cout ? j : 0)];
+                if constexpr (FOLD)
+                    v = bn_bwd_dx(v, p.fold_x[(size_t)safe_row * p.Cout + (j < p.Cout ? j : 0)], ft[nb][2], ft[nb][3], ft[nb][4],
+                                  ft[nb][0], ft[nb][1], fold_invV);
                 b[h][nb] = __int_as_float(__float_as_int(v) & ((ok[h] && j < p.Cout) ? -1 : 0));
             }
 #pragma unroll
@@ -1994,11 +2049,11 @@
     }
 }
 
-template <int KG, int NBT>
+template <int KG, int NBT, bool FOLD = false>
 __global__ __launch_bounds__(256) void spconv_wgrad_kernel(WgradArgs p)
 {
     __shared__ float s_red[4 * NBT * 256];
-    wgrad_body<KG, NBT>(p, blockIdx.x, blockIdx.y, blockIdx.z, s_red);
+    wgrad_body<KG, NBT, FOLD>(p, blockIdx.x, blockIdx.y, blockIdx.z, s_red);
 }
 
 struct WgradLaunch {
@@ -2010,8 +2065,9 @@
     WgradArgs p;
 };
 static_assert(sizeof(WgradLaunch) <= 128, "ms3d_spconv_wgrad_launch_bytes() promises 128");
-
-template <int KG, int NBT>
+constexpr int WGRAD_FOLD_VARIANT = 10000;
+
+template <int KG, int NBT, bool FOLD = false>
 __global__ __launch_bounds__(256) void spconv_wgrad_multi_kernel(const unsigned char *__restrict__ descs, int n_desc)
 {
     __shared__ float s_red[4 * NBT * 256];
@@ -2023,7 +2079,7 @@
     }
     const WgradLaunch d = *reinterpret_cast<const WgradLaunch *>(descs + 128 * (size_t)lo);
     const int local = blk - d.block_begin;
-    wgrad_body<KG, NBT>(d.p, local % d.gx, (local / d.gx) % d.gy, local / (d.gx * d.gy), s_red);
+    wgrad_body<KG, NBT, FOLD>(d.p, local % d.gx, (local / d.gx) % d.gy, local / (d.gx * d.gy), s_red);
 }
 
 template <int P>
@@ -2373,20 +2429,21 @@
     if (defer) {
         defer->block_begin = 0;
         defer->gx = grid.x; defer->gy = grid.y; defer->gz = grid.z;
-        defer->variant = KG * 100 + NBT;
+        defer->variant = KG * 100 + NBT + (p.fold ? WGRAD_FOLD_VARIANT : 0);
         defer->nblk = nblk_rows;
         defer->p = p;
         return 0;
     }
-    spconv_wgrad_kernel<KG, NBT><<<grid, 256, 0, stream>>>(p);
+    if (p.fold) spconv_wgrad_kernel<KG, NBT, true><<<grid, 256, 0, stream>>>(p);
+    else spconv_wgrad_kernel<KG, NBT><<<grid, 256, 0, stream>>>(p);
     MS3D_LAUNCH_CHECK();
     return 0;
 }
 
-template <int KG, int NBT>
+template <int KG, int NBT, bool FOLD = false>
 int launch_wgrad_multi(const void *descs, int n_desc, int total_blocks, hipStream_t stream)
 {
-    spconv_wgrad_multi_kernel<KG, NBT><<<total_blocks, 256, 0, stream>>>(static_cast<const unsigned char *>(descs), n_desc);
+    spconv_wgrad_multi_kernel<KG, NBT, FOLD><<<total_blocks, 256, 0, stream>>>(static_cast<const unsigned char *>(descs), n_desc);
     MS3D_LAUNCH_CHECK();
     return 0;
 }
@@ -2851,6 +2908,30 @@
         for (int i = 0; i < 16; i++) t += s_sum[i][threadIdx.x];
         out[col] = (float)t;
     }
+}
+
+__global__ __launch_bounds__(1024) void reduce_partial_fold_kernel(const float *__restrict__ partial, int nparts, int C,
+                                                                   const float *__restrict__ scale, const float *__restrict__ mean,
+                                                                   const float *__restrict__ invstd, float *__restrict__ tab)
+{
+    __shared__ double s_sum[16][17];
+    const int n = 2 * C;
+    const int col = blockIdx.x * 16 + (threadIdx.x & 15), lane_p = threadIdx.x >> 4;
+    double s = 0.0;
+    if (col < n)
+        for (int p = lane_p; p < nparts; p += 64) s += (double)partial[(size_t)p * n + col];
+    s += __shfl_xor(s, 16, 64);
+    s += __shfl_xor(s, 32, 64);
+    if ((threadIdx.x & 63) < 16) s_sum[threadIdx.x >> 6][threadIdx.x & 15] = s;
+    __syncthreads();
+    if (threadIdx.x < 16 && col < n) {
+        double t = 0.0;
+#pragma unroll
+        for (int i = 0; i < 16; i++) t += s_sum[i][threadIdx.x];
+        tab[col] = (float)t;
+    }
+    for (int t = blockIdx.x * 1024 + threadIdx.x; t < 3 * C; t += gridDim.x * 1024)
+        tab[n + t] = t < C ? scale[t] : (t < n ? mean[t - C] : invstd[t - n]);
 }
 
 struct BnBwdState {
@@ -3150,6 +3231,7 @@
 {
     return pairstream_layer_ok(K, Cin, Cout) && Vout >= pairlist_min_rows() && Vout <= (1 << 22);
 }
+constexpr int BN_FOLD_MAX_ROWS = 0;
 constexpr int SMALL_TILES = 1100;
 FwdGeom fwd_geometry(int Vout, int K, int Cin, int Cout, bool with_bn_partial, int pl_rows)
 {
@@ -3298,6 +3380,11 @@
     g.ok = g.G >= 1 && g.nbt >= 1 && g.nbt <= MAX_NBT;
     return g;
 }
+bool fwd_takes_small_f32(const FwdGeom &g, int K, int Cin, int Cout, bool bf_image)
+{
+    if (!g.ok || g.ws || !g.small) return false;
+    return !(bf_image && (g.rt > 1 || (bf3_dims_ok(K, Cin, Cout) && g.nbt >= 2)));
+}
 }
 
 extern "C" {
@@ -3348,7 +3435,8 @@
                                const float *residual, const float *bn_x, const float *bn_scale, const float *bn_shift,
                                const float *bn_mean, const float *bn_invstd, float *bn_partial, int out_stats,
                                const float *bias, const int *pl_tile_start, const int *pl_entries, const float *wf_aux,
-                               int aux_kind, ms3d_stream_t stream_);
+                               int aux_kind, ms3d_stream_t stream_, const float *fold_x = nullptr,
+                               const float *fold_tab = nullptr);
 
 int ms3d_spconv_forward(const float *in, const float *wf, const int *nbr, int Vout, int K, int Cin, int Cout,
                         float *out, const float *pre_scale, const float *pre_shift, int pre_relu,
@@ -3367,11 +3455,12 @@
                                const float *residual, const float *bn_x, const float *bn_scale, const float *bn_shift,
                                const float *bn_mean, const float *bn_invstd, float *bn_partial, int out_stats,
                                const float *bias, const int *pl_tile_start, const int *pl_entries, const float *wf_stream,
-                               int aux_kind, ms3d_stream_t stream_)
+                               int aux_kind, ms3d_stream_t stream_, const float *fold_x, const float *fold_tab)
 {
     hipStream_t stream = (hipStream_t)stream_;
     if (Vout <= 0) return 0;
     ConvArgs p;
+    p.fold_x = fold_x; p.fold_tab = fold_tab; p.fold_invV = 1.f / (float)Vout;
     p.bias = bias;
     p.wfs = nullptr;
     p.wfb = nullptr;
@@ -3393,6 +3482,7 @@
     p.G = g.G;
     dim3 grid(g.nblk, g.ny);
     const bool aligned = (Cin % 16 == 0);
+    if (fold_x && !(fold_tab && aligned && K > 1 && fwd_takes_small_f32(g, K, Cin, Cout, pieces && wf_stream))) return MS3D_E_UNSUPPORTED;
     p.ws_slabs = nullptr; p.ws_cnt = nullptr; p.ws_ng = p.ws_kg = p.ws_R = p.ws_tpp = 0;
     if (g.ws) {
         const int units = g.ws_R * g.ny;
@@ -3571,7 +3661,7 @@
                                        float *dW, const float *pre_scale, const float *pre_shift, int pre_relu,
                                        float *partial_ws, const int *ol_kt_start, const int *ol_entries, int *defer_nblk,
                                        ms3d_stream_t stream_, void *defer_launch = nullptr, int precision = 0,
-                                       bool submanifold = true);
+                                       bool submanifold = true, const float *fold_x = nullptr, const float *fold_tab = nullptr);
 
 int ms3d_spconv_backward_weight_p(const float *in, const float *dout, const int *nbr, int Vout, int K, int Cin, int Cout,
                                   float *dW, const float *pre_scale, const float *pre_shift, int pre_relu,
@@ -3605,7 +3695,8 @@
 static int spconv_backward_weight_impl(const float *in, const float *dout, const int *nbr, int Vout, int K, int Cin, int Cout,
                                        float *dW, const float *pre_scale, const float *pre_shift, int pre_relu,
                                        float *partial_ws, const int *ol_kt_start, const int *ol_entries, int *defer_nblk,
-                                       ms3d_stream_t stream_, void *defer_launch, int precision, bool submanifold)
+                                       ms3d_stream_t stream_, void *defer_launch, int precision, bool submanifold,
+                                       const float *fold_x, const float *fold_tab)
 {
     hipStream_t stream = (hipStream_t)stream_;
     const long n = (long)K * Cin * Cout;
@@ -3625,7 +3716,12 @@
     if (n >= 100000 && chunks > wide_chunks) chunks = wide_chunks;
     if (n >= 400000 && chunks > xwide_chunks) chunks = xwide_chunks;
     const bool use_list = ol_kt_start && ol_entries && wgrad_list_cols_ok(K, p.NBtot) && K <= 27 && Cin % 16 == 0 && Cout % 16 == 0;
+    p.fold = 0;
     p.ol_kt_start = ol_kt_start; p.ol_entries = ol_entries;
+    if (fold_x) {
+        if (!fold_tab || !submanifold || use_list || wgrad_bf3_ok(Vout, K, Cin, Cout, use_list, submanifold)) return MS3D_E_UNSUPPORTED;
+        p.fold = 1; p.fold_x = fold_x; p.fold_tab = fold_tab;
+    }
     int nblk;
     static const int list_wide_chunks = [] { const char *e = getenv("MS3D_WGRAD_LIST_WIDE_CHUNKS"); return e ? atoi(e) : 64; }();
     static const int nch2 = env_int("MS3D_WGRAD_LIST_NCH2", 1);
@@ -3740,6 +3836,10 @@
         MS3D_WM(9, 1) MS3D_WM(8, 1) MS3D_WM(9, 2) MS3D_WM(8, 2) MS3D_WM(9, 3) MS3D_WM(8, 3) MS3D_WM(4, 4) MS3D_WM(4, 5)
         MS3D_WM(4, 6) MS3D_WM(4, 7) MS3D_WM(3, 8) MS3D_WM(2, 10) MS3D_WM(2, 12) MS3D_WM(2, 14)
 #undef MS3D_WM
+#define MS3D_WM(KG, NBT) case WGRAD_FOLD_VARIANT + KG * 100 + NBT: return launch_wgrad_multi<KG, NBT, true>(descs, n_desc, total_blocks, stream);
+        MS3D_WM(9, 1) MS3D_WM(8, 1) MS3D_WM(9, 2) MS3D_WM(8, 2) MS3D_WM(9, 3) MS3D_WM(8, 3) MS3D_WM(4, 4) MS3D_WM(4, 5)
+        MS3D_WM(4, 6) MS3D_WM(4, 7) MS3D_WM(3, 8) MS3D_WM(2, 10) MS3D_WM(2, 12) MS3D_WM(2, 14)
+#undef MS3D_WM
     }
     return MS3D_E_UNSUPPORTED;
 }
@@ -3965,7 +4065,7 @@
     return pool[dev][i];
 }
 
-int ms3d_spconv_layer_backward_g(const float *x, const float *dy, const float *wf_buf, const int *nbr_fwd,
+int ms3d_spconv_layer_backward_f(const float *x, const float *dy, const float *wf_buf, const int *nbr_fwd,
                                  const int *nbr_bwd, int Vin, int Vout, int K, int Cin, int Cout, const float *scale,
                                  const float *shift, const float *mean, const float *invstd, int pre_relu, int training,
                                  int need_dx, float *dx, const float *dx_add, float *dgb, float *dW, float *ws,
@@ -3973,9 +4073,11 @@
                                  const int *pl_bwd_entries, void *ev_start, void *ev_stop, void *ev_wg_start, void *ev_wg_stop,
                                  float *ws_wgrad, ms3d_stream_t wgrad_stream, int join, float *wgrad_slabs,
                                  int *wgrad_deferred_nblk, void *wgrad_deferred_launch, int precision, int submanifold,
-                                 ms3d_stream_t stream)
+                                 int defer_apply, const float *fold_x, const float *fold_tab, ms3d_stream_t stream)
 {
     if (submanifold && Vin != Vout) return MS3D_E_UNSUPPORTED;
+    if (defer_apply && !(scale && pre_relu && training && need_dx && !dx_add)) return MS3D_E_UNSUPPORTED;
+    if ((fold_x != nullptr) != (fold_tab != nullptr) || (fold_x && !(submanifold && K > 1))) return MS3D_E_UNSUPPORTED;
     const size_t nwf = ms3d_spconv_wf_floats(K, Cin, Cout);
     const float *wft = wf_buf + 3 * nwf, *wfts = wf_buf + 4 * nwf;
     const int aux_kind = ms3d_spconv_aux_kind_p(K, Cin, Cout, precision);
@@ -3991,7 +4093,7 @@
                                             wgrad_slabs ? wgrad_slabs : slabs, ol_fwd_kt_start, ol_fwd_entries,
                                             wgrad_slabs ? wgrad_deferred_nblk : nullptr, (ms3d_stream_t)side,
                                             (wgrad_slabs && !ev_wg_start) ? wgrad_deferred_launch : nullptr, precision,
-                                            submanifold != 0);
+                                            submanifold != 0, fold_x, fold_tab);
         if (ev_wg_stop) MS3D_CHECK(hipEventRecord((hipEvent_t)ev_wg_stop, side));
         return r;
     };
@@ -4012,7 +4114,7 @@
         if (!bn) {
             rc = spconv_forward_impl(dy, wft, nbr_bwd, Vin, K, Cout, Cin, dx, nullptr, nullptr, 0, dx_add, nullptr, nullptr,
                                      nullptr, nullptr, nullptr, nullptr, 0, nullptr, pl_bwd_tile_start, pl_bwd_entries, wfts,
-                                     aux_kind, stream);
+                                     aux_kind, stream, fold_x, fold_tab);
             if (rc) return rc;
             if (ev_stop) MS3D_CHECK(hipEventRecord((hipEvent_t)ev_stop, main));
             ev_stop = nullptr;
@@ -4023,18 +4125,21 @@
             float *partial = ws;
             rc = spconv_forward_impl(dy, wft, nbr_bwd, Vin, K, Cout, Cin, dx, nullptr, nullptr, 0, nullptr, x, scale, shift,
                                      mean, invstd, partial, 0, nullptr, pl_bwd_tile_start, pl_bwd_entries, wfts, aux_kind,
-                                     stream);
+                                     stream, fold_x, fold_tab);
             if (rc) return rc;
             if (ev_stop) MS3D_CHECK(hipEventRecord((hipEvent_t)ev_stop, main));
             ev_stop = nullptr;
-            if (need_dx && training) {
+            if (defer_apply) {
+                reduce_partial_fold_kernel<<<ms3d_divup(2 * Cin, 16), 1024, 0, main>>>(partial, nparts, Cin, scale, mean, invstd, dgb);
+                MS3D_LAUNCH_CHECK();
+            } else if (need_dx && training) {
                 rc = ms3d_bn_bwd_reduce_apply(partial, nparts, dx, x, Vin, Cin, scale, mean, invstd, dx_add, dx, dgb, stream);
                 if (rc) return rc;
             } else {
                 rc = ms3d_reduce_partials(partial, nparts, 2 * Cin, dgb, stream);
                 if (rc) return rc;
             }
-            if (need_dx && !training) {
+            if (need_dx && !training && !defer_apply) {
                 {
                     if (dx_add) return MS3D_E_UNSUPPORTED;
                     rc = ms3d_bn_apply(dx, Vin, Cin, scale, nullptr, 0, dx, stream);
@@ -4051,6 +4156,37 @@
     const int pb2 = ms3d_spconv_partial_blocks(Vin, K, Cout, Cin, ms3d_spconv_pairlist_rows_dense(Vin, K, Cout, Cin));
     slabs = ws + (size_t)(pb0 > pb1 ? (pb0 > pb2 ? pb0 : pb2) : (pb1 > pb2 ? pb1 : pb2)) * 2 * Cin;
     return run_wgrad();
+}
+
+int ms3d_spconv_layer_backward_g(const float *x, const float *dy, const float *wf_buf, const int *nbr_fwd,
+                                 const int *nbr_bwd, int Vin, int Vout, int K, int Cin, int Cout, const float *scale,
+                                 const float *shift, const float *mean, const float *invstd, int pre_relu, int training,
+                                 int need_dx, float *dx, const float *dx_add, float *dgb, float *dW, float *ws,
+                                 const int *ol_fwd_kt_start, const int *ol_fwd_entries, const int *pl_bwd_tile_start,
+                                 const int *pl_bwd_entries, void *ev_start, void *ev_stop, void *ev_wg_start, void *ev_wg_stop,
+                                 float *ws_wgrad, ms3d_stream_t wgrad_stream, int join, float *wgrad_slabs,
+                                 int *wgrad_deferred_nblk, void *wgrad_deferred_launch, int precision, int submanifold,
+                                 ms3d_stream_t stream)
+{
+    return ms3d_spconv_layer_backward_f(x, dy, wf_buf, nbr_fwd, nbr_bwd, Vin, Vout, K, Cin, Cout, scale, shift, mean, invstd,
+                                        pre_relu, training, need_dx, dx, dx_add, dgb, dW, ws, ol_fwd_kt_start, ol_fwd_entries,
+                                        pl_bwd_tile_start, pl_bwd_entries, ev_start, ev_stop, ev_wg_start, ev_wg_stop, ws_wgrad,
+                                        wgrad_stream, join, wgrad_slabs, wgrad_deferred_nblk, wgrad_deferred_launch, precision,
+                                        submanifold, 0, nullptr, nullptr, stream);
+}
+
+int ms3d_spconv_bn_fold_wanted(int V, int K, int Cin, int Cout, int offset_list, int pl_rows_bwd, int precision)
+{
+    const char *e = getenv("MS3D_BN_FOLD");
+    const int mode = e ? atoi(e) : -1;
+    if (mode == 0 || V <= 0 || K <= 1 || Cin % 16 || Cout % 16) return 0;
+    const int kind = ms3d_spconv_aux_kind_p(K, Cin, Cout, precision);
+    if (kind == MS3D_E_UNSUPPORTED) return 0;
+    const FwdGeom g = fwd_geometry(V, K, Cout, Cin, true, pl_rows_bwd);
+    if (!fwd_takes_small_f32(g, K, Cout, Cin, aux_pieces(kind) != 0)) return 0;
+    if (!ms3d_spconv_wgrad_is_table_walk(V, K, Cin, Cout, offset_list)) return 0;
+    if (mode > 0) return 1;
+    return V <= BN_FOLD_MAX_ROWS ? 1 : 0;
 }
 
 int ms3d_spconv_layer_backward_p(const float *x, const float *dy, const float *wf_buf, const int *nbr_fwd,
diff --git a/minsu3d_amd/csrc_host/ms3d_host.cpp b/minsu3d_amd/csrc_host/ms3d_host.cpp
--- a/minsu3d_amd/csrc_host/ms3d_host.cpp
+++ b/minsu3d_amd/csrc_host/ms3d_host.cpp
@@ -55,20 +55,21 @@
     int64_t vin, int64_t vout, int64_t K, int64_t cin, int64_t cout, const OptT &scale, const OptT &shift, const OptT &mean,
     const OptT &invstd, bool relu, bool training, bool need_dx, const OptT &dx_add, at::Tensor ws, const OptT &ol_kt_start,
     const OptT &ol_entries, const OptT &pl_tile_start, const OptT &pl_entries, int64_t ev0, int64_t ev1, int64_t ev2,
-    int64_t ev3, int64_t defer_floats, bool defer_launch, int64_t precision, int64_t submanifold)
+    int64_t ev3, int64_t defer_floats, bool defer_launch, int64_t precision, int64_t submanifold, bool defer_apply,
+    const OptT &fold_x, const OptT &fold_tab)
 {
     if (submanifold < 0) submanifold = (K == 27 && vin == vout) ? 1 : 0;
     TORCH_CHECK(x.is_cuda() && x.is_contiguous() && dy.is_contiguous(), "x / dy: contiguous device tensors");
     const bool has_bn = scale.has_value() && scale->defined();
     OptT dx, dgb, slabs;
     if (need_dx || has_bn) dx = at::empty({vin, cin}, x.options());
-    if (has_bn) dgb = at::empty({2, cin}, x.options());
+    if (has_bn) dgb = at::empty({defer_apply ? 5 : 2, cin}, x.options());
     at::Tensor dW = at::empty({K, cin, cout}, x.options());
     int nblk = 0;
     alignas(16) unsigned char launch[128];
     reinterpret_cast<int *>(launch)[4] = 0;
     if (defer_floats > 0) slabs = at::empty({defer_floats}, x.options());
-    check(ms3d_spconv_layer_backward_g(
+    check(ms3d_spconv_layer_backward_f(
               x.data_ptr<float>(), dy.data_ptr<float>(), wf_buf.data_ptr<float>(), nbr_fwd.data_ptr<int>(),
               nbr_bwd.data_ptr<int>(), (int)vin, (int)vout, (int)K, (int)cin, (int)cout, fptr(scale), fptr(shift), fptr(mean),
               fptr(invstd), (has_bn && relu) ? 1 : 0, (has_bn && training) ? 1 : 0, need_dx ? 1 : 0,
@@ -77,8 +78,8 @@
               iptr(ol_entries), iptr(pl_tile_start), iptr(pl_entries), (void *)ev0, (void *)ev1, (void *)ev2, (void *)ev3,
               nullptr, nullptr, 0, slabs.has_value() ? slabs->data_ptr<float>() : nullptr,
               slabs.has_value() ? &nblk : nullptr, (slabs.has_value() && defer_launch) ? (void *)launch : nullptr,
-              (int)precision, (int)submanifold, cur()),
-          "ms3d_spconv_layer_backward_g");
+              (int)precision, (int)submanifold, defer_apply ? 1 : 0, fptr(fold_x), fptr(fold_tab), cur()),
+          "ms3d_spconv_layer_backward_f");
     if (!need_dx) dx = c10::nullopt;
     const bool described = reinterpret_cast<int *>(launch)[4] != 0;
     return {dx, dgb, dW, slabs, (int64_t)nblk, py::bytes(reinterpret_cast<const char *>(launch), described ? 128 : 0)};
@@ -154,7 +155,19 @@
               return conv_layer_forward(x, W, nbr_fwd, vout, K, cin, cout, mirror_bwd, pre_scale, pre_shift, pre_relu, residual,
                                         bias, wf_buf, nparts, pl_tile_start, pl_entries, ev_start, ev_stop, 0);
           });
-    m.def("conv_layer_backward_g", &conv_layer_backward);
+    m.def("conv_layer_backward_f", &conv_layer_backward);
+    m.def("conv_layer_backward_g",
+          [](const at::Tensor &x, const at::Tensor &dy, const at::Tensor &wf_buf, const at::Tensor &nbr_fwd,
+             const at::Tensor &nbr_bwd, int64_t vin, int64_t vout, int64_t K, int64_t cin, int64_t cout, const OptT &scale,
+             const OptT &shift, const OptT &mean, const OptT &invstd, bool relu, bool training, bool need_dx,
+             const OptT &dx_add, at::Tensor ws, const OptT &ol_kt_start, const OptT &ol_entries, const OptT &pl_tile_start,
+             const OptT &pl_entries, int64_t ev0, int64_t ev1, int64_t ev2, int64_t ev3, int64_t defer_floats,
+             bool defer_launch, int64_t precision, int64_t submanifold) {
+              return conv_layer_backward(x, dy, wf_buf, nbr_fwd, nbr_bwd, vin, vout, K, cin, cout, scale, shift, mean, invstd,
+                                         relu, training, need_dx, dx_add, ws, ol_kt_start, ol_entries, pl_tile_start,
+                                         pl_entries, ev0, ev1, ev2, ev3, defer_floats, defer_launch, precision, submanifold,
+                                         false, c10::nullopt, c10::nullopt);
+          });
     m.def("conv_layer_backward",
           [](const at::Tensor &x, const at::Tensor &dy, const at::Tensor &wf_buf, const at::Tensor &nbr_fwd,
              const at::Tensor &nbr_bwd, int64_t vin, int64_t vout, int64_t K, int64_t cin, int64_t cout, const OptT &scale,
@@ -164,7 +177,8 @@
              bool defer_launch, int64_t precision) {
               return conv_layer_backward(x, dy, wf_buf, nbr_fwd, nbr_bwd, vin, vout, K, cin, cout, scale, shift, mean, invstd,
                                          relu, training, need_dx, dx_add, ws, ol_kt_start, ol_entries, pl_tile_start,
-                                         pl_entries, ev0, ev1, ev2, ev3, defer_floats, defer_launch, precision, -1);
+                                         pl_entries, ev0, ev1, ev2, ev3, defer_floats, defer_launch, precision, -1, false,
+                                         c10::nullopt, c10::nullopt);
           });
     m.def("conv_layer_backward",
           [](const at::Tensor &x, const at::Tensor &dy, const at::Tensor &wf_buf, const at::Tensor &nbr_fwd,
@@ -175,7 +189,8 @@
              bool defer_launch) {
               return conv_layer_backward(x, dy, wf_buf, nbr_fwd, nbr_bwd, vin, vout, K, cin, cout, scale, shift, mean, invstd,
                                          relu, training, need_dx, dx_add, ws, ol_kt_start, ol_entries, pl_tile_start,
-                                         pl_entries, ev0, ev1, ev2, ev3, defer_floats, defer_launch, 0, -1);
+                                         pl_entries, ev0, ev1, ev2, ev3, defer_floats, defer_launch, 0, -1, false, c10::nullopt,
+                                         c10::nullopt);
           });
     m.def("bn_finalize", &bn_finalize);
     m.def("gather_rows", &gather_rows);
```

After: 194.8 scenes/sec. -2.1%, worse.
